# scroll-tech/zkevm-circuits

Hardware: AMD Instinct MI355X
Metric: SuperCircuit-shape proof-gen wall-clock (s) at k = 20 (lower is better)
Workload: dtype u32x8 limbs (254-bit modular integer, Montgomery)

## Files before the change

zkevm-circuits_amd/csrc/api.hip:

```cpp
#include <algorithm>
#include <set>

#include <thread>
#include "ctx.hpp"
#include "host_fq.hpp"
#include "host_util.hpp"

namespace zk {

Fr fr_from_u64(uint64_t v) {
    Fr a = Fr::zero();
    a.l[0] = (uint32_t)v;
    a.l[1] = (uint32_t)(v >> 32);
    return to_mont(a);
}
Fr fr_pow(Fr base, uint64_t e) { return pow_u64(base, e); }
Fr fr_inv_host(const Fr& a) { return inv(a); }
static Fr root_of_unity_28() {
    Fr c = Fr{{0x60c37c9cu, 0xd34f1ed9u, 0xd39329c8u, 0x3215cf6du, 0x3dd31f74u, 0x98865ea9u, 0x166d18b7u, 0x03ddb9f5u}};
    return to_mont(c);
}
Fr fr_root_of_unity(uint32_t log_n) {
    Fr w = root_of_unity_28();
    for (uint32_t i = log_n; i < 28; ++i) w = sqr(w);
// ... 32 lines not shown
        if (alias) st = prev_st;
        else {
            if (hipStreamCreateWithFlags(&st, hipStreamNonBlocking) != hipSuccess) { delete c; return ZK_ERR_HIP; }
            c->owned_streams.push_back(st);
            prev_st = st;
        }
        bool ok = st != nullptr;
        switch (alias ? *q - 'A' + 'a' : *q) {
            case 'm': if (c->stream) ok = false; else c->stream = st; break;
            case 'c': if (c->stream_copy) ok = false; else { c->stream_copy = st; ok = hipEventCreateWithFlags(&c->ev_copy, hipEventDisableTiming) == hipSuccess; } break;
            case 'a': if (c->stream_aux) ok = false; else { c->stream_aux = st; ok = hipEventCreateWithFlags(&c->ev_aux, hipEventDisableTiming) == hipSuccess; } break;
            case '2': if (c->stream2) ok = false; else c->stream2 = st; break;
            case 'b': if (c->stream2b) ok = false; else c->stream2b = st; break;
            case 'x': if (c->stream2c) ok = false; else c->stream2c = st; break;
            case 'd': break;
            default: ok = false;
        }
        if (!ok) { delete c; return ZK_ERR_INVALID_ARG; }
    }
    if (!c->stream) { delete c; return ZK_ERR_INVALID_ARG; }
    if (c->stream2) for (int i = 0; i < 3; ++i) { (void)hipEventCreateWithFlags(&c->ev_p1[i], hipEventDisableTiming); (void)hipEventCreateWithFlags(&c->ev_p2[i], hipEventDisableTiming); }
    c->own_stream = true;
    if (hipEventCreate(&c->ev0) != hipSuccess || hipEventCreate(&c->ev1) != hipSuccess) { delete c; return ZK_ERR_HIP; }
    *out = c;
    return ZK_OK;
}

void zk_ctx_destroy(zk_ctx* ctx) {
    if (!ctx) return;
    (void)hipSetDevice(ctx->device);
    (void)hipStreamSynchronize(ctx->stream);
    ctx->domains.clear();
    for (auto& kv : ctx->pow_tables) (void)hipFree(kv.second);
    ctx->pool_trim();
    ctx->prof_resolve();
    for (auto e : ctx->prof_pool) (void)hipEventDestroy(e);
    for (auto& s : ctx->scratch) if (s.ptr) (void)hipFree(s.ptr);
    if (ctx->ev0) (void)hipEventDestroy(ctx->ev0);
    if (ctx->ev1) (void)hipEventDestroy(ctx->ev1);
    zk::comm_release(ctx);
    std::set<hipStream_t> streams(ctx->owned_streams.begin(), ctx->owned_streams.end());
    for (hipStream_t st : {ctx->stream2, ctx->stream2b, ctx->stream2c, ctx->stream_aux, ctx->stream_copy}) if (st) streams.insert(st);
    if (ctx->own_stream && ctx->stream) streams.insert(ctx->stream); else streams.erase(ctx->stream);
    for (hipStream_t st : streams) { (void)hipStreamSynchronize(st); (void)hipStreamDestroy(st); }
    if (ctx->ev_aux) (void)hipEventDestroy(ctx->ev_aux);
    if (ctx->ev_copy) (void)hipEventDestroy(ctx->ev_copy);
    if (ctx->ev_pipe) (void)hipEventDestroy(ctx->ev_pipe);
    for (auto& kv : ctx->msm_graphs) (void)hipGraphExecDestroy((hipGraphExec_t)kv.second);
    for (auto e : ctx->ev_p1) if (e) (void)hipEventDestroy(e);
    for (auto e : ctx->ev_p2) if (e) (void)hipEventDestroy(e);
    delete ctx;
}

const char* zk_last_error(const zk_ctx* ctx) { return ctx ? ctx->err.c_str() : "null context"; }

int zk_ctx_set_stream(zk_ctx* ctx, void* hip_stream) {
    if (!ctx) return ZK_ERR_INVALID_ARG;
    ZK_HIP(ctx, hipStreamSynchronize(ctx->stream));
    if (ctx->own_stream && ctx->stream) {
        bool shared = false;
        for (hipStream_t st : {ctx->stream2, ctx->stream2b, ctx->stream2c, ctx->stream_aux, ctx->stream_copy}) shared |= st == ctx->stream;
        if (!shared) {
            ctx->owned_streams.erase(std::remove(ctx->owned_streams.begin(), ctx->owned_streams.end(), ctx->stream), ctx->owned_streams.end());
            (void)hipStreamDestroy(ctx->stream);
        }
        ctx->own_stream = false;
// ... 195 lines not shown
    Fr omega_inv = fr_inv_host(omega);
    Fr ninv = fr_inv_host(fr_from_u64(1ull << log_n));
    return ntt_run_many(ctx, (Fr* const*)d_datas, nullptr, count, log_n, omega_inv, &ninv, nullptr, nullptr, false);
}
int zk_ntt_omega(zk_ctx* ctx, void* d_data, uint32_t log_n, const void* h_omega) {
    if (!ctx) return ZK_ERR_INVALID_ARG;
    ZK_REQUIRE(ctx, d_data && h_omega, "null pointer");
    ZK_REQUIRE(ctx, log_n <= 28, "log_n exceeds the two-adicity of Fr (28)");
    return ntt_run(ctx, (Fr*)d_data, log_n, *(const Fr*)h_omega, nullptr, nullptr, nullptr);
}
int zk_coeff_to_extended(zk_ctx* ctx, const void* d_coeffs, uint32_t k, uint32_t ext_k, void* d_out) {
    if (!ctx) return ZK_ERR_INVALID_ARG;
    ZK_REQUIRE(ctx, d_coeffs && d_out && d_coeffs != d_out, "null or aliased pointer");
    ZK_REQUIRE(ctx, k <= ext_k && ext_k <= 28, "need k <= ext_k <= 28");
    const size_t n = (size_t)1 << k, ne = (size_t)1 << ext_k;
    ZK_HIP(ctx, hipMemcpyAsync(d_out, d_coeffs, n * sizeof(Fr), hipMemcpyDeviceToDevice, ctx->stream));
    if (ne > n) ZK_HIP(ctx, hipMemsetAsync((char*)d_out + n * sizeof(Fr), 0, (ne - n) * sizeof(Fr), ctx->stream));
    Fr zeta = fr_zeta();
    int rc = ntt_run(ctx, (Fr*)d_out, ext_k, fr_root_of_unity(ext_k), nullptr, &zeta, nullptr);
    return rc;
}
int zk_coeff_to_coset(zk_ctx* ctx, const void* d_coeffs, uint32_t k, const void* h_g, void* d_out) {
    if (!ctx) return ZK_ERR_INVALID_ARG;
    ZK_REQUIRE(ctx, d_coeffs && d_out && h_g, "null pointer");
    ZK_REQUIRE(ctx, k <= 28, "k exceeds the two-adicity of Fr (28)");
    return ntt_run(ctx, (Fr*)d_out, k, fr_root_of_unity(k), nullptr, (const Fr*)h_g, nullptr, d_coeffs == d_out ? nullptr : (const Fr*)d_coeffs, true);
}
int zk_coeff_to_coset_batch(zk_ctx* ctx, const void* const* d_coeffs, uint32_t k, const void* h_g, void* const* d_outs, size_t count) {
    if (!ctx) return ZK_ERR_INVALID_ARG;
    ZK_REQUIRE(ctx, (d_coeffs && d_outs) || !count, "null pointer");
    ZK_REQUIRE(ctx, h_g, "null pointer");
    ZK_REQUIRE(ctx, k <= 28, "k exceeds the two-adicity of Fr (28)");
    for (size_t i = 0; i < count; ++i) ZK_REQUIRE(ctx, d_coeffs[i] && d_outs[i], "null column pointer");
    return ntt_run_many(ctx, (Fr* const*)d_outs, (const Fr* const*)d_coeffs, count, k, fr_root_of_unity(k), nullptr, (const Fr*)h_g, nullptr, true);
}
int zk_extended_to_coeff(zk_ctx* ctx, void* d_ext, uint32_t ext_k) {
    if (!ctx) return ZK_ERR_INVALID_ARG;
    ZK_REQUIRE(ctx, d_ext, "null pointer");
    ZK_REQUIRE(ctx, ext_k <= 28, "ext_k exceeds 28");
    Fr omega_inv = fr_inv_host(fr_root_of_unity(ext_k));
    Fr ninv = fr_inv_host(fr_from_u64(1ull << ext_k));
    Fr zeta_inv = sqr(fr_zeta());
    return ntt_run(ctx, (Fr*)d_ext, ext_k, omega_inv, &ninv, nullptr, &zeta_inv);
}

int zk_msm_g1(zk_ctx* ctx, const void* d_scalars, const void* d_bases, size_t n, void* h_out_affine) {
    if (!ctx) return ZK_ERR_INVALID_ARG;
    ZK_REQUIRE(ctx, h_out_affine && ((d_scalars && d_bases) || n == 0), "null pointer");
    return msm_run(ctx, (const Fr*)d_scalars, (const G1Affine*)d_bases, n, (G1Affine*)h_out_affine);
}
int zk_commit(zk_ctx* ctx, const zk_srs* srs, int basis, const void* d_scalars, size_t n, void* h_out_affine) {
    if (!ctx) return ZK_ERR_INVALID_ARG;
    ZK_REQUIRE(ctx, srs && h_out_affine && (d_scalars || !n), "null pointer");
    ZK_REQUIRE(ctx, basis == 0 || basis == 1, "basis must be 0 (monomial) or 1 (Lagrange)");
    ZK_REQUIRE(ctx, n <= ((size_t)1 << srs->k), "polynomial longer than the SRS");
    const G1Affine* b = basis ? srs->g_lagrange : srs->g;
    ZK_REQUIRE(ctx, b, "SRS has no Lagrange basis");
    const Fr* sp = (const Fr*)d_scalars;
    return msm_batch_srs(ctx, srs, basis, &sp, 1, n, (G1Affine*)h_out_affine);
}
int zk_g1_sum_host(const void* h_points_affine, size_t n, void* h_out_affine) {
    if (!h_out_affine || (!h_points_affine && n)) return ZK_ERR_INVALID_ARG;
    const G1Affine* p = (const G1Affine*)h_points_affine;
    host::PXyzz acc;
    memset(&acc, 0, sizeof acc);
    const host::F4 one = host::fone<host::FqC>();
    for (size_t i = 0; i < n; ++i) {
// ... 178 lines not shown
```

zkevm-circuits_amd/csrc/ctx.hpp:

```cpp
#pragma once
#include <hip/hip_runtime.h>
#include <cstdarg>
#include <cstdio>
#include <cstring>
#include <map>
#include <memory>
#include <string>
#include <vector>

#include "../../include/zkmi355.h"
#include "ec.hip.hpp"
#include "ff.hip.hpp"

namespace zk {

struct NttDomain;

struct Scratch {
    void* ptr = nullptr;
    size_t cap = 0;
};

}

// ... 2 lines not shown
    hipStream_t stream = nullptr;
    bool own_stream = false;
    std::string err;
    hipEvent_t ev0 = nullptr, ev1 = nullptr;
    hipDeviceProp_t prop{};
    zk::Scratch scratch[19];
    hipStream_t stream2 = nullptr, stream2b = nullptr, stream2c = nullptr;
    std::vector<hipStream_t> owned_streams;
    hipEvent_t ev_p1[3] = {nullptr, nullptr, nullptr}, ev_p2[3] = {nullptr, nullptr, nullptr};
    std::map<uint64_t, std::vector<uint64_t>> msm_graph_keys;
    std::map<uint64_t, void*> msm_graphs;
    uint32_t msm_blinded_tail = 0;
    bool msm_graph_broken = false;
    hipEvent_t ev_pipe = nullptr;
    hipStream_t stream_copy = nullptr;
    hipEvent_t ev_copy = nullptr;
    hipStream_t stream_aux = nullptr;
    hipEvent_t ev_aux = nullptr;
    bool ensure_aux() {
        if (stream_aux) return ev_aux || hipEventCreateWithFlags(&ev_aux, hipEventDisableTiming) == hipSuccess;
        int least = 0, greatest = 0;
        const char* e = getenv("ZK_AUX_PRIORITY");
        const bool prio = e && atoi(e) == 1 && hipDeviceGetStreamPriorityRange(&least, &greatest) == hipSuccess && greatest != least;
        hipError_t rc = prio ? hipStreamCreateWithPriority(&stream_aux, hipStreamNonBlocking, greatest) : hipStreamCreateWithFlags(&stream_aux, hipStreamNonBlocking);
        if (rc != hipSuccess) { (void)hipGetLastError(); rc = hipStreamCreateWithFlags(&stream_aux, hipStreamNonBlocking); }
        if (rc != hipSuccess) { stream_aux = nullptr; return false; }
        if (!ev_aux && hipEventCreateWithFlags(&ev_aux, hipEventDisableTiming) != hipSuccess) return false;
        return true;
    }
    void* comm = nullptr;
    uint32_t comm_rank = 0, comm_world = 1;
    std::map<uint64_t, std::shared_ptr<zk::NttDomain>> domains;
    std::map<uint64_t, void*> pow_tables;
    std::vector<void*> pinned;
    std::map<size_t, std::vector<void*>> pool;
    size_t pool_bytes = 0, pool_cap = (size_t)96 << 30;
    size_t coset_cache_bytes = 0;
    void* pool_get(size_t bytes) {
        bytes = (bytes + 255) & ~(size_t)255;
        if (!bytes) bytes = 256;
        auto it = pool.find(bytes);
        if (it != pool.end() && !it->second.empty()) { void* p = it->second.back(); it->second.pop_back(); pool_bytes -= bytes; return p; }
        void* p = nullptr;
        if (hipMalloc(&p, bytes) == hipSuccess) return p;
        (void)hipGetLastError();
        pool_trim();
        if (hipMalloc(&p, bytes) == hipSuccess) return p;
        (void)hipGetLastError();
        return nullptr;
    }
    void pool_put(void* p, size_t bytes) {
        if (!p) return;
        bytes = (bytes + 255) & ~(size_t)255;
        if (!bytes) bytes = 256;
        if (pool_bytes + bytes > pool_cap) { (void)hipStreamSynchronize(stream); (void)hipFree(p); return; }
        pool[bytes].push_back(p);
        pool_bytes += bytes;
    }
    void pool_trim() {
        (void)hipStreamSynchronize(stream);
        for (auto& kv : pool) for (void* p : kv.second) (void)hipFree(p);
        pool.clear();
        pool_bytes = 0;
    }
    uint32_t msm_attr_set = 0;
    bool quotient_attr_set = false;
// ... 75 lines not shown
    zk::G1Affine* pfx_negtot_tab[2] = {nullptr, nullptr};
};

#define ZK_HIP(ctx, call)                                                                          \
    do {                                                                                           \
        hipError_t e__ = (call);                                                                   \
        if (e__ != hipSuccess) return (ctx)->fail(ZK_ERR_HIP, "%s failed: %s (%s:%d)", #call, hipGetErrorString(e__), __FILE__, __LINE__); \
    } while (0)

#define ZK_CHECK_LAUNCH(ctx)                                                                       \
    do {                                                                                           \
        hipError_t e__ = hipGetLastError();                                                        \
        if (e__ != hipSuccess) return (ctx)->fail(ZK_ERR_HIP, "kernel launch failed: %s (%s:%d)", hipGetErrorString(e__), __FILE__, __LINE__); \
    } while (0)

#define ZK_REQUIRE(ctx, cond, msg)                                                                 \
    do {                                                                                           \
        if (!(cond)) return (ctx)->fail(ZK_ERR_INVALID_ARG, "invalid argument: %s (%s:%d)", msg, __FILE__, __LINE__); \
    } while (0)

namespace zk {
enum ScratchSlot { SC_NTT = 0, SC_MSM_KEYS = 1, SC_MSM_BUCKETS = 2, SC_MSM_MISC = 3, SC_POLY = 4, SC_POLY2 = 5, SC_TMP = 6, SC_TMP2 = 7, SC_MSM_BUCKETS2 = 8, SC_MSM_RESULTS = 9, SC_QTMP = 10, SC_COMM = 11, SC_MSM_BUCKETS3 = 12, SC_MSM_BUCKETS4 = 13, SC_MSM_DESC = 14, SC_MSM_TAILS = 15, SC_NTT_AUX = 16, SC_QACC = 17, SC_QSLICE = 18 };

Fr fr_from_u64(uint64_t v);
Fr fr_pow(Fr base, uint64_t e);
Fr fr_inv_host(const Fr& a);
Fr fr_root_of_unity(uint32_t log_n);
Fr fr_zeta();

int ntt_run(zk_ctx* ctx, Fr* d_data, uint32_t log_n, const Fr& omega, const Fr* scale , const Fr* coset_pre , const Fr* coset_post ,
            const Fr* d_src = nullptr ,
            bool fuse_pre = false );
int ntt_run_many(zk_ctx* ctx, Fr* const* d_datas, const Fr* const* d_srcs, size_t count, uint32_t log_n, const Fr& omega, const Fr* scale, const Fr* coset_pre, const Fr* coset_post, bool fuse_pre);
int fr_scale_run(zk_ctx* ctx, Fr* d_a, const Fr& s, uint64_t n);
enum G1Enc : int { G1_ENC_COMPRESSED = 0, G1_ENC_RAW = 1, G1_ENC_BE_XY = 2 };
int g1_decode_run(zk_ctx* ctx, const void* d_in, int enc, G1Affine* d_out, uint64_t n, uint32_t* d_bad, uint8_t* d_bad_at);
int msm_run(zk_ctx* ctx, const Fr* d_scalars, const G1Affine* d_bases, size_t n, G1Affine* h_out);
int msm_run_rp(zk_ctx* ctx, const Fr* d_scalars, const G1Affine* d_bases, const G1Affine* d_bases_rp, size_t n, G1Affine* h_out);
int msm_batch_rp(zk_ctx* ctx, const Fr* const* d_scalar_ptrs, size_t count, const G1Affine* d_bases, const G1Affine* d_bases_rp, size_t n, G1Affine* h_out);
int msm_segments_run(zk_ctx* ctx, const Fr* d_scalars, const G1Affine* d_bases, const uint32_t* h_off, size_t num_segments, G1Affine* h_out);
int srs_bases_rp(zk_ctx* ctx, const zk_srs* srs, int basis, const G1Affine** out);
int srs_window_table(zk_ctx* ctx, const zk_srs* srs, int basis, size_t n, const G1Affine** out, size_t* stride);
typedef int (*MsmStageFn)(void* user, size_t it);
int msm_batch_tab(zk_ctx* ctx, const Fr* const* d_scalar_ptrs, size_t count, const G1Affine* d_bases, const G1Affine* d_bases_rp, const G1Affine* d_table, size_t tab_stride,
                  size_t n, G1Affine* h_out, MsmStageFn stage = nullptr, void* stage_user = nullptr);
int msm_batch_srs(zk_ctx* ctx, const zk_srs* srs, int basis, const Fr* const* d_scalar_ptrs, size_t count, size_t n, G1Affine* h_out, MsmStageFn stage = nullptr, void* stage_user = nullptr,
                  const uint8_t* narrow = nullptr );
int msm_runs_try(zk_ctx* ctx, const zk_srs* srs, int basis, const Fr* const* d_scalar_ptrs, size_t count, size_t n, const uint8_t* narrow, G1Affine* h_out, uint8_t* done);
int msm_diff_try(zk_ctx* ctx, const zk_srs* srs, int basis, const Fr* const* d_scalar_ptrs, size_t count, size_t n, const uint8_t* narrow, G1Affine* h_out, uint8_t* done);
int commit_batch_staged(zk_ctx* ctx, const zk_srs* srs, int basis, const void* const* d_scalar_ptrs, size_t count, size_t n, void* h_out_affine, MsmStageFn stage, void* stage_user, const uint8_t* narrow = nullptr);
void sample_narrow(const void* const* h_cols, size_t count, size_t n, uint8_t* narrow);
int sample_narrow_dev(zk_ctx* ctx, const void* const* d_cols, size_t count, size_t n, uint8_t* narrow);
int sample_narrow_dev_typed(zk_ctx* ctx, const void* const* d_cols, const uint8_t* widths, size_t count, size_t n, size_t rows, uint8_t* narrow);
int lookup_multiplicities_enqueue(zk_ctx* ctx, const Fr* const* d_inputs, size_t num_inputs, const Fr* d_table, size_t usable_rows, Fr* d_m, size_t n, uint32_t* d_status, bool reuse_hash = false);
struct MockFail { uint32_t kind, index, sub, row; };
int mock_hash_build(zk_ctx* ctx, const Fr* d_table, size_t rows, int scratch_slot, const uint32_t** slots_out, uint32_t* mask_out);
int mock_nonzero_enqueue(zk_ctx* ctx, const Fr* d_vals, const uint32_t* d_row_ids, uint32_t count, uint32_t kind, uint32_t index, uint32_t sub, MockFail* d_out, uint32_t cap, uint32_t* d_counter);
int mock_probe_enqueue(zk_ctx* ctx, const Fr* d_inputs, const Fr* d_table, const uint32_t* d_slots, uint32_t mask, const uint32_t* d_row_ids, uint32_t count,
                       uint32_t kind, uint32_t index, uint32_t sub, MockFail* d_out, uint32_t cap, uint32_t* d_counter);
int mock_perm_enqueue(zk_ctx* ctx, const Fr* const* d_sigma, const Fr* const* d_cols, const Fr* d_ids, const uint32_t* d_slots, uint32_t mask, uint32_t num_cols, uint32_t k,
                      uint32_t kind, MockFail* d_out, uint32_t cap, uint32_t* d_counter);
int fr_add_const_many(zk_ctx* ctx, const void* const* d_src, void* const* d_dst, size_t count, const void* h_k, size_t n);
int fr_from_uint_run(zk_ctx* ctx, hipStream_t stream, const void* d_packed, uint32_t width, uint64_t n, Fr* d_out);
int fr_from_uint_batch_run(zk_ctx* ctx, hipStream_t stream, const void* const* d_packed, const uint8_t* widths, size_t count, uint64_t n, Fr* const* d_out);
int sigma_from_mapping_run(zk_ctx* ctx, hipStream_t stream, const void* const* d_map, size_t count, uint64_t n, uint32_t P, const Fr* d_omega, const Fr* d_delta, uint32_t* d_bad, Fr* const* d_out);
int g_to_lagrange(zk_ctx* ctx, const G1Affine* d_g, uint32_t k, G1Affine* d_out);
// ... 9 lines not shown
```

zkevm-circuits_amd/csrc/ff29.hip.hpp:

```cpp
#pragma once
#include "ff.hip.hpp"

namespace zk {

constexpr uint32_t MASK29 = (1u << 29) - 1;

struct Fq29P {
    static constexpr uint32_t INV = 0x4866389u;
    __host__ __device__ static constexpr uint32_t M(int i) {
        constexpr uint32_t m[9] = {0x187cfd47u, 0x10460b6u, 0x1c72a34fu, 0x2d522d0u, 0x1585d978u, 0x2db40c0u, 0xa6e141u, 0xe5c2634u, 0x30644eu};
        return m[i];
    }
    using P32 = FqP;
};
struct Fr29P {
    static constexpr uint32_t INV = 0xfffffffu;
    __host__ __device__ static constexpr uint32_t M(int i) {
        constexpr uint32_t m[9] = {0x10000001u, 0x1f0fac9fu, 0xe5c2450u, 0x7d090f3u, 0x1585d283u, 0x2db40c0u, 0xa6e141u, 0xe5c2634u, 0x30644eu};
        return m[i];
    }
    using P32 = FrP;
};

template <class P>
// ... 354 lines not shown
    uint32_t m[9];
    F29<P> t;
    uint64_t acc = 0;
#pragma unroll
    for (int k = 0; k < 17; ++k) {
        const int lo = k < 9 ? 0 : k - 8, hi = k < 9 ? k : 8, nm = k < 9 ? k : 17 - k;
        uint32_t ys[9], ds[9], fs[9], ks[9];
#pragma unroll
        for (int i = lo; i <= hi; ++i) { ys[i - lo] = b.l[k - i]; ds[i - lo] = d.l[k - i]; fs[i - lo] = f.l[k - i]; ks[i - lo] = P::M(k - i); }
        acc = dotv(a.l + lo, ys, hi - lo + 1, acc);
        acc = dotv(c.l + lo, ds, hi - lo + 1, acc);
        acc = dotv(e.l + lo, fs, hi - lo + 1, acc);
        acc = dotk(m + lo, ks, nm, acc);
        if (k < 9) {
            m[k] = ((uint32_t)acc * P::INV) & MASK29;
            acc += (uint64_t)m[k] * P::M(0);
        } else {
            t.l[k - 9] = (uint32_t)acc & MASK29;
        }
        acc >>= 29;
    }
    t.l[8] = (uint32_t)acc;
    return t;
}
template <int K, class P>
__host__ __device__ __forceinline__ F29<P> neg29k(const F29<P>& b) {
    F29<P> r;
#pragma unroll
    for (int i = 0; i < 9; ++i) r.l[i] = kp_balanced<P>(K, i) - b.l[i];
    return r;
}

template <class P>
__host__ __device__ __forceinline__ Fp<typename P::P32> reduce_lazy29(const F29<P>& x) {
    constexpr uint64_t mhi = ((uint64_t)P::P32::M(7) << 32) | P::P32::M(6);
    constexpr uint32_t C = (uint32_t)((((unsigned __int128)1) << 92) / ((unsigned __int128)mhi + 1));
    const uint32_t q = (uint32_t)(((uint64_t)x.l[8] * C) >> 52);
    F29<P> r;
    int64_t c = 0;
#pragma unroll
    for (int i = 0; i < 9; ++i) {
        const int64_t s_ = (int64_t)x.l[i] - (int64_t)((uint64_t)q * P::M(i)) + c;
        r.l[i] = i < 8 ? (uint32_t)(s_ & MASK29) : (uint32_t)s_;
        c = s_ >> 29;
    }
    return pack29_lt2p(r);
}

template <class P>
__host__ __device__ __forceinline__ F29<P> sqr29_c(const F29<P>& a) {
    uint32_t m[9], a2[9];
#pragma unroll
    for (int i = 0; i < 9; ++i) a2[i] = a.l[i] << 1;
    F29<P> t;
    uint64_t acc = 0;
#pragma unroll
    for (int k = 0; k < 17; ++k) {
        const int lo = k < 9 ? 0 : k - 8, hi = k < 9 ? k : 8, nm = k < 9 ? k : 17 - k;
        uint32_t xs[9], ys[9], ks[9];
        int n = 0;
#pragma unroll
        for (int i = lo; 2 * i < k; ++i) { xs[n] = a2[i]; ys[n] = a.l[k - i]; ++n; }
        if (!(k & 1)) { xs[n] = a.l[k / 2]; ys[n] = a.l[k / 2]; ++n; }
#pragma unroll
        for (int i = lo; i <= hi; ++i) ks[i - lo] = P::M(k - i);
        acc = dotv(xs, ys, n, acc);
        acc = dotk(m + lo, ks, nm, acc);
        if (k < 9) {
            m[k] = ((uint32_t)acc * P::INV) & MASK29;
            acc += (uint64_t)m[k] * P::M(0);
        } else {
            t.l[k - 9] = (uint32_t)acc & MASK29;
        }
        acc >>= 29;
    }
    t.l[8] = (uint32_t)acc;
    return t;
}


// ... 88 lines not shown
```

zkevm-circuits_amd/csrc/ntt.hip:

```cpp
#include <climits>
#include <type_traits>

#include "ctx.hpp"
#include "ff29.hip.hpp"

namespace zk {

constexpr int NTT_MAX_DIGIT = 10;
constexpr int NTT_TILE = 4096;
constexpr int NTT_THREADS = 1024;
constexpr int NTT_LDS_BYTES_PER_ELT = 36;

struct Tw29;

constexpr int NTT_BATCH = 16;
struct NttIo { const Fr* src[NTT_BATCH]; Fr* dst[NTT_BATCH]; };

struct NttPass {
    int log_np;
    int log_m;
    const Tw29* tw;
    const Fr* out_tw = nullptr;
};

// ... 21 lines not shown
__device__ __forceinline__ uint32_t bitrev(uint32_t x, int bits) { return bits ? (__brev(x) >> (32 - bits)) : 0u; }

__host__ __device__ __forceinline__ Fr to_rprime(Fr x) {
#pragma unroll
    for (int i = 0; i < 5; ++i) x = dbl(x);
    return x;
}

struct Lds29 {
    uint32_t* p;
    int stride;
    __device__ __forceinline__ Fr29 load(int idx) const {
        Fr29 r;
#pragma unroll
        for (int k = 0; k < 9; ++k) r.l[k] = p[k * stride + idx];
        return r;
    }
    __device__ __forceinline__ void store(int idx, const Fr29& v) const {
#pragma unroll
        for (int k = 0; k < 9; ++k) p[k * stride + idx] = v.l[k];
    }
};

__global__ void k_powers(Fr base, Fr mul, Fr* out, uint32_t count, int rprime) {
    uint32_t j = blockIdx.x * blockDim.x + threadIdx.x;
    if (j >= count) return;
    Fr r = mul, b = base;
    uint32_t e = j;
    while (e) {
        if (e & 1) r = r * b;
        b = sqr(b);
        e >>= 1;
    }
    stg(out + j, rprime ? to_rprime(r) : r);
}

__device__ __forceinline__ Fr two_level(const Fr* __restrict__ lo, const Fr* __restrict__ hi, int h, uint32_t e) {
    return ldg(lo + (e & ((1u << h) - 1))) * ldg(hi + (e >> h));
}
__device__ __forceinline__ Fr29 two_level29(const Fr* __restrict__ lo, const Fr* __restrict__ hi, int h, uint32_t e) {
    return mul29(unpack29<Fr29P>(ldg(lo + (e & ((1u << h) - 1)))), unpack29<Fr29P>(ldg(hi + (e >> h))));
}

__global__ void k_build_out_twiddles(Fr* __restrict__ out_tw, const Fr* __restrict__ lo, const Fr* __restrict__ hi, int h, int log_np, int log_m, int tw_shift, uint64_t n,
                                     Fr fin, int apply_fin) {
    const uint64_t g = (uint64_t)blockIdx.x * blockDim.x + threadIdx.x;
    if (g >= n) return;
    const uint64_t m = 1ull << log_m;
    const uint32_t jpp = (uint32_t)(g & (m - 1)), d = (uint32_t)(g >> log_m) & ((1u << log_np) - 1);
    Fr29 v = two_level29(lo, hi, h, (jpp * d) << tw_shift);
    if (apply_fin) v = mul29(v, unpack29<Fr29P>(fin));
    stg(out_tw + g, pack29_lt2p(v));
}

__device__ __forceinline__ void bfly29(Fr29& u, Fr29& x, const Fr29& w) {
    const Fr29 v = mul29(x, w);
    Fr29 a0 = add29(u, v), a1 = sub29k<4>(u, v);
    normalize29(a0);
    normalize29(a1);
    u = a0;
    x = a1;
}
struct Tw29 { uint4 q[3]; };
__device__ __forceinline__ Fr29 tw29(const Tw29* __restrict__ tw, uint32_t idx) {
    const uint4 a = tw[idx].q[0], b = tw[idx].q[1], c = tw[idx].q[2];
    return Fr29{{a.x, a.y, a.z, a.w, b.x, b.y, b.z, b.w, c.x}};
}
// ... 123 lines not shown
    for (int s = 0; s < log_np;) {
        const int r = ((log_np - s) & 1) ? 1 : 2;
        auto step = [&](auto R, auto FIRST, auto LAST) {
            ntt_pass_step<decltype(R)::value, decltype(FIRST)::value, decltype(LAST)::value, OPT_RUNTIME, OPT_RUNTIME>(L, src, dst, tw, pre, out_tw, lo, hi, h, tw_shift, log_np, s, log_t, 1ull << log_m, t.base, t.blk);
        };
        if (s == 0) { if (r == 1) step(Int<1>{}, Bool<true>{}, Bool<false>{}); else step(Int<2>{}, Bool<true>{}, Bool<false>{}); }
        else if (s + r == log_np) step(Int<2>{}, Bool<false>{}, Bool<true>{});
        else step(Int<2>{}, Bool<false>{}, Bool<false>{});
        s += r;
        if (s < log_np) __syncthreads();
    }
}
template <int LOG_NP, int S, bool HAS_PRE>
__device__ __forceinline__ void ntt_pass_steps(const Lds29& L, const Fr* __restrict__ src, Fr* __restrict__ dst, const Tw29* __restrict__ tw,
                                               const Fr* __restrict__ pre, const Fr* __restrict__ out_tw, const int log_t, const uint64_t m, const uint64_t base) {
    constexpr int R = ((LOG_NP - S) & 1) ? 1 : 2;
    constexpr bool LAST = S + R == LOG_NP;
    ntt_pass_step<R, S == 0, LAST, HAS_PRE ? OPT_YES : OPT_NO, OPT_YES>(L, src, dst, tw, pre, out_tw, nullptr, nullptr, 0, 0, LOG_NP, S, log_t, m, base, 0u);
    if constexpr (!LAST) {
        __syncthreads();
        ntt_pass_steps<LOG_NP, S + R, HAS_PRE>(L, src, dst, tw, pre, out_tw, log_t, m, base);
    }
}
template <int LOG_NP, bool HAS_PRE>
__global__ void __launch_bounds__(NTT_THREADS)
k_ntt_pass_f(NttIo io, const Tw29* __restrict__ tw, const Fr* __restrict__ lo, const Fr* __restrict__ hi, int h, int , int log_t, int log_m, int tw_shift,
             const Fr* __restrict__ pre, const Fr* __restrict__ out_tw, uint32_t ncols, int xcd_cols, int log_grp) {
    extern __shared__ __attribute__((aligned(16))) uint32_t smem[];
    const PassTile t = pass_tile(LOG_NP, log_t, log_m, ncols, xcd_cols, log_grp);
    ntt_pass_steps<LOG_NP, 0, HAS_PRE>(Lds29{smem, 1 << (LOG_NP + log_t)}, io.src[t.col], io.dst[t.col], tw, pre, out_tw, log_t, 1ull << log_m, t.base);
}

__host__ __device__ __forceinline__ int ntt_row_pad(int log_np) { return log_np >= 8 ? 8 : 0; }
template <int R, bool FIRST, bool LAST, Opt PRE, Opt FOLDED>
__device__ __forceinline__ void ntt_last_step(const Lds29& L, const Fr* __restrict__ src, Fr* __restrict__ dst, const Tw29* __restrict__ tw, const Fr* __restrict__ pre,
                                              const Fr29& fin29, const bool fin_folded, const int log_np, const int s, const int log_t, const int row,
                                              const uint32_t blk, const uint32_t mid, const int log_mid, const int log_n1) {
    static_assert(R == 2 || FIRST, "only the first step of a pass can be radix 2");
    constexpr int NE = 1 << R;
    const int hgt = 1 << s, T = 1 << log_t, items = (1 << (log_np + log_t)) >> R;
    const bool has_pre = opt_on<PRE>(pre != nullptr), folded = opt_on<FOLDED>(fin_folded);
    for (int it = threadIdx.x; it < items; it += blockDim.x) {
        int c, b;
        if (LAST) { c = it & (T - 1); b = it >> log_t; }
        else { b = it & ((1 << (log_np - R)) - 1); c = it >> (log_np - R); }
        const int j = b & (hgt - 1);
        const int lo_d = ((b >> s) << (s + R)) | j;
        const uint64_t i1 = ((uint64_t)blk << log_t) + c;
        Fr29 e[4];
        if (FIRST) {
            Fr raw[NE], praw[NE];
            uint64_t gi[NE];
#pragma unroll
            for (int k = 0; k < NE; ++k) {
                gi[k] = (((i1 << log_mid) + mid) << log_np) + bitrev(lo_d + k * hgt, log_np);
                raw[k] = ldg(src + gi[k]);
                if (PRE == OPT_YES) praw[k] = ldg(pre + gi[k]);
            }
#pragma unroll
            for (int k = 0; k < NE; ++k) {
                e[k] = unpack29<Fr29P>(raw[k]);
                if (has_pre) e[k] = mul29(e[k], unpack29<Fr29P>(PRE == OPT_YES ? praw[k] : ldg(pre + gi[k])));
            }
            dit_first_step<R>(e, tw, log_np);
        } else {
#pragma unroll
            for (int k = 0; k < NE; ++k) e[k] = L.load(c * row + lo_d + k * hgt);
            dit_step<R>(e, tw, log_np, s, j);
        }
#pragma unroll
        for (int k = 0; k < NE; ++k) {
            const int dl = lo_d + k * hgt;
            if (LAST) stg(dst + (i1 + (((uint64_t)mid + ((uint64_t)dl << log_mid)) << log_n1)), folded ? reduce_lazy29(e[k]) : pack29_lt2p(mul29(e[k], fin29)));
            else L.store(c * row + dl, e[k]);
        }
    }
}

__device__ __forceinline__ uint32_t last_tile(int xcd_remap) {
    return xcd_remap ? (blockIdx.x & 7u) * (gridDim.x >> 3) + (blockIdx.x >> 3) : blockIdx.x;
}

__global__ void __launch_bounds__(NTT_THREADS)
k_ntt_last(NttIo io, const Tw29* __restrict__ tw, int log_np, int log_t, int log_n1, int log_mid, Fr fin, const Fr* __restrict__ pre, int fin_folded, int xcd_remap) {
    extern __shared__ __attribute__((aligned(16))) uint32_t smem[];
    const Fr* __restrict__ src = io.src[blockIdx.y];
    Fr* __restrict__ dst = io.dst[blockIdx.y];
    const int row = (1 << log_np) + ntt_row_pad(log_np);
    const Lds29 L{smem, row << log_t};
    const uint32_t bx = last_tile(xcd_remap), mid = bx & ((1u << log_mid) - 1), blk = bx >> log_mid;
    const Fr29 fin29 = unpack29<Fr29P>(fin);
    for (int s = 0; s < log_np;) {
        const int r = ((log_np - s) & 1) ? 1 : 2;
        const bool last = s + r == log_np;
        auto step = [&](auto R, auto FIRST, auto LAST) {
            ntt_last_step<decltype(R)::value, decltype(FIRST)::value, decltype(LAST)::value, OPT_RUNTIME, OPT_RUNTIME>(L, src, dst, tw, pre, fin29, fin_folded != 0, log_np, s, log_t, row, blk, mid, log_mid, log_n1);
        };
        if (s == 0 && last) { if (r == 1) step(Int<1>{}, Bool<true>{}, Bool<true>{}); else step(Int<2>{}, Bool<true>{}, Bool<true>{}); }
        else if (s == 0) { if (r == 1) step(Int<1>{}, Bool<true>{}, Bool<false>{}); else step(Int<2>{}, Bool<true>{}, Bool<false>{}); }
        else if (last) step(Int<2>{}, Bool<false>{}, Bool<true>{});
        else step(Int<2>{}, Bool<false>{}, Bool<false>{});
        s += r;
        if (s < log_np) __syncthreads();
    }
}
template <int LOG_NP, int S>
__device__ __forceinline__ void ntt_last_steps(const Lds29& L, const Fr* __restrict__ src, Fr* __restrict__ dst, const Tw29* __restrict__ tw,
                                               const int log_t, const int row, const uint32_t blk, const uint32_t mid, const int log_mid, const int log_n1) {
    constexpr int R = ((LOG_NP - S) & 1) ? 1 : 2;
    constexpr bool LAST = S + R == LOG_NP;
    ntt_last_step<R, S == 0, LAST, OPT_NO, OPT_YES>(L, src, dst, tw, nullptr, Fr29{}, true, LOG_NP, S, log_t, row, blk, mid, log_mid, log_n1);
    if constexpr (!LAST) {
        __syncthreads();
        ntt_last_steps<LOG_NP, S + R>(L, src, dst, tw, log_t, row, blk, mid, log_mid, log_n1);
    }
}
template <int LOG_NP>
__global__ void __launch_bounds__(NTT_THREADS)
k_ntt_last_f(NttIo io, const Tw29* __restrict__ tw, int , int log_t, int log_n1, int log_mid, Fr fin, const Fr* __restrict__ pre, int fin_folded, int xcd_remap) {
    extern __shared__ __attribute__((aligned(16))) uint32_t smem[];
    const int row = (1 << LOG_NP) + ntt_row_pad(LOG_NP);
    const uint32_t bx = last_tile(xcd_remap), mid = bx & ((1u << log_mid) - 1), blk = bx >> log_mid;
    ntt_last_steps<LOG_NP, 0>(Lds29{smem, row << log_t}, io.src[blockIdx.y], io.dst[blockIdx.y], tw, log_t, row, blk, mid, log_mid, log_n1);
}

__global__ void k_scale(Fr* a, Fr s, uint64_t n) {
    uint64_t i = (uint64_t)blockIdx.x * blockDim.x + threadIdx.x;
    if (i < n) stg(a + i, ldg(a + i) * s);
}
int fr_scale_run(zk_ctx* ctx, Fr* d_a, const Fr& s, uint64_t n) {
    if (!n) return ZK_OK;
    hipLaunchKernelGGL(k_scale, dim3((unsigned)((n + 255) / 256)), dim3(256), 0, ctx->stream, d_a, s, n);
    ZK_CHECK_LAUNCH(ctx);
    return ZK_OK;
}

__global__ void k_distribute_powers(const Fr* src, Fr* dst, const Fr* __restrict__ lo, const Fr* __restrict__ hi, int h, uint64_t n) {
    uint64_t i = (uint64_t)blockIdx.x * blockDim.x + threadIdx.x;
    if (i >= n) return;
    stg(dst + i, ldg(src + i) * two_level(lo, hi, h, (uint32_t)i));
}

static int build_powers(zk_ctx* ctx, const Fr& base, const Fr& mul, Fr* d_out, uint32_t count, int rprime) {
    hipLaunchKernelGGL(k_powers, dim3((count + 255) / 256), dim3(256), 0, ctx->stream, base, mul, d_out, count, rprime);
    ZK_CHECK_LAUNCH(ctx);
    return ZK_OK;
}

static uint64_t domain_key(uint32_t log_n, const Fr& omega, const Fr* scale) {
    uint64_t hsh = 1469598103934665603ull;
    auto mix = [&](uint32_t v) { hsh = (hsh ^ v) * 1099511628211ull; };
    mix(log_n);
    for (int i = 0; i < 8; ++i) mix(omega.l[i]);
    if (scale) for (int i = 0; i < 8; ++i) mix(scale->l[i] ^ 0x9e3779b9u);
    return hsh;
}
// ... 160 lines not shown
    NttPlan pl{};
    int log_tile = 11;
    if (kn.last_logtile >= 10 && kn.last_logtile <= 12) log_tile = kn.last_logtile;
    pl.log_t = std::min(std::max(log_tile - ps.log_np, 0), log_n1);
    pl.tile = 1 << (ps.log_np + pl.log_t);
    pl.blocks = (unsigned)((1ull << dom.log_n) >> (ps.log_np + pl.log_t));
    pl.fixed = kn.fixed && P > 1 && dom.fin_folded && has_fixed_instance(ps.log_np);
    pl.grid = dim3(pl.blocks, (unsigned)nb);
    pl.threads = plan_threads(pl.tile, pl.fixed);
    pl.lds = (size_t)(pl.tile + (ntt_row_pad(ps.log_np) << pl.log_t)) * NTT_LDS_BYTES_PER_ELT;
    pl.xcd = (log_mid == 0 && pl.blocks % 8 == 0 && pl.blocks >= 16 && kn.xcd_last) ? 1 : 0;
    return pl;
}

static bool pass_kernel_ready(zk_ctx* ctx, const void* kernel, size_t max_lds) {
    auto it = ctx->ntt_fixed_attr.find(kernel);
    if (it != ctx->ntt_fixed_attr.end()) return it->second;
    const bool ok = hipFuncSetAttribute(kernel, hipFuncAttributeMaxDynamicSharedMemorySize, (int)max_lds) == hipSuccess;
    if (!ok) (void)hipGetLastError();
    return ctx->ntt_fixed_attr[kernel] = ok;
}
constexpr size_t NTT_PASS_MAX_LDS = (size_t)NTT_TILE * NTT_LDS_BYTES_PER_ELT, NTT_LAST_MAX_LDS = (size_t)(NTT_TILE + 128) * NTT_LDS_BYTES_PER_ELT;

using PassKernel = decltype(&k_ntt_pass);
using LastKernel = decltype(&k_ntt_last);
static PassKernel pass_instance(int log_np, bool pre) {
    switch (log_np) {
        case 7: return pre ? k_ntt_pass_f<7, true> : k_ntt_pass_f<7, false>;
        case 8: return pre ? k_ntt_pass_f<8, true> : k_ntt_pass_f<8, false>;
        case 9: return pre ? k_ntt_pass_f<9, true> : k_ntt_pass_f<9, false>;
        default: return pre ? k_ntt_pass_f<10, true> : k_ntt_pass_f<10, false>;
    }
}
static LastKernel last_instance(int log_np) {
    switch (log_np) {
        case 7: return k_ntt_last_f<7>;
        case 8: return k_ntt_last_f<8>;
        case 9: return k_ntt_last_f<9>;
        default: return k_ntt_last_f<10>;
    }
}
static int launch_pass(zk_ctx* ctx, const NttDomain& dom, int p, size_t nb, const NttKnobs& kn, const NttIo& io, const Fr* pre) {
    const NttPass& ps = dom.pass[p];
    if (ps.log_np < 3) return ctx->fail(ZK_ERR_INVALID_ARG, "NTT: a strided pass over a digit of 2^%d", ps.log_np);
    NttPlan pl = plan_pass(dom, p, nb, kn, ps.out_tw != nullptr);
    PassKernel kernel = pl.fixed ? pass_instance(ps.log_np, pre != nullptr) : k_ntt_pass;
    if (pl.fixed && !pass_kernel_ready(ctx, (const void*)kernel, NTT_PASS_MAX_LDS)) {
        NttKnobs generic = kn;
        generic.fixed = false;
        pl = plan_pass(dom, p, nb, generic, ps.out_tw != nullptr);
        kernel = k_ntt_pass;
    }
    if (!pl.fixed && !pass_kernel_ready(ctx, (const void*)kernel, NTT_PASS_MAX_LDS)) return ctx->fail(ZK_ERR_HIP, "NTT: the device refuses %zu bytes of LDS per workgroup", NTT_PASS_MAX_LDS);
    ZkProfScope pscope(ctx, "ntt_pass");
    pscope.bytes = (uint64_t)nb * (1ull << dom.log_n) * 64 / (uint64_t)dom.npass;
    hipLaunchKernelGGL(kernel, pl.grid, dim3(pl.threads), pl.lds, ctx->stream, io, ps.tw, (const Fr*)dom.d_lo, (const Fr*)dom.d_hi, dom.h, ps.log_np, pl.log_t, ps.log_m,
                       (int)dom.log_n - ps.log_np - ps.log_m, pre, ps.out_tw, (uint32_t)nb, pl.xcd, pl.log_grp);
    ZK_CHECK_LAUNCH(ctx);
    return ZK_OK;
}
static int launch_last(zk_ctx* ctx, const NttDomain& dom, size_t nb, const NttKnobs& kn, const NttIo& io, const Fr* pre) {
    const int P = dom.npass;
    const NttPass& ps = dom.pass[P - 1];
    NttPlan pl = plan_last(dom, nb, kn);
    LastKernel kernel = pl.fixed ? last_instance(ps.log_np) : k_ntt_last;
    if (pl.fixed && !pass_kernel_ready(ctx, (const void*)kernel, NTT_LAST_MAX_LDS)) {
        NttKnobs generic = kn;
        generic.fixed = false;
        pl = plan_last(dom, nb, generic);
        kernel = k_ntt_last;
    }
    if (!pl.fixed && !pass_kernel_ready(ctx, (const void*)kernel, NTT_LAST_MAX_LDS)) return ctx->fail(ZK_ERR_HIP, "NTT: the device refuses %zu bytes of LDS per workgroup", NTT_LAST_MAX_LDS);
    ZkProfScope pscope(ctx, "ntt_last");
    pscope.bytes = (uint64_t)nb * (1ull << dom.log_n) * 64 / (uint64_t)P;
    hipLaunchKernelGGL(kernel, pl.grid, dim3(pl.threads), pl.lds, ctx->stream, io, ps.tw, ps.log_np, pl.log_t, P == 1 ? 0 : dom.pass[0].log_np, P == 3 ? dom.pass[1].log_np : 0,
                       dom.final_mul, pre, dom.fin_folded ? 1 : 0, pl.xcd);
    ZK_CHECK_LAUNCH(ctx);
    return ZK_OK;
}

static size_t columns_per_launch(uint32_t log_n, size_t count, bool coset_pass, const NttKnobs& kn) {
    if (count <= 1 || coset_pass) return 1;
    const uint64_t tiles = std::max<uint64_t>(1, (1ull << log_n) >> 12);
    size_t per_launch = (size_t)std::min<uint64_t>(NTT_BATCH, std::max<uint64_t>(1, 4096 / tiles));
    if (kn.batch >= 1 && kn.batch <= NTT_BATCH) per_launch = (size_t)kn.batch;
    return per_launch;
}

int ntt_run(zk_ctx* ctx, Fr* d_data, uint32_t log_n, const Fr& omega, const Fr* scale, const Fr* coset_pre, const Fr* coset_post, const Fr* d_src, bool fuse_pre) {
    return ntt_run_many(ctx, &d_data, d_src ? &d_src : nullptr, 1, log_n, omega, scale, coset_pre, coset_post, fuse_pre);
}
int ntt_run_many(zk_ctx* ctx, Fr* const* d_datas, const Fr* const* d_srcs, size_t count, uint32_t log_n, const Fr& omega, const Fr* scale, const Fr* coset_pre, const Fr* coset_post, bool fuse_pre) {
    if (count == 0) return ZK_OK;
    const NttKnobs kn = read_ntt_knobs();
    if (log_n == 0) {
        for (size_t i = 0; i < count; ++i) {
            if (d_srcs && d_srcs[i] && d_srcs[i] != d_datas[i]) ZK_HIP(ctx, hipMemcpyAsync(d_datas[i], d_srcs[i], sizeof(Fr), hipMemcpyDeviceToDevice, ctx->stream));
            if (scale) {
                hipLaunchKernelGGL(k_scale, dim3(1), dim3(64), 0, ctx->stream, d_datas[i], *scale, (uint64_t)1);
                ZK_CHECK_LAUNCH(ctx);
            }
        }
        return ZK_OK;
    }
    const uint64_t n = 1ull << log_n;
    const Fr* pre_table = nullptr;
    int rc = (coset_pre && fuse_pre) ? get_pow_table(ctx, log_n, *coset_pre, POW_FULL, &pre_table) : ZK_OK;
    if (rc) return rc;
    const bool pre_apart = coset_pre && !pre_table;
    std::shared_ptr<NttDomain> dom;
    rc = get_domain(ctx, kn, log_n, omega, scale, &dom);
    if (rc) return rc;
    const int P = dom->npass;
    size_t per_launch = columns_per_launch(log_n, count, pre_apart || coset_post, kn);
    Fr* scratch = nullptr;
    if (P > 1) {
        const int slot = ctx->stream_aux && ctx->stream == ctx->stream_aux ? SC_NTT_AUX : SC_NTT;
        for (;;) {
            scratch = (Fr*)ctx->get_scratch(slot, sizeof(Fr) * n * per_launch);
            if (scratch || per_launch == 1) break;
            (void)hipGetLastError();
            per_launch = (per_launch + 1) / 2;
        }
        if (!scratch) return ZK_ERR_OOM;
    }
    for (size_t first = 0; first < count; first += per_launch) {
        const size_t nb = std::min(per_launch, count - first);
        NttIo io{};
        for (size_t j = 0; j < nb; ++j) {
            Fr* dd = d_datas[first + j];
            io.src[j] = d_srcs && d_srcs[first + j] ? d_srcs[first + j] : dd;
            if (pre_apart) { rc = run_distribute(ctx, log_n, *coset_pre, io.src[j], dd); if (rc) return rc; io.src[j] = dd; }
        }
        for (int p = 0; p + 1 < P; ++p) {
            for (size_t j = 0; j < nb; ++j) io.dst[j] = (p == P - 2) ? scratch + j * n : d_datas[first + j];
            rc = launch_pass(ctx, *dom, p, nb, kn, io, p == 0 ? pre_table : nullptr);
            if (rc) return rc;
            for (size_t j = 0; j < nb; ++j) io.src[j] = io.dst[j];
        }
        for (size_t j = 0; j < nb; ++j) io.dst[j] = d_datas[first + j];
        rc = launch_last(ctx, *dom, nb, kn, io, P == 1 ? pre_table : nullptr);
        if (rc) return rc;
        if (coset_post) for (size_t j = 0; j < nb; ++j) { rc = run_distribute(ctx, log_n, *coset_post, io.dst[j], io.dst[j]); if (rc) return rc; }
    }
    return ZK_OK;
}

template <int W>
__global__ void __launch_bounds__(256) k_ntt_cross(const Fr* __restrict__ recv, Fr* __restrict__ out, size_t cols, const Fr* __restrict__ tw , Fr scale, int scaled) {
    const size_t c = (size_t)blockIdx.x * blockDim.x + threadIdx.x;
    if (c >= cols) return;
    constexpr int LOGW = W == 2 ? 1 : W == 4 ? 2 : W == 8 ? 3 : 4;
    Fr a[W];
#pragma unroll
    for (int i = 0; i < W; ++i) {
        int rev = 0;
#pragma unroll
        for (int b = 0; b < LOGW; ++b) rev |= ((i >> b) & 1) << (LOGW - 1 - b);
        a[rev] = ldg(recv + (size_t)i * cols + c);
    }
#pragma unroll
    for (int st = 1; st <= LOGW; ++st) {
#pragma unroll
        for (int h = 0; h < W / 2; ++h) {
            const int half = 1 << (st - 1), t = h & (half - 1), lo = ((h >> (st - 1)) << st) + t, hi = lo + half;
            const Fr u = a[lo];
            const Fr v = t == 0 ? a[hi] : a[hi] * tw[t << (LOGW - st)];
            a[lo] = u + v;
            a[hi] = u - v;
        }
    }
#pragma unroll
    for (int j = 0; j < W; ++j) stg(out + (size_t)j * cols + c, scaled ? a[j] * scale : a[j]);
}

}

using namespace zk;
// ... 74 lines not shown
```

zkevm-circuits_amd/csrc/prover.hip:

```cpp
#include <algorithm>
#include <array>
#include <unordered_map>
#include <unordered_set>
#include <memory>
#include <string>

#include <chrono>
#include <cstdlib>
#include <random>
#include <tuple>
#include <functional>
#include "ctx.hpp"
#include "host_hash.hpp"
#include "cs.hpp"
#include "quotient_plan.hpp"

using namespace zk;
using zk::host::F4;
using namespace zk::cs;
using namespace zk::qplan;

extern "C" int zk_quotient_eval(zk_ctx*, const uint32_t*, uint32_t, const void* const*, uint32_t, const void*, uint32_t, uint32_t, uint32_t, int, void*);
extern "C" int zk_fr_powers(zk_ctx*, const void*, const void*, void*, size_t);
extern "C" int zk_ntt(zk_ctx*, void*, uint32_t, int);
extern "C" int zk_fr_batch_invert(zk_ctx*, void*, size_t);
extern "C" int zk_fr_random(zk_ctx*, const uint8_t*, uint64_t, uint64_t, void*, size_t);
extern "C" int zk_lookup_multiplicities(zk_ctx*, const void*, const void*, size_t, void*, size_t, uint64_t*);
extern "C" int zk_coeff_to_coset(zk_ctx*, const void*, uint32_t, const void*, void*);
extern "C" int zk_coeff_to_coset_batch(zk_ctx*, const void* const*, uint32_t, const void*, void* const*, size_t);
extern "C" int zk_fr_scatter_scaled(zk_ctx*, const void*, size_t, const void*, void*, size_t, size_t);
extern "C" int zk_msm_g1(zk_ctx*, const void*, const void*, size_t, void*);
extern "C" int zk_g1_sum_host(const void*, size_t, void*);
extern "C" int zk_poly_eval_batch(zk_ctx*, const void* const*, size_t, size_t, const void*, void*);
extern "C" int zk_poly_eval_pairs(zk_ctx*, const void* const*, const uint32_t*, size_t, const void*, size_t, size_t, void*);

namespace {

static thread_local zk_ctx* tl_pool_ctx = nullptr;
struct PoolScope {
    zk_ctx* prev;
    explicit PoolScope(zk_ctx* c) : prev(tl_pool_ctx) { tl_pool_ctx = c; }
    ~PoolScope() { tl_pool_ctx = prev; }
};

struct DevBuf {
// ... 27 lines not shown
        owner = nullptr;
        return hipMalloc(&p, n ? n : 1) == hipSuccess;
    }
    Fr* fr() const { return (Fr*)p; }
};

struct PinnedBuf {
    void* p = nullptr;
    ~PinnedBuf() { if (p) (void)hipHostFree(p); }
    bool alloc(size_t bytes) { return hipHostMalloc(&p, bytes ? bytes : 1, hipHostMallocDefault) == hipSuccess; }
};


struct StageTrace {
    zk_ctx* ctx; bool on; std::chrono::steady_clock::time_point t0;
    explicit StageTrace(zk_ctx* c) : ctx(c), on(getenv("ZK_PROVER_TRACE") != nullptr), t0(std::chrono::steady_clock::now()) {}
    void mark(const char* what) {
        if (!on) return;
        (void)hipStreamSynchronize(ctx->stream);
        const auto t1 = std::chrono::steady_clock::now();
        fprintf(stderr, "[zk prover] %-28s %8.2f ms\n", what, std::chrono::duration<double, std::milli>(t1 - t0).count());
        t0 = t1;
    }
};

}

struct zk_pk : zk::cs::ConstraintSystem {
    std::vector<DevBuf> fixed_lag, fixed_coeff, sigma_lag, sigma_coeff;
    DevBuf omega_lag, l0_lag, llast_lag, lactive_lag, l0_coeff, llast_coeff, lactive_coeff;
    mutable std::vector<std::unordered_map<uint32_t, DevBuf>> part_cache;
    mutable int part_cache_state = -1;
    mutable size_t part_cache_bytes = 0;
    std::vector<G1Affine> fixed_com, sigma_com;
    F4 vk_repr;
    const zk_srs* srs = nullptr;
    mutable std::shared_ptr<const QuotientPlan> qplan;
};

struct zk_proof {
    const zk_pk* pk;
    host::XorShiftRng rng;
    host::Transcript tr;
    std::vector<DevBuf> inst_lag, inst_coeff, adv_lag, adv_coeff;
    std::vector<std::vector<DevBuf>> adv_coset;
    std::vector<uint32_t> pre_mask;
    bool pre_planned = false;
    uint32_t phase = 0;
    int multiopen = ZK_MULTIOPEN_GWC;
    int vanishing_random = ZK_VANISHING_ONE;
    bool advice_on_device = false;
    bool advice_in_place = false;
    bool lag_partial = false;
    std::vector<F4> absorbed;
    zk_transcript_vtable ext_vt{};
    uint32_t rank = 0, world = 1;
    zk_allgather_fn gather = nullptr;
    void* gather_user = nullptr;
    bool use_comm = false;
    zk_allgather_fn gather_dev = nullptr;
    void* gather_dev_user = nullptr;
    std::vector<F4> challenges;
    zk_proof(const zk_pk* k, const uint8_t* seed) : pk(k), rng(seed), inst_lag(k->I), inst_coeff(k->I), adv_lag(k->A), adv_coeff(k->A), challenges(k->chal_phase.size(), host::fr_zero()) {}
};

namespace {

#define PK_TRY(expr) do { int rc__ = (expr); if (rc__) return rc__; } while (0)
#define PK_ALLOC(ctx, buf, nbytes) do { if (!(buf).alloc(nbytes)) return (ctx)->fail(ZK_ERR_OOM, "prover: alloc failed"); } while (0)

struct StreamRestore {
    zk_ctx* c; hipStream_t s;
    explicit StreamRestore(zk_ctx* ctx) : c(ctx), s(ctx->stream) {}
    ~StreamRestore() { c->stream = s; }
};

size_t device_free_bytes(bool* ok = nullptr) {
    size_t free_b = 0, total_b = 0;
    const bool got = hipMemGetInfo(&free_b, &total_b) == hipSuccess;
    if (!got) { (void)hipGetLastError(); free_b = 0; }
    if (ok) *ok = got;
    return free_b;
}

struct PairOwners {
    uint32_t E = 0, rank = 0;
    bool sharded = false;
    std::vector<uint32_t> owner;
    size_t at(uint32_t e, uint32_t r) const { return ((size_t)e << E) | r; }
    bool mine(uint32_t e, uint32_t r) const { return class_on_coset(E, e, r) && (!sharded || owner[at(e, r)] == rank); }
};

template <class Count>
std::vector<std::pair<uint32_t, uint32_t>> cosets_by_columns_served(uint32_t R, Count served) {
    std::vector<std::pair<uint32_t, uint32_t>> by_count;
    for (uint32_t r = 0; r < R; ++r) {
        const uint32_t cnt = served(r);
        if (cnt) by_count.push_back({cnt, r});
    }
    std::sort(by_count.begin(), by_count.end(), [](const auto& a, const auto& b) { return a.first != b.first ? a.first > b.first : a.second < b.second; });
    return by_count;
}

int lincomb(zk_ctx* ctx, uint32_t k, const std::vector<const void*>& polys, const F4& ch, void* d_out) {
    std::vector<uint32_t> words;
    std::vector<const void*> cols;
    for (size_t j = polys.size(); j-- > 0;) { words.insert(words.end(), {Q_PUSH_COL, (uint32_t)cols.size(), 0u, Q_FOLD, 0u, 0u}); cols.push_back(polys[j]); }
    return zk_quotient_eval(ctx, words.data(), (uint32_t)(words.size() / 3), cols.data(), (uint32_t)cols.size(), &ch, 1, k, k, 0, d_out);
}

int commit_lagrange(zk_ctx* ctx, const zk_srs* srs, const Fr* d_vals, size_t n, G1Affine* out) { return zk_commit(ctx, srs, 1, d_vals, n, out); }
int commit_coeff(zk_ctx* ctx, const zk_srs* srs, const Fr* d_vals, size_t n, G1Affine* out) { return zk_commit(ctx, srs, 0, d_vals, n, out); }

int to_coeff(zk_ctx* ctx, const zk_pk* pk, const DevBuf& lag, DevBuf* coeff) {
    const size_t n = (size_t)1 << pk->k;
// ... 64 lines not shown
        default: break;
    }
    if (ref >= C_DELTA0 && ref - C_DELTA0 < e.beta_delta.size()) { *out = e.beta_delta[ref - C_DELTA0]; return true; }
    if (ref >= C_CHAL0 && ref - C_CHAL0 < e.challenges.size()) { *out = e.challenges[ref - C_CHAL0]; return true; }
    if (ref >= C_YPOW0 && ref < C_CHAL0) { *out = ref - C_YPOW0 < e.ypow.size() ? e.ypow[ref - C_YPOW0] : host::fr_pow(e.y, ref - C_YPOW0); return true; }
    return false;
}
int concretise(zk_ctx* ctx, const Env& e, const Prog& g, Concrete* c) {
    for (const Instr& in : g) {
        uint32_t a = in.a;
        if (in.op == Q_PUSH_COL) {
            auto it = c->col_index.find(in.a);
            if (it == c->col_index.end()) {
                const void* p = resolve_col(e, in.a);
                if (!p) return ctx->fail(ZK_ERR_INVALID_ARG, "prover: unresolved column reference 0x%08x", in.a);
                a = (uint32_t)c->cols.size();
                c->cols.push_back(p);
                c->col_index[in.a] = a;
            } else a = it->second;
        } else if (in.op == Q_PUSH_CONST || in.op == Q_FOLD || in.op == Q_MUL_CONST || in.op == Q_ADD_CONST) {
            auto it = c->const_index.find(in.a);
            if (it == c->const_index.end()) {
                F4 v;
                if (!resolve_const(e, in.a, &v)) return ctx->fail(ZK_ERR_INVALID_ARG, "prover: unresolved constant reference 0x%08x", in.a);
                a = (uint32_t)c->consts.size();
                c->consts.push_back(v);
                c->const_index[in.a] = a;
            } else a = it->second;
        }
        c->words.push_back(in.op); c->words.push_back(a); c->words.push_back(in.b);
    }
    return ZK_OK;
}
int run_program(zk_ctx* ctx, const Env& e, const Prog& g, void* d_out) {
    Concrete c;
    PK_TRY(concretise(ctx, e, g, &c));
    {
        static const int alias = getenv("ZK_QUOTIENT_ALIAS") ? atoi(getenv("ZK_QUOTIENT_ALIAS")) : 0;
        if (alias > 0 && ctx->prof_tag && !strcmp(ctx->prof_tag, "quotient_coset")) for (size_t i = 0; i < c.cols.size(); ++i) c.cols[i] = c.cols[i % (size_t)alias];
    }
    return zk_quotient_eval(ctx, c.words.data(), (uint32_t)(c.words.size() / 3), c.cols.data(), (uint32_t)c.cols.size(),
                            c.consts.empty() ? nullptr : c.consts.data(), (uint32_t)c.consts.size(), e.pk->k, e.pk->k, 0, d_out);
}
const Fr* coeff_of(const zk_pk* pk, uint32_t ref, const std::vector<DevBuf>& adv, const std::vector<DevBuf>& inst, const std::vector<DevBuf>& pz,
                   const std::vector<DevBuf>& lkm, const std::vector<DevBuf>& lkphi) {
    const uint32_t type = ref >> 24, idx = ref & 0xFFFFFF;
    auto at = [&](const std::vector<DevBuf>& v) -> const Fr* { return idx < v.size() ? v[idx].fr() : nullptr; };
    switch (type) {
        case CT_FIXED: return at(pk->fixed_coeff);
        case CT_ADVICE: return at(adv);
        case CT_INSTANCE: return at(inst);
        case CT_SPECIAL: return idx == SP_L0 ? pk->l0_coeff.fr() : idx == SP_LLAST ? pk->llast_coeff.fr() : idx == SP_LACTIVE ? pk->lactive_coeff.fr() : nullptr;
        case CT_PERM_Z: return at(pz);
        case CT_SIGMA: return at(pk->sigma_coeff);
        case CT_LK_M: return at(lkm);
        case CT_LK_PHI: return at(lkphi);
        default: return nullptr;
    }
}

size_t share_size(const zk_proof* pr, size_t count) { return (count + pr->world - 1) / pr->world; }
int share_gather(zk_ctx* ctx, const zk_proof* pr, const void* local, size_t count, size_t elem, void* out) {
    const size_t per = share_size(pr, count);
    std::vector<uint8_t> all(per * pr->world * elem);
    if (per && pr->gather(pr->gather_user, local, per * elem, all.data())) return ctx->fail(ZK_ERR_INVALID_ARG, "sharded session: all-gather callback failed");
    for (size_t i = 0; i < count; ++i) memcpy((uint8_t*)out + i * elem, all.data() + ((i % pr->world) * per + i / pr->world) * elem, elem);
    return ZK_OK;
}

int sharded_commit(zk_ctx* ctx, const zk_proof* pr, const zk_srs* srs, int basis, const void* const* ptrs, size_t count, size_t n, G1Affine* out, uint8_t kind = 0 ) {
    const std::vector<uint8_t> hint(count, kind);
    if (pr->world <= 1 || !pr->gather) return commit_batch_staged(ctx, srs, basis, ptrs, count, n, out, nullptr, nullptr, hint.data());
    if (count < pr->world && n >= ((size_t)pr->world << 10)) {
        const size_t base = n / pr->world, rem = n % pr->world;
        const size_t lo = pr->rank * base + std::min<size_t>(pr->rank, rem), len = base + (pr->rank < rem ? 1 : 0);
// ... 505 lines not shown
    StageTrace trace(ctx);
    struct Stage {
        zk_ctx* ctx; size_t body, tail;
        std::vector<const void*> src; std::vector<void*> dst; std::vector<F4> blind_v; const F4* blind = nullptr;
        std::vector<uint8_t> width;
        void* packed = nullptr;
        bool grouped = false; size_t expanded = 0;
        uint32_t world = 1;
        hipMemcpyKind kind = hipMemcpyHostToDevice;
        std::vector<size_t> own;
        const zk_pk* pk = nullptr; std::vector<DevBuf*> lag, coeff;
        zk_proof* pr = nullptr; std::vector<uint32_t> col; std::vector<size_t> pending; std::vector<Fr> g_of_r;
        int flush() {
            if (pending.empty()) return ZK_OK;
            StreamRestore back(ctx);
            ctx->stream = ctx->stream_aux;
            const size_t n_ = (size_t)1 << pk->k;
            std::vector<Fr*> dsts;
            std::vector<const Fr*> srcs;
            for (size_t c_ : pending) {
                PK_ALLOC(ctx, *coeff[c_], n_ * 32);
                dsts.push_back(coeff[c_]->fr());
                srcs.push_back(lag[c_]->fr());
            }
            const Fr omega_inv = fr_inv_host(fr_root_of_unity(pk->k)), ninv = fr_inv_host(fr_from_u64(1ull << pk->k));
            PK_TRY(ntt_run_many(ctx, dsts.data(), srcs.data(), dsts.size(), pk->k, omega_inv, &ninv, nullptr, nullptr, false));
            for (size_t r = 0; r < g_of_r.size(); ++r) {
                std::vector<const void*> csrc;
                std::vector<void*> cdst;
                for (size_t c_ : pending) {
                    const uint32_t gc = col[c_];
                    if (!(pr->pre_mask[gc] >> r & 1u)) continue;
                    DevBuf& slot = pr->adv_coset[r][gc];
                    if (!slot.alloc(n_ * 32)) {
                        for (uint32_t& m_ : pr->pre_mask) m_ = 0;
                        break;
                    }
                    csrc.push_back(coeff[c_]->p);
                    cdst.push_back(slot.p);
                }
                if (!csrc.empty()) PK_TRY(zk_coeff_to_coset_batch(ctx, csrc.data(), pk->k, &g_of_r[r], cdst.data(), csrc.size()));
            }
            pending.clear();
            return ZK_OK;
        }
    } sg{ctx, (size_t)pk->u * 32, (size_t)(pk->bf + 1) * 32, {}, {}, {}};
    sg.pk = pk;
    sg.pr = pr;
    sg.kind = dev_src ? hipMemcpyDeviceToDevice : hipMemcpyHostToDevice;
    sg.grouped = dev_src && widths;
    for (uint32_t c = 0; c < pk->A; ++c) {
        if (!seen[c]) continue;
        if (in_place && by_col[c] && (!owner_only || sg.dst.size() % pr->world == pr->rank)) pr->adv_lag[c].borrow(const_cast<void*>(by_col[c]));
        else if (!pr->adv_lag[c].alloc(n * 32)) return ctx->fail(ZK_ERR_OOM, "prover: alloc of %zu bytes failed", n * 32);
        sg.src.push_back(by_col[c]);
        sg.width.push_back(width_of[c]);
        sg.dst.push_back(pr->adv_lag[c].p);
        sg.lag.push_back(&pr->adv_lag[c]);
        sg.coeff.push_back(&pr->adv_coeff[c]);
        sg.col.push_back(c);
        for (uint32_t r = 0; r <= pk->bf; ++r) sg.blind_v.push_back(pr->rng.next_fr());
    }
    DevBuf packed_buf;
    size_t widest_packed = 0;
    for (uint8_t w : sg.width) if (w < 32) widest_packed = std::max<size_t>(widest_packed, w);
    if (widest_packed && !sg.grouped) {
        PK_ALLOC(ctx, packed_buf, (size_t)pk->u * widest_packed);
        sg.packed = packed_buf.p;
    }
    PinnedBuf blind_pinned;
    if (!blind_pinned.alloc(sg.blind_v.size() * sizeof(F4))) return ctx->fail(ZK_ERR_OOM, "prover: pinned staging allocation failed");
    memcpy(blind_pinned.p, sg.blind_v.data(), sg.blind_v.size() * sizeof(F4));
    sg.blind = (const F4*)blind_pinned.p;
    trace.mark("  advice: blinding rows drawn and staged");
// ... 175 lines not shown
        const int rc = choose_quotient_plan(*pk, knobs, &pk->qplan, &err);
        if (rc) return ctx->fail(rc, "%s", err.c_str());
    }
    *out = pk->qplan;
    return ZK_OK;
}
static int advice_coset_plan(zk_ctx* ctx, const zk_pk* pk, std::vector<uint32_t>& mask, size_t* key_slots = nullptr) {
    std::shared_ptr<const QuotientPlan> qp;
    PK_TRY(quotient_plan(ctx, pk, &qp));
    advice_coset_masks(*pk, *qp, mask, key_slots);
    return ZK_OK;
}
static int advice_lagrange_readers(zk_ctx* ctx, const zk_pk* pk, std::vector<uint8_t>* need) {
    std::shared_ptr<const QuotientPlan> qp;
    PK_TRY(quotient_plan(ctx, pk, &qp));
    advice_lagrange_readers(*pk, *qp, need);
    return ZK_OK;
}


static int plan_advice_cosets(zk_ctx* ctx, zk_proof* pr) {
    pr->pre_planned = true;
    const zk_pk* pk = pr->pk;
    const bool sharded = pr->world > 1 && pr->gather;
    const char* env = getenv("ZK_ADVICE_COSET_GB");
    const double cap = (env ? atof(env) : (pr->advice_on_device ? 0.0 : 64.0)) * (double)(1ull << 30);
    if (sharded || cap <= 0 || pk->A == 0) return ZK_OK;
    std::vector<uint32_t> mask;
    size_t key_slots = 0;
    PK_TRY(advice_coset_plan(ctx, pk, mask, &key_slots));
    const uint32_t E = pk->ext_k - pk->k, R = 1u << E;
    if (E > 5) return ZK_OK;
    const double col_bytes = (double)((size_t)1 << pk->k) * 32.0;
    bool mem_known = false;
    const size_t free_b = device_free_bytes(&mem_known);
    if (!mem_known) return ZK_OK;
    const double cols_ahead = (pr->advice_in_place ? 1.0 : 2.0) * pk->A + 3.0 * (2.0 * pk->L + pk->C) + (2.0 * pk->L + pk->C + pk->I + 8.0) + 2.0 * R + 32.0;
    double avail = (double)free_b + (double)ctx->pool_bytes - cols_ahead * col_bytes - 16.0 * (double)(1ull << 30);
    if (pk->part_cache_state < 0 || (pk->part_cache_state == 1 && pk->part_cache_bytes == 0)) {
        const double key_need = (double)key_slots * col_bytes;
        const char* kenv = getenv("ZK_PK_COSET_CACHE_GB");
        const double kcap = std::min((kenv ? atof(kenv) : 96.0) * (double)(1ull << 30), (double)ctx->prop.totalGlobalMem / 3.0);
        if (key_need <= kcap) avail -= std::max(0.0, key_need - (double)pk->part_cache_bytes);
    }
    const double budget = std::min(cap, avail);
    const auto by_count = cosets_by_columns_served(R, [&](uint32_t r) { uint32_t cnt = 0; for (uint32_t m_ : mask) cnt += m_ >> r & 1u; return cnt; });
    uint32_t chosen = 0;
    double used = 0;
    for (const auto& cr : by_count) {
        uint32_t rest = 0;
        for (uint32_t m_ : mask) rest += (m_ & ~(chosen | 1u << cr.second)) != 0;
        if (used + cr.first * col_bytes > cap || used + (cr.first + rest) * col_bytes > avail) break;
        used += cr.first * col_bytes;
        chosen |= 1u << cr.second;
    }
    if (getenv("ZK_PROVER_TRACE")) {
        fprintf(stderr, "[zk prover] advice coset plan: free %.1f + pooled %.1f GiB, reserve %.1f GiB, budget %.1f GiB, cosets by columns served:", free_b / 1073741824.0, ctx->pool_bytes / 1073741824.0,
                (cols_ahead * col_bytes) / 1073741824.0 + 16.0, budget / 1073741824.0);
        for (const auto& cr : by_count) fprintf(stderr, " r%u:%u", cr.second, cr.first);
        fprintf(stderr, " -> chosen 0x%x\n", chosen);
    }
    if (!chosen) return ZK_OK;
    pr->pre_mask.assign(pk->A, 0u);
    for (uint32_t c = 0; c < pk->A; ++c) pr->pre_mask[c] = mask[c] & chosen;
    pr->adv_coset.resize(R);
    for (auto& v : pr->adv_coset) v.resize(pk->A);
    if (getenv("ZK_PROVER_TRACE")) fprintf(stderr, "[zk prover] advice cosets computed ahead: cosets 0x%x, %.1f GiB\n", chosen, used / (double)(1ull << 30));
    return ZK_OK;
}

int zk_pk_quotient_plan(zk_ctx* ctx, const zk_pk* pk, uint32_t* out_summary, size_t cap_summary) {
    if (!ctx) return ZK_ERR_INVALID_ARG;
    ZK_REQUIRE(ctx, pk && out_summary, "null pointer");
    std::shared_ptr<const QuotientPlan> qp;
    PK_TRY(quotient_plan(ctx, pk, &qp));
    if (write_plan_summary(*qp, out_summary, cap_summary, 0xFFFFFFFFu, nullptr, 0, nullptr)) return ctx->fail(ZK_ERR_INVALID_ARG, "zk_pk_quotient_plan: the summary needs %u words", 8 + 8 * (qp->E + 1));
    return ZK_OK;
}


struct Finish {
    zk_ctx* ctx;
    zk_proof* pr;
    const zk_pk* pk;
    const zk_srs* srs;
    const uint32_t k, ext_k;
    const size_t n;
    Env lag;
    StageTrace trace;
    const bool sharded;
    const bool shard_args;
    std::vector<uint32_t> act;
    bool late_cosets = false;
    std::vector<std::vector<DevBuf>> lk_f;
    std::vector<DevBuf> lk_t, lk_m, lk_phi;
    std::vector<uint8_t> same_table;
    std::vector<uint32_t> table_owner;
    std::vector<DevBuf> pz_lag;
    DevBuf random_coeff;
    std::vector<DevBuf> pz_coeff, m_coeff, phi_coeff, rem_coeff;
    DevBuf h;
    F4 x, w, w_inv;
    std::vector<Open> evals, queries;
    size_t e_fix = 0, e_random = 0, e_sigma = 0, e_lk = 0;
    std::vector<size_t> e_pz;
    DevBuf hcomb;
    F4 h_eval;

    Finish(zk_ctx* c, zk_proof* p)
        : ctx(c), pr(p), pk(p->pk), srs(p->pk->srs), k(p->pk->k), ext_k(p->pk->ext_k), n((size_t)1 << p->pk->k),
          lag{p->pk, nullptr, &p->adv_lag, &p->inst_lag, nullptr, nullptr, nullptr, host::fr_one(), host::fr_one(), host::fr_one(), host::fr_one(), {}, p->challenges},
          trace(c), sharded(p->world > 1 && p->gather),
          shard_args(sharded && pk->L >= p->world && !(getenv("ZK_SHARD_LOOKUPS") && atoi(getenv("ZK_SHARD_LOOKUPS")) == 0)),
          lk_f(pk->L), lk_t(pk->L), lk_m(pk->L), lk_phi(pk->L), same_table(pk->L, 0), table_owner(pk->L, 0), pz_lag(pk->C),
          pz_coeff(pk->C), m_coeff(pk->L), phi_coeff(pk->L), e_pz(pk->C) {
        for (uint32_t l = 0; l < pk->L; ++l) if (!shard_args || l % pr->world == pr->rank) act.push_back(l);
        const Fr t = fr_root_of_unity(k);
        memcpy(w.l, &t, 32);
        w_inv = host::fr_inv(w);
    }
    Finish(const Finish&) = delete;
    Finish& operator=(const Finish&) = delete;

    F4 rotate(int32_t rot) const { F4 p = x; const F4 b = rot >= 0 ? w : w_inv; for (int32_t i = 0; i < (rot >= 0 ? rot : -rot); ++i) p = host::fr_mul(p, b); return p; }
    int32_t norm_rot(int32_t rot) const { const int64_t nn = (int64_t)n; return (int32_t)((((int64_t)rot % nn) + nn) % nn); }
    F4 point_of(int32_t nrot) const { const int64_t nn = (int64_t)n; return rotate(nrot > nn / 2 ? (int32_t)(nrot - nn) : nrot); }
};

struct AuxJoin { zk_ctx* c; const bool* on; ~AuxJoin() { if (*on && c->stream_aux) (void)hipStreamSynchronize(c->stream_aux); } };

static int stage_late_advice_cosets(Finish& f) {
    zk_ctx* ctx = f.ctx; zk_proof* pr = f.pr; const zk_pk* pk = f.pk; const size_t n = f.n;
    const char* env = getenv("ZK_ADVICE_COSET_LATE_GB");
    const double cap = (env ? atof(env) : 0.0) * (double)(1ull << 30);
    const uint32_t E = f.ext_k - f.k, R = 1u << E;
    if (f.sharded || !(cap > 0) || !pk->A || E > 5 || !ctx->ensure_aux()) return ZK_OK;
    std::vector<uint32_t> mask;
    size_t key_slots = 0;
    PK_TRY(advice_coset_plan(ctx, pk, mask, &key_slots));
    if (pr->adv_coset.empty()) { pr->adv_coset.resize(R); for (auto& v : pr->adv_coset) v.resize(pk->A); }
    const double col_bytes = (double)n * 32.0;
    const size_t free_b = device_free_bytes();
    double avail = (double)free_b + (double)ctx->pool_bytes - (4.0 * (2.0 * pk->L + pk->C) + (2.0 * pk->L + pk->C + pk->I + 8.0) + 2.0 * R + 32.0) * col_bytes - 24.0 * (double)(1ull << 30);
    if (pk->part_cache_state < 0 || (pk->part_cache_state == 1 && pk->part_cache_bytes == 0)) avail -= (double)key_slots * col_bytes;
    auto todo = [&](uint32_t r, uint32_t c) { return (mask[c] >> r & 1u) && !pr->adv_coset[r][c].p && pr->adv_coeff[c].p; };
    const auto by_count = cosets_by_columns_served(R, [&](uint32_t r) { uint32_t cnt = 0; for (uint32_t c = 0; c < pk->A; ++c) cnt += todo(r, c); return cnt; });
    double used = 0;
    StreamRestore back(ctx);
    const hipStream_t main_stream = ctx->stream;
    const Fr w_ext = fr_root_of_unity(f.ext_k);
    for (const auto& cr : by_count) {
        if (used + cr.first * col_bytes > std::min(cap, avail)) continue;
        Fr g = fr_zeta();
        for (uint32_t i = 0; i < cr.second; ++i) g = g * w_ext;
        std::vector<const void*> csrc;
        std::vector<void*> cdst;
        bool ok = true;
        for (uint32_t c = 0; c < pk->A && ok; ++c) {
            if (!todo(cr.second, c)) continue;
            DevBuf& slot = pr->adv_coset[cr.second][c];
            if (!slot.alloc(n * 32)) { ok = false; break; }
            csrc.push_back(pr->adv_coeff[c].p);
            cdst.push_back(slot.p);
        }
        if (!f.late_cosets) {
            ZK_HIP(ctx, hipEventRecord(ctx->ev_aux, main_stream));
            ZK_HIP(ctx, hipStreamWaitEvent(ctx->stream_aux, ctx->ev_aux, 0));
        }
        ctx->stream = ctx->stream_aux;
        f.late_cosets = true;
        if (!csrc.empty()) PK_TRY(zk_coeff_to_coset_batch(ctx, csrc.data(), f.k, &g, cdst.data(), csrc.size()));
        ctx->stream = main_stream;
        used += csrc.size() * col_bytes;
        if (!ok) break;
    }
    if (f.late_cosets) {
        ZK_HIP(ctx, hipEventRecord(ctx->ev_aux, ctx->stream_aux));
        if (getenv("ZK_PROVER_TRACE")) fprintf(stderr, "[zk prover] advice cosets computed beside the lookup / permutation stages: %.1f GiB\n", used / (double)(1ull << 30));
    }
    return ZK_OK;
}

static int exchange_owned(Finish& f, std::vector<DevBuf>& cols) {
    zk_ctx* ctx = f.ctx; const zk_proof* pr = f.pr; const size_t n = f.n;
    const size_t total = cols.size(), W = pr->world, groups_total = (total + W - 1) / W;
    static const size_t xg_knob = getenv("ZK_SHARD_EXCHANGE_GROUPS") ? (size_t)atol(getenv("ZK_SHARD_EXCHANGE_GROUPS")) : 16;
    const size_t XG = std::max<size_t>(1, std::min(xg_knob, groups_total));
    DevBuf gbuf, sbuf;
    PK_ALLOC(ctx, gbuf, W * XG * n * 32);
    PK_ALLOC(ctx, sbuf, XG * n * 32);
    HostStaging host;
    for (size_t grp0 = 0; grp0 < groups_total; grp0 += XG) {
        const size_t gcnt = std::min(XG, groups_total - grp0);
        for (size_t g = 0; g < gcnt; ++g) {
            const size_t mine_c = (grp0 + g) * W + pr->rank;
            if (mine_c < total) ZK_HIP(ctx, hipMemcpyAsync((char*)sbuf.p + g * n * 32, cols[mine_c].p, n * 32, hipMemcpyDeviceToDevice, ctx->stream));
            else ZK_HIP(ctx, hipMemsetAsync((char*)sbuf.p + g * n * 32, 0, n * 32, ctx->stream));
        }
        bool on_device = false;
        PK_TRY(allgather_rows(ctx, pr, false, sbuf.p, true, gcnt * n * 32, gbuf.p, host, &on_device));
        if (!on_device) PK_TRY(zk_h2d(ctx, gbuf.p, host.recv.data(), host.recv.size()));
        for (size_t g = 0; g < gcnt; ++g)
            for (uint32_t q_ = 0; q_ < W; ++q_) {
                const size_t c_ = (grp0 + g) * W + q_;
// ... 271 lines not shown
            PK_TRY(run_program(ctx, lag_r, rp.prog, f.rem_coeff[j].p));
            const F4 yp = host::fr_pow(f.lag.y, K - 1 - rp.last);
            PK_TRY(zk_fr_scale(ctx, f.rem_coeff[j].p, &yp, n));
            dsts.push_back(f.rem_coeff[j].fr());
        }
        const Fr omega_inv = fr_inv_host(fr_root_of_unity(pk->k)), ninv = fr_inv_host(fr_from_u64(1ull << pk->k));
        PK_TRY(ntt_run_many(ctx, dsts.data(), nullptr, dsts.size(), pk->k, omega_inv, &ninv, nullptr, nullptr, false));
        f.trace.mark("  quotient: remainders of the split constraints");
    }
    for (uint32_t e = 0; e <= E; ++e)
        if (q.cls(e).used || e == E) {
            PK_ALLOC(ctx, q.h[e], ((size_t)n << e) * 32);
            if (!q.cls(e).used) ZK_HIP(ctx, hipMemsetAsync(q.h[e].p, 0, ((size_t)n << e) * 32, ctx->stream));
        }
    return ZK_OK;
}

static void quotient_decide_key_cache(Finish& f, const Quotient& q) {
    zk_ctx* ctx = f.ctx; const zk_pk* pk = f.pk; const size_t n = f.n;
    const std::vector<uint32_t>& refs = q.plan->refs;
    size_t key_slots = 0;
    for (uint32_t ref : refs) {
        if (!key_column(ref)) continue;
        for (uint32_t r = 0; r < q.nparts; ++r) {
            bool read = false;
            for (uint32_t e = 0; e <= q.E && !read; ++e) read = q.cls(e).used && class_on_coset(q.E, e, r) && q.reads(e, ref);
            key_slots += read;
        }
    }
    const char* env = getenv("ZK_PK_COSET_CACHE_GB");
    double budget = (env ? atof(env) : 96.0) * (double)(1ull << 30);
    budget = std::min(budget, (double)ctx->prop.totalGlobalMem / 3.0) - (double)ctx->coset_cache_bytes;
    const size_t free_b = device_free_bytes();
    const double need = (double)key_slots * n * 32.0;
    const double session = (double)refs.size() * n * 32.0 + (double)((size_t)n << q.E) * 32.0 * 2.0;
    pk->part_cache_state = (need <= budget && need + session <= (double)free_b + (double)ctx->pool_bytes) ? 1 : 0;
    if (pk->part_cache_state) pk->part_cache.resize(q.nparts);
}

static int quotient_deal_pairs(Finish& f, const Quotient& q, CosetPass& cp) {
    zk_ctx* ctx = f.ctx; const zk_proof* pr = f.pr;
    const uint32_t E = q.E;
    cp.deal.resize(f.sharded ? pr->world : 1);
    cp.owners = PairOwners{E, pr->rank, f.sharded, std::vector<uint32_t>((size_t)(E + 1) << E, 0u)};
    if (f.sharded) {
        PK_ALLOC(ctx, cp.rtmp, f.n * 32);
        std::vector<QPair> all;
        for (uint32_t e = 0; e <= E; ++e)
            if (q.cls(e).used)
                for (uint32_t r = 0; r < q.nparts; r += 1u << (E - e)) all.push_back({e, r, (double)q.cls(e).refs.size() + (double)q.cls(e).prog.size() / 64.0});
        std::stable_sort(all.begin(), all.end(), [](const QPair& a, const QPair& b) { return a.cost > b.cost; });
        std::vector<double> load(pr->world, 0.0);
        for (const QPair& pp_ : all) {
            uint32_t best = 0;
            for (uint32_t q_ = 1; q_ < pr->world; ++q_) if (load[q_] < load[best]) best = q_;
            load[best] += pp_.cost;
            cp.deal[best].push_back(pp_);
            cp.owners.owner[cp.owners.at(pp_.e, pp_.r)] = best;
        }
        for (auto& d_ : cp.deal) std::sort(d_.begin(), d_.end(), [](const QPair& a, const QPair& b) { return a.r != b.r ? a.r < b.r : a.e < b.e; });
    }
    const Fr w_ext = fr_root_of_unity(f.ext_k);
    Fr g = fr_zeta();
    for (uint32_t r_ = 0; r_ < q.nparts; ++r_) {
        bool any = false;
        for (uint32_t e = 0; e <= E && !any; ++e) any = q.cls(e).used && cp.owners.mine(e, r_);
        if (any) cp.cosets.push_back({r_, g});
        g = g * w_ext;
    }
    return ZK_OK;
}

static int quotient_transform(Finish& f, const Quotient& q, CosetPass& cp, CosetWork& w) {
    zk_ctx* ctx = f.ctx; zk_proof* pr = f.pr; const zk_pk* pk = f.pk; const size_t n = f.n;
    const std::vector<uint32_t>& refs = q.plan->refs;
    std::vector<DevBuf>& bufs = cp.part_buf;
    const bool cache_on = cp.cache_on;
    const uint32_t k = f.k;
    const Fr w_n = fr_root_of_unity(k);
    auto pre_coset = [&](uint32_t ref, uint32_t r) -> const void* {
        if ((ref >> 24) != CT_ADVICE || r >= pr->adv_coset.size()) return nullptr;
        const uint32_t c_ = ref & 0xFFFFFFu;
        return c_ < pr->adv_coset[r].size() ? pr->adv_coset[r][c_].p : nullptr;
    };
    const uint32_t r_ = w.r;
    w.active.clear();
    for (uint32_t e = 0; e <= q.E; ++e)
        if (q.cls(e).used && cp.owners.mine(e, r_)) w.active.push_back(e);
    w.part_of.clear();
    std::vector<const void*> bat_src;
    std::vector<void*> bat_dst;
    std::vector<std::pair<uint32_t, DevBuf>> fresh_slots;
    for (size_t i = 0; i < refs.size(); ++i) {
        bool needed = false;
        for (uint32_t e : w.active) needed |= q.reads(e, refs[i]);
        if (!needed) continue;
        if (const void* pre = pre_coset(refs[i], r_)) { w.part_of[refs[i]] = pre; continue; }
        if (!(cache_on && key_column(refs[i])) && !bufs[i].p) PK_ALLOC(ctx, bufs[i], n * 32);
        void* dst = bufs[i].p;
        DevBuf fresh;
        const bool cached = cache_on && key_column(refs[i]);
        if (cached) {
            auto it = pk->part_cache[r_].find(refs[i]);
            if (it != pk->part_cache[r_].end()) { w.part_of[refs[i]] = it->second.p; continue; }
            const char* env_fail = getenv("ZK_PK_COSET_CACHE_FAIL_AFTER");
            const bool inject = env_fail && pk->part_cache_bytes / (n * 32) + fresh_slots.size() >= (size_t)atoll(env_fail);
            bool got = pk->part_cache_state == 1 && !inject && fresh.alloc_unpooled(n * 32);
            if (!got && pk->part_cache_state == 1) {
                (void)hipGetLastError();
                ctx->pool_trim();
                got = !inject && fresh.alloc_unpooled(n * 32);
                if (!got) { (void)hipGetLastError(); pk->part_cache_state = 2; }
            }
            if (got) dst = fresh.p;
            else {
                if (!bufs[i].p) PK_ALLOC(ctx, bufs[i], n * 32);
                dst = bufs[i].p;
            }
        }
        w.part_of[refs[i]] = dst;
        if (refs[i] == colref(CT_SPECIAL, SP_X)) PK_TRY(zk_fr_powers(ctx, &w_n, &w.g, dst, n));
        else {
            const Fr* cf = (refs[i] >> 24) == CT_SPLIT_R ? ((refs[i] & 0xFFFFFFu) < f.rem_coeff.size() ? f.rem_coeff[refs[i] & 0xFFFFFFu].fr() : nullptr)
                                                         : coeff_of(pk, refs[i], pr->adv_coeff, pr->inst_coeff, f.pz_coeff, f.m_coeff, f.phi_coeff);
            if (!cf) return ctx->fail(ZK_ERR_INVALID_ARG, "prover: unresolved column reference 0x%08x", refs[i]);
            bat_src.push_back(cf);
            bat_dst.push_back(dst);
        }
        if (cached && fresh.p) fresh_slots.emplace_back(refs[i], std::move(fresh));
    }
    PK_TRY(zk_coeff_to_coset_batch(ctx, bat_src.data(), k, &w.g, bat_dst.data(), bat_src.size()));
    for (auto& fs : fresh_slots) {
        pk->part_cache_bytes += n * 32;
        ctx->coset_cache_bytes += n * 32;
        pk->part_cache[r_][fs.first] = std::move(fs.second);
    }
    return ZK_OK;
}

static int quotient_programs(Finish& f, Quotient& q, CosetPass& cp, CosetWork& w) {
    zk_ctx* ctx = f.ctx; const size_t n = f.n;
    const uint32_t k = f.k, E = q.E, K = q.K;
    const bool sharded = f.sharded;
    const Fr one_fr = Fr::one();
    DevBuf& hpart = cp.hpart;
    Env& part = cp.part;
    std::vector<DevBuf>& mine = cp.mine;
    const uint32_t r_ = w.r;
    part.part = &w.part_of;
    Fr gn = w.g;
    for (uint32_t i = 0; i < k; ++i) gn = sqr(gn);
    const Fr vinv = fr_inv_host(gn - Fr::one());
    for (uint32_t e : w.active) {
        ctx->prof_tag = "quotient_coset";
        const int rc_q = run_program(ctx, part, q.cls(e).prog, hpart.p);
        ctx->prof_tag = nullptr;
        PK_TRY(rc_q);
        const F4 yp = host::fr_pow(f.lag.y, K - 1 - q.cls(e).last);
        Fr scale;
        memcpy((void*)&scale, yp.l, 32);
        scale = scale * vinv;
        if (sharded) {
            PK_TRY(zk_fr_scale(ctx, hpart.p, &scale, n));
            DevBuf keep;
            PK_ALLOC(ctx, keep, n * 32);
            ZK_HIP(ctx, hipMemcpyAsync(keep.p, hpart.p, n * 32, hipMemcpyDeviceToDevice, ctx->stream));
            mine.push_back(std::move(keep));
        }
        PK_TRY(zk_fr_scatter_scaled(ctx, hpart.p, n, sharded ? &one_fr : &scale, q.h[e].p, (size_t)1 << e, r_ >> (E - e)));
    }
    return ZK_OK;
}

static int quotient_exchange_pairs(Finish& f, Quotient& q, CosetPass& cp) {
    zk_ctx* ctx = f.ctx; const zk_proof* pr = f.pr; const size_t n = f.n;
    const Fr one_fr = Fr::one();
    if (cp.mine.size() != cp.deal[pr->rank].size()) return ctx->fail(ZK_ERR_INVALID_ARG, "sharded session: %zu pairs evaluated, %zu dealt", cp.mine.size(), cp.deal[pr->rank].size());
    size_t rounds = 0;
    for (const auto& d_ : cp.deal) rounds = std::max(rounds, d_.size());
    for (size_t t = 0; t < rounds; ++t) {
        const void* mine_t = t < cp.mine.size() ? cp.mine[t].p : cp.hpart.p;
        if ((pr->use_comm || pr->gather_dev) && !cp.gbuf.p) PK_ALLOC(ctx, cp.gbuf, (size_t)pr->world * n * 32);
        bool on_device = false;
        PK_TRY(allgather_rows(ctx, pr, pr->use_comm, mine_t, t < cp.mine.size(), n * 32, cp.gbuf.p, cp.host, &on_device));
        for (uint32_t q_ = 0; q_ < pr->world; ++q_) {
            if (q_ == pr->rank || t >= cp.deal[q_].size()) continue;
            const QPair& pp_ = cp.deal[q_][t];
            const void* src = on_device ? (const void*)((const char*)cp.gbuf.p + (size_t)q_ * n * 32) : nullptr;
            if (!src) { PK_TRY(zk_h2d(ctx, cp.rtmp.p, cp.host.recv.data() + (size_t)q_ * n * 32, n * 32)); src = cp.rtmp.p; }
            PK_TRY(zk_fr_scatter_scaled(ctx, src, n, &one_fr, q.h[pp_.e].p, (size_t)1 << pp_.e, pp_.r >> (q.E - pp_.e)));
        }
    }
    return ZK_OK;
}

static int quotient_to_coeff(Finish& f, Quotient& q) {
    zk_ctx* ctx = f.ctx;
    const uint32_t E = q.E;
    DevBuf& h = q.h[E];
    for (uint32_t e = 0; e < E; ++e) {
        if (!q.cls(e).used) continue;
        PK_TRY(zk_extended_to_coeff(ctx, q.h[e].p, f.k + e));
    }
    PK_TRY(zk_extended_to_coeff(ctx, h.p, f.ext_k));
    for (uint32_t e = 0; e < E; ++e) {
        if (!q.cls(e).used) continue;
        PK_TRY(zk_field_vec_op(ctx, ZK_FIELD_FR, ZK_OP_ADD, h.p, q.h[e].p, h.p, f.n << e));
        q.h[e].release();
    }
    f.h = std::move(h);
    return ZK_OK;
}

static int stage_quotient(Finish& f) {
    zk_ctx* ctx = f.ctx;
    Quotient q;
    PK_TRY(quotient_prepare(f, q));
    {
        CosetPass cp;
        if (f.pk->part_cache_state < 0) quotient_decide_key_cache(f, q);
        cp.cache_on = f.pk->part_cache_state >= 1;
        cp.part_buf.resize(q.plan->refs.size());
        PK_ALLOC(ctx, cp.hpart, f.n * 32);
        if (f.late_cosets) ZK_HIP(ctx, hipStreamWaitEvent(ctx->stream, ctx->ev_aux, 0));
        cp.part = f.lag;
        PK_TRY(quotient_deal_pairs(f, q, cp));
        CosetWork work;
        for (const auto& rg : cp.cosets) {
            work.r = rg.first; work.g = rg.second;
            PK_TRY(quotient_transform(f, q, cp, work));
            f.trace.mark("  quotient: cosets of the columns");
            PK_TRY(quotient_programs(f, q, cp, work));
            f.trace.mark("  quotient: program");
        }
        if (f.sharded) PK_TRY(quotient_exchange_pairs(f, q, cp));
    }
    PK_TRY(quotient_to_coeff(f, q));
    f.trace.mark("quotient eval + ifft");
    return ZK_OK;
}

static int stage_h_commits(Finish& f) {
    zk_ctx* ctx = f.ctx; const size_t n = f.n;
    const uint32_t pieces = f.pk->d - 1;
    std::vector<const void*> hptrs(pieces);
    for (uint32_t i = 0; i < pieces; ++i) hptrs[i] = f.h.fr() + (size_t)i * n;
    std::vector<G1Affine> coms(pieces);
    PK_TRY(sharded_commit(ctx, f.pr, f.srs, 0, hptrs.data(), pieces, n, coms.data()));
    for (const G1Affine& com : coms) f.pr->tr.write_point(com);
    f.trace.mark("h commits");
    return ZK_OK;
}
// ... 225 lines not shown

static int multiopen_gwc(Finish& f) {
    zk_ctx* ctx = f.ctx; const size_t n = f.n; host::Transcript& tr = f.pr->tr;
    const std::vector<Open>& queries = f.queries;
    DevBuf batch, wit;
    PK_ALLOC(ctx, batch, n * 32);
    PK_ALLOC(ctx, wit, n * 32);
    const F4 v = tr.squeeze();
    std::vector<int32_t> rots;
    for (const Open& o : queries) if (std::find(rots.begin(), rots.end(), o.rot) == rots.end()) rots.push_back(o.rot);
    for (int32_t rot : rots) {
        std::vector<const void*> members;
        for (const Open& o : queries) if (o.rot == rot) members.push_back(o.poly);
        PK_TRY(lincomb(ctx, f.k, members, v, batch.p));
        const F4 z = f.point_of(rot);
        PK_TRY(zk_kate_division(ctx, batch.p, n, &z, wit.p));
        G1Affine com;
        PK_TRY(commit_coeff(ctx, f.srs, wit.fr(), n - 1, &com));
        tr.write_point(com);
    }
    PK_TRY(zk_ctx_sync(ctx));
    f.trace.mark("multiopen");
    return ZK_OK;
}

static int write_proof_out(zk_ctx* ctx, const host::Transcript& tr, void* h_proof, size_t proof_cap, size_t* proof_len) {
    if (tr.err) return ctx->fail(ZK_ERR_INVALID_ARG, "transcript failed with status %d (external callback, or the identity point in a Poseidon / EVM transcript)", tr.err);
    *proof_len = tr.proof.size();
    if (tr.proof.size() > proof_cap) return ctx->fail(ZK_ERR_INVALID_ARG, "proof buffer too small: need %zu bytes", tr.proof.size());
    memcpy(h_proof, tr.proof.data(), tr.proof.size());
    return ZK_OK;
}

int zk_proof_finish(zk_ctx* ctx, zk_proof* pr_raw, void* h_proof, size_t proof_cap, size_t* proof_len) {
    if (!ctx) return ZK_ERR_INVALID_ARG;
    PoolScope pool_scope(ctx);
    std::unique_ptr<zk_proof> pr(pr_raw);
    ZK_REQUIRE(ctx, pr && h_proof && proof_len, "null pointer");
    if (pr->phase != pr->pk->num_phases) return ctx->fail(ZK_ERR_INVALID_ARG, "only %u of %u advice phases were committed", pr->phase, pr->pk->num_phases);
    host::Transcript& tr = pr->tr;
    Finish f(ctx, pr.get());
    AuxJoin aux_join{ctx, &f.late_cosets};
    f.lag.theta = tr.squeeze();
    PK_TRY(stage_late_advice_cosets(f));
    PK_TRY(stage_lookup_multiplicities(f));
    f.lag.beta = tr.squeeze();
    f.lag.gamma = tr.squeeze();
    PK_TRY(stage_permutation_products(f));
    PK_TRY(stage_lookup_grand_sums(f));
    PK_TRY(stage_vanishing_random(f));
    f.lag.y = tr.squeeze();
    PK_TRY(stage_coefficient_forms(f));
    PK_TRY(stage_quotient(f));
    PK_TRY(stage_h_commits(f));
    f.x = tr.squeeze();
    PK_TRY(stage_evaluations(f));
    PK_TRY(stage_h_recombination(f));
    stage_opening_queries(f);
    PK_TRY(pr->multiopen == ZK_MULTIOPEN_SHPLONK ? multiopen_shplonk(f) : multiopen_gwc(f));
    return write_proof_out(ctx, tr, h_proof, proof_cap, proof_len);
}

struct zk_transcript { host::Transcript tr; };
zk_transcript* zk_transcript_new(int kind) {
    if (kind != ZK_TRANSCRIPT_BLAKE2B && kind != ZK_TRANSCRIPT_POSEIDON && kind != ZK_TRANSCRIPT_EVM) return nullptr;
    zk_transcript* t = new (std::nothrow) zk_transcript();
    if (t) t->tr.reset(kind);
    return t;
}
void zk_transcript_free(zk_transcript* t) { delete t; }
static int transcript_status(zk_transcript* t) { const int e = t->tr.err; t->tr.err = 0; return e; }
int zk_transcript_common_point(zk_transcript* t, const void* affine64) {
    if (!t || !affine64) return ZK_ERR_INVALID_ARG;
    G1Affine p; memcpy((void*)&p, affine64, 64);
    t->tr.common_point(p);
    return transcript_status(t);
// ... 259 lines not shown
```

zkevm-circuits_amd/csrc/quotient.hip:

```cpp
#include "ctx.hpp"
#include "ff29.hip.hpp"
#include <unordered_map>

namespace zk {

using Q29 = F29<Fr29P>;

template <class P>
__host__ __device__ constexpr uint32_t kp_norm(int K, int idx) {
    uint64_t carry = 0;
    uint32_t out = 0;
    for (int i = 0; i <= idx; ++i) {
        const uint64_t v = (uint64_t)K * P::M(i) + carry;
        out = i < 8 ? (uint32_t)(v & MASK29) : (uint32_t)v;
        carry = v >> 29;
    }
    return out;
}
__device__ __forceinline__ Q29 q_settle(Q29 r) {
    normalize29(r);
    Q29 d;
    int32_t c = 0;
#pragma unroll
    for (int i = 0; i < 9; ++i) {
// ... 256 lines not shown
        d[i] = i < 8 ? ((uint32_t)s_ & MASK29) : (uint32_t)s_;
        c = s_ >> 29;
    }
    const bool neg_ = (int32_t)d[8] < 0;
#pragma unroll
    for (int i = 0; i < 9; ++i) r.l[i] = neg_ ? r.l[i] : d[i];
    q_settle_ip(r);
}

enum QClass : uint32_t {
    C_SPILL = 1u << 0,
    C_UNPACK_T = 1u << 1,
    C_UNPACK_B = 1u << 2,
    C_UNPACK_B32 = 1u << 3,
    C_POP_B = 1u << 4,
    C_HASMEM = 1u << 5,
    C_FLAGS = 1u << 6,
    C_MULV = 1u << 7,
    C_MULC = 1u << 8,
    C_ADDV = 1u << 9,
    C_SUBV = 1u << 10,
    C_FOLDC = 1u << 11,
    C_RARE = 1u << 12,
    C_PUSHC = 1u << 13,
    C_ADDC = 1u << 14,
    C_RSUB = 1u << 15,
    C_MULS = 1u << 16,
    C_NEG = 1u << 17, C_SQ = 1u << 18, C_DBL = 1u << 19, C_TEE = 1u << 20,
    C_FOLD = 1u << 21,
    C_MACC = 1u << 22,
    C_UNPACK_T32 = 1u << 23,
    C_MAC2 = 1u << 24,
    C_MACS = 1u << 25,
};
static uint32_t q_class_mask(uint32_t w0) {
    uint32_t m = 0;
    switch (w0 & 0xffu) {
        case Q_PUSH_COL: m = C_SPILL | C_UNPACK_T | C_HASMEM; break;
        case Q_PUSH_CONST: m = C_SPILL | C_RARE | C_PUSHC; break;
        case Q_ADD: m = C_POP_B | C_ADDV; break;
        case Q_SUB: m = C_POP_B | C_RARE | C_RSUB; break;
        case Q_MUL: m = C_POP_B | C_RARE | C_MULS; break;
        case Q_NEG: m = C_RARE | C_NEG; break;
        case Q_SQUARE: m = C_RARE | C_SQ; break;
        case Q_DOUBLE: m = C_RARE | C_DBL; break;
        case Q_FOLD: m = C_RARE | C_FOLD; break;
        case Q_MUL_CONST: m = C_MULC; break;
        case Q_ADD_CONST: m = C_RARE | C_ADDC; break;
        case Q_TEE_TMP: m = C_RARE | C_TEE; break;
        case K_ADD_COL: m = C_UNPACK_B | C_HASMEM | C_ADDV; break;
        case K_SUB_COL: m = C_UNPACK_B | C_HASMEM | C_SUBV; break;
        case K_RSUB_COL: m = C_UNPACK_B | C_HASMEM | C_RARE | C_RSUB; break;
        case K_MUL_COL: m = C_UNPACK_B32 | C_HASMEM | C_MULV; break;
        case K_FOLD_COL: m = C_UNPACK_B | C_HASMEM | C_FOLDC; break;
        case K_MAC_COL: m = C_UNPACK_B32 | C_HASMEM | C_MACC; break;
        case K_PUSH_COL32: return C_UNPACK_T32 | C_HASMEM;
        case K_MAC2_COL: m = C_UNPACK_B32 | C_HASMEM | C_MAC2; break;
        case K_MAC_STK: m = C_POP_B | C_RARE | C_MACS; break;
        default: break;
    }
    if (w0 & (K_SETTLE0 | K_SETTLE1 | K_NORM0 | K_NORM1 | K_SETTLE0_8 | K_SETTLE1_8)) m |= C_FLAGS;
    return m;
}

template <bool FULL, bool ACC_MEM>
__global__ void __launch_bounds__(Q_THREADS) Q_OCC_ATTR
k_quotient_eval2(const uint32_t* __restrict__ prog, uint32_t prog_len, const Fr* const* __restrict__ cols, const QC29* __restrict__ consts,
                 const QC29* __restrict__ consts_rp , const Fr* __restrict__ t_evals , uint32_t ext_k, uint32_t k,
                 Fr* __restrict__ out, Fr* tmp , uint32_t* acc_mem , uint32_t tile_alias ,
                 const uint32_t* __restrict__ slice_tab , uint32_t num_slices ) {
    extern __shared__ __attribute__((aligned(16))) uint32_t smem[];
    auto st_addr = [&](int slot) -> uint32_t {
        uint32_t a = (uint32_t)slot * (9u * Q_THREADS * 4u) + threadIdx.x * 4u;
        asm volatile("" : "+v"(a));
        return a;
    };
    auto st_put = [&](int slot, const Q29& v) {
        const uint32_t a = st_addr(slot);
#pragma unroll
        for (int q = 0; q < 9; ++q) *(uint32_t*)((char*)smem + a + q * (Q_THREADS * 4)) = v.l[q];
    };
    auto st_get = [&](int slot, Q29& v) {
        const uint32_t a = st_addr(slot);
#pragma unroll
        for (int q = 0; q < 9; ++q) v.l[q] = *(const uint32_t*)((const char*)smem + a + q * (Q_THREADS * 4));
    };
    const uint64_t ne = 1ull << ext_k;
    uint32_t blk = blockIdx.x;
    if (tile_alias) { const uint32_t xcd = blk & 7u, j = blk >> 3; blk = ((j >> tile_alias) << 3) | xcd; }
    if (num_slices) {
        const uint32_t xcd = blk & 7u, j = blk >> 3, sl = j % num_slices;
        blk = ((j / num_slices) << 3) | xcd;
        prog += slice_tab[2 * sl];
        prog_len = slice_tab[2 * sl + 1];
        out += (size_t)sl << ext_k;
    }
    const uint32_t i = blk * blockDim.x + threadIdx.x;
    const bool live = FULL || i < (uint32_t)ne;
    const uint32_t rot_scale = 1u << (ext_k - k), row_mask = (uint32_t)ne - 1u;
    Q29 t0, acc, B;
#pragma unroll
    for (int q = 0; q < 9; ++q) { t0.l[q] = 0; acc.l[q] = 0; B.l[q] = 0; }
    int sp = 0;
    typedef uint32_t U32x4 __attribute__((ext_vector_type(4)));
    using GU4 = const U32x4 __attribute__((address_space(1)));
    using GU1 = uint32_t __attribute__((address_space(1)));
    struct Raw { U32x4 lo, hi; };
    auto load = [&](uint32_t a, uint32_t b, Raw& r) {
        const uint32_t row = (i + b * rot_scale) & row_mask;
        if (FULL || live) {
            GU4* q = (GU4*)(uintptr_t)(cols[a] + row);
            r.lo = q[0]; r.hi = q[1];
        }
    };
    auto raw_fr = [](Raw& r) -> Fr {
        asm volatile("" : "+v"(r.lo), "+v"(r.hi));
        Fr x;
        x.l[0] = r.lo.x; x.l[1] = r.lo.y; x.l[2] = r.lo.z; x.l[3] = r.lo.w;
        x.l[4] = r.hi.x; x.l[5] = r.hi.y; x.l[6] = r.hi.z; x.l[7] = r.hi.w;
        return x;
    };
    auto cst = [&](const QC29* __restrict__ tab, uint32_t j) -> Q29 {
        Q29 r;
#pragma unroll
        for (int q = 0; q < 9; ++q) r.l[q] = tab[j].l[q];
        return r;
    };
    auto fold = [&](uint32_t w0_, const Q29& c, const Q29& v) {
        if (!ACC_MEM) {
            mul29_ub_ipa(acc, c);
#pragma unroll
            for (int q = 0; q < 9; ++q) acc.l[q] += v.l[q];
            return;
        }
        Q29 a;
#pragma unroll
        for (int q = 0; q < 9; ++q) a.l[q] = 0;
        uint32_t ii = i;
        asm volatile("" : "+v"(ii));
        GU1* qa = (GU1*)(uintptr_t)(acc_mem + ii);
        if (!(w0_ & K_FIRST_FOLD) && live) {
#pragma unroll
            for (int l = 0; l < 9; ++l) a.l[l] = qa[(uint64_t)l << ext_k];
        }
        mul29_ub_ipa(a, c);
        if (live) {
#pragma unroll
            for (int l = 0; l < 9; ++l) qa[(uint64_t)l << ext_k] = a.l[l] + v.l[l];
        }
    };
    uint32_t w0 = prog[0], w1 = prog[1], w2 = prog[2], w3 = prog[3];
    uint32_t n0 = prog[4], n1 = prog[5], n2 = prog[6], n3 = prog[7];
    Raw m;
    m.lo = U32x4{0, 0, 0, 0}; m.hi = U32x4{0, 0, 0, 0};
    if (w3 & C_HASMEM) load(w1, w2, m);
    for (uint32_t pc = 0; pc < prog_len; ++pc) {
        const uint32_t f0 = prog[4 * pc + 8], f1 = prog[4 * pc + 9], f2 = prog[4 * pc + 10], f3 = prog[4 * pc + 11];
        if ((w0 & 0xffu) == Q_END) break;
        if (w3 & C_SPILL) { if (sp >= 1) st_put(sp - 1, t0); ++sp; }
        if (w3 & C_UNPACK_T) q_unpack_to(t0, raw_fr(m));
        if (w3 & C_UNPACK_T32) {
            if (w0 & K_SETTLE0) q_settle_ip(t0);
            if (w0 & K_NORM0) normalize29(t0);
            if (w0 & K_SETTLE0_8) q_settle8_ip(t0);
            st_put(sp - 1, t0);
            ++sp;
            q_unpack_x32_to(t0, raw_fr(m));
        }
        if (w3 & C_UNPACK_B) q_unpack_to(B, raw_fr(m));
        if (w3 & C_UNPACK_B32) q_unpack_x32_to(B, raw_fr(m));
        if (w3 & C_POP_B) { st_get(sp - 2, B); --sp; }
        if (n3 & C_HASMEM) load(n1, n2, m);
        if (w3 & C_FLAGS) {
            if (w0 & K_SETTLE0) q_settle_ip(t0);
            if (w0 & K_SETTLE1) q_settle_ip(B);
            if (w0 & K_NORM0) normalize29(t0);
            if (w0 & K_NORM1) normalize29(B);
            if (w0 & K_SETTLE0_8) q_settle8_ip(t0);
            if (w0 & K_SETTLE1_8) q_settle8_ip(B);
        }
        if (w3 & C_MULV) mul29_ipa(t0, B);
        if (w3 & C_MULC) mul29_ub_ipa(t0, cst(consts_rp, w1));
        if (w3 & C_MACC) {
            Q29 S;
            st_get(sp - 2, S);
            --sp;
            mul2add29_ub_ipa(t0, B, S, cst(consts_rp, w0 >> K_CONST_SHIFT));
        }
        if (w3 & C_MAC2) {
            Q29 M1, X, S;
            st_get(sp - 2, M1);
            st_get(sp - 3, X);
            st_get(sp - 4, S);
            sp -= 3;
            mul3add29_ub_ipa(t0, B, X, M1, S, cst(consts_rp, w0 >> K_CONST_SHIFT));
        }
        if (w3 & C_ADDV) {
#pragma unroll
            for (int q = 0; q < 9; ++q) t0.l[q] += B.l[q];
        }
        if (w3 & C_SUBV) {
#pragma unroll
            for (int q = 0; q < 9; ++q) t0.l[q] = t0.l[q] + kp_balanced<Fr29P>(2, q) - B.l[q];
        }
        if (w3 & C_FOLDC) fold(w0, cst(consts_rp, w0 >> K_CONST_SHIFT), B);
        if (w3 & C_RARE) {
            if (w3 & C_PUSHC) {
                const Q29 c = cst(consts, w1);
#pragma unroll
                for (int q = 0; q < 9; ++q) t0.l[q] = c.l[q];
            }
            if (w3 & C_ADDC) {
                const Q29 c = cst(consts, w1);
#pragma unroll
                for (int q = 0; q < 9; ++q) t0.l[q] += c.l[q];
            }
            if (w3 & C_RSUB) {
#pragma unroll
                for (int q = 0; q < 9; ++q) t0.l[q] = B.l[q] + kp_balanced<Fr29P>(2, q) - t0.l[q];
                normalize29(t0);
            }
            if (w3 & C_MULS) { q_shl5_ip(t0); mul29_ipb(t0, B); }
            if (w3 & C_MACS) {
                Q29 S;
                st_get(sp - 2, S);
                --sp;
                q_shl5_ip(t0);
                mul2add29_ub_ipb(t0, B, S, cst(consts_rp, w0 >> K_CONST_SHIFT));
            }
            if (w3 & C_NEG) {
#pragma unroll
                for (int q = 0; q < 9; ++q) t0.l[q] = kp_balanced<Fr29P>(2, q) - t0.l[q];
                normalize29(t0);
            }
            if (w3 & C_SQ) { Q29 s2 = t0; q_shl5_ip(s2); mul29_ipa(t0, s2); }
            if (w3 & C_DBL) {
#pragma unroll
                for (int q = 0; q < 9; ++q) t0.l[q] <<= 1;
            }
            if (w3 & C_TEE) { if (live) stg(tmp + (((uint64_t)w1 << ext_k) + i), pack29_lt2p(t0)); }
            if (w3 & C_FOLD) { fold(w0, cst(consts_rp, w1), t0); --sp; if (sp >= 1) st_get(sp - 1, t0); }
        }
        w0 = n0; w1 = n1; w2 = n2; w3 = n3;
        n0 = f0; n1 = f1; n2 = f2; n3 = f3;
    }
    if (live) {
        Q29 a = acc;
        if (ACC_MEM) {
            GU1* qa = (GU1*)(uintptr_t)(acc_mem + i);
#pragma unroll
            for (int l = 0; l < 9; ++l) a.l[l] = qa[(uint64_t)l << ext_k];
        }
        if (t_evals) stg(out + i, pack29_lt2p(mul29(a, unpack29<Fr29P>(ldg(t_evals + (i & (rot_scale - 1u)))))));
        else { normalize29(a); stg(out + i, reduce_lazy29(a)); }
    }
}

struct LNode {
    enum Kind : uint8_t { MEM, CONST, UN, BIN, CONSTOP, TEE, MAT } kind;
    bool has_tee;
    bool is_tmp;
    uint32_t op, a, b;
    int32_t x, y;
};
struct LowInstr { uint32_t w0, a, b; };

static void lower_fuse(const uint32_t* prog, uint32_t len, uint32_t num_cols, std::vector<LowInstr>* out, bool mac = false, bool mac2 = false, uint32_t* declined = nullptr) {
    std::vector<LNode> nodes;
    nodes.reserve(len);
    std::vector<int32_t> st;
    auto leafish = [&](int32_t n) { return nodes[n].kind == LNode::MEM || nodes[n].kind == LNode::CONST; };
    std::vector<int16_t> du, net;
    du.reserve(len); net.reserve(len);
// ... 384 lines not shown
    if (!h_program || !out_instr || !out_depth) return ZK_ERR_INVALID_ARG;
    if (out_declined) *out_declined = 0;
    {
        int sp = 0;
        for (uint32_t pc = 0; pc < num_instr && h_program[3 * pc] != Q_END; ++pc) {
            const uint32_t op = h_program[3 * pc];
            if (op == Q_PUSH_COL || op == Q_PUSH_CONST || op == Q_PUSH_TMP) ++sp;
            else if (op == Q_ADD || op == Q_SUB || op == Q_MUL) { if (sp < 2) return ZK_ERR_INVALID_ARG; --sp; }
            else if (op == Q_FOLD) { if (sp < 1) return ZK_ERR_INVALID_ARG; --sp; }
            else if (op == Q_NEG || op == Q_SQUARE || op == Q_DOUBLE || op == Q_MUL_CONST || op == Q_ADD_CONST || op == Q_TEE_TMP) { if (sp < 1) return ZK_ERR_INVALID_ARG; }
            else return ZK_ERR_INVALID_ARG;
        }
    }
    std::vector<LowInstr> low;
    if (fuse) lower_fuse(h_program, num_instr, num_cols, &low, (fuse & 2) != 0, (fuse & 6) == 6, out_declined);
    else
        for (uint32_t pc = 0; pc < num_instr && h_program[3 * pc] != Q_END; ++pc) {
            const uint32_t op = h_program[3 * pc], a_ = h_program[3 * pc + 1], b_ = h_program[3 * pc + 2];
            if (op == Q_PUSH_TMP) low.push_back({Q_PUSH_COL, num_cols + a_, 0});
            else low.push_back({op, a_, b_});
        }
    int depth = 0;
    if (lower_bounds(&low, num_cols, &depth)) return ZK_ERR_INVALID_ARG;
    *out_instr = (uint32_t)low.size();
    *out_depth = depth;
    if (out_words) {
        if (cap_words < low.size() * 3) return ZK_ERR_INVALID_ARG;
        for (size_t i = 0; i < low.size(); ++i) { out_words[3 * i] = low[i].w0; out_words[3 * i + 1] = low[i].a; out_words[3 * i + 2] = low[i].b; }
    }
    return ZK_OK;
}

struct SlicePlan { std::vector<uint32_t> cut; };
static bool plan_slices(const uint32_t* prog, uint32_t len, uint32_t ext_k, SlicePlan* out) {
    const int knob = getenv("ZK_QUOTIENT_SLICES") ? atoi(getenv("ZK_QUOTIENT_SLICES")) : -1;
    if (knob == 0 || (knob < 0 && (len < 2048 || ext_k < 16)) || ext_k < 11) return false;
    std::vector<uint32_t> bpos;
    std::vector<uint64_t> bcost;
    std::vector<int32_t> blocked(len + 2, 0);
    std::vector<uint32_t> last_tee;
    std::vector<uint64_t> ops;
    std::vector<uint32_t> colset;
    uint64_t cost = 0, reads = 0;
    int sp = 0;
    uint32_t n = 0;
    for (; n < len && prog[3 * n] != Q_END; ++n) {
        const uint32_t op = prog[3 * n], a = prog[3 * n + 1];
        switch (op) {
            case Q_PUSH_COL: ++sp; cost += 3; ++reads; ops.push_back(((uint64_t)a << 32) | prog[3 * n + 2]); colset.push_back(a); break;
            case Q_PUSH_CONST: ++sp; cost += 1; break;
            case Q_PUSH_TMP:
                ++sp; cost += 3;
                if (a < last_tee.size()) { ++blocked[last_tee[a] + 1]; --blocked[n + 1]; }
                break;
            case Q_TEE_TMP: if (a >= last_tee.size()) last_tee.resize(a + 1, 0); last_tee[a] = n; cost += 4; break;
            case Q_ADD: case Q_SUB: --sp; cost += 1; break;
            case Q_MUL: --sp; cost += 24; break;
            case Q_SQUARE: case Q_MUL_CONST: cost += 24; break;
            case Q_FOLD: --sp; cost += 24; if (sp == 0) { bpos.push_back(n + 1); bcost.push_back(cost); } break;
            default: cost += 1; break;
        }
    }
    if (bpos.size() < 2 || bpos.back() != n) return false;
    std::sort(ops.begin(), ops.end()); ops.erase(std::unique(ops.begin(), ops.end()), ops.end());
    std::sort(colset.begin(), colset.end()); colset.erase(std::unique(colset.begin(), colset.end()), colset.end());
    if (knob < 0 && reads < 4 * ops.size()) return false;
    const uint64_t rows_in_flight = std::min<uint64_t>(1ull << ext_k, 327680);
    const uint64_t ws = colset.size() * 32ull * rows_in_flight;
    uint32_t want = knob > 0 ? (uint32_t)knob : (uint32_t)std::min<uint64_t>(64, (ws + (96ull << 20) - 1) / (96ull << 20));
    if (want < 2) return false;
    std::vector<char> ok(bpos.size(), 1);
    {
        int32_t run = 0;
        size_t b = 0;
        for (uint32_t q = 0; q <= n && b < bpos.size(); ++q) {
            run += blocked[q];
            if (bpos[b] == q) { ok[b] = run == 0; ++b; }
        }
    }
    out->cut.assign(1, 0);
    uint32_t made = 1;
    for (size_t b = 0; b + 1 < bpos.size() && made < want; ++b) {
        if (!ok[b]) continue;
        if (bcost[b] * want >= cost * made) { out->cut.push_back(bpos[b]); ++made; }
    }
    out->cut.push_back(n);
    return out->cut.size() > 2;
}

extern "C" int zk_host_quotient_slices(const uint32_t* program, uint32_t num_instr, uint32_t ext_k, uint32_t* out_cuts, size_t cap, uint32_t* out_count) {
    if (!program || !out_count) return ZK_ERR_INVALID_ARG;
    SlicePlan plan;
    *out_count = 0;
    if (!plan_slices(program, num_instr, ext_k, &plan)) return ZK_OK;
    *out_count = (uint32_t)plan.cut.size();
    if (out_cuts) {
        if (cap < plan.cut.size()) return ZK_ERR_INVALID_ARG;
        for (size_t i = 0; i < plan.cut.size(); ++i) out_cuts[i] = plan.cut[i];
    }
    return ZK_OK;
}

extern "C" int zk_quotient_eval(zk_ctx* ctx, const uint32_t* h_program, uint32_t num_instr, const void* const* h_col_ptrs, uint32_t num_cols,
                                const void* h_consts, uint32_t num_consts, uint32_t k, uint32_t ext_k, int divide_by_vanishing, void* d_out) {
    if (!ctx) return ZK_ERR_INVALID_ARG;
    ZK_REQUIRE(ctx, h_program && d_out && (h_col_ptrs || !num_cols) && (h_consts || !num_consts), "null pointer");
    ZK_REQUIRE(ctx, k <= ext_k && ext_k <= 28, "need k <= ext_k <= 28");
    int depth = 0;
    uint32_t num_tmp = 0;
    int rc = validate_program(ctx, h_program, num_instr, num_cols, num_consts, &depth, &num_tmp);
    if (rc) return rc;
    const int kernel_knob = getenv("ZK_QUOTIENT_KERNEL") ? atoi(getenv("ZK_QUOTIENT_KERNEL")) : 2;
    const bool v2 = kernel_knob != 1;
    const int mac_level = getenv("ZK_QUOTIENT_MAC") ? atoi(getenv("ZK_QUOTIENT_MAC")) : 2;
    const bool mac = v2 && mac_level != 0, mac2 = mac && mac_level != 1;
    const uint64_t ne = 1ull << ext_k;
    SlicePlan plan;
    const bool sliced = v2 && ((ne / Q_THREADS) & 7) == 0 && plan_slices(h_program, num_instr, ext_k, &plan);
    const uint32_t S = sliced ? (uint32_t)plan.cut.size() - 1 : 1;
    std::vector<std::vector<LowInstr>> lows(S);
    std::vector<Fr> slice_k;
    if (sliced) {
        uint32_t next_slot = 0;
        int dmax = 0;
        slice_k.assign(S, Fr::one());
        for (uint32_t sl = 0; sl < S; ++sl) {
            std::vector<uint32_t> sub(h_program + 3 * plan.cut[sl], h_program + 3 * plan.cut[sl + 1]);
            std::unordered_map<uint32_t, uint32_t> slot_of;
            int spd = 0;
            for (size_t q = 0; q < sub.size() / 3; ++q) {
                const uint32_t op = sub[3 * q];
                if (op == Q_TEE_TMP || op == Q_PUSH_TMP) {
                    auto it = slot_of.find(sub[3 * q + 1]);
                    if (it == slot_of.end()) {
                        if (op == Q_PUSH_TMP) return ctx->fail(ZK_ERR_INVALID_ARG, "quotient program: slice %u reads an intermediate parked outside it", sl);
                        it = slot_of.emplace(sub[3 * q + 1], next_slot++).first;
                    }
                    sub[3 * q + 1] = it->second;
                }
                if (op == Q_PUSH_COL || op == Q_PUSH_CONST || op == Q_PUSH_TMP) ++spd;
                else if (op == Q_ADD || op == Q_SUB || op == Q_MUL) --spd;
                else if (op == Q_FOLD) { --spd; slice_k[sl] = slice_k[sl] * ((const Fr*)h_consts)[sub[3 * q + 1]]; }
            }
            sub.push_back(Q_END); sub.push_back(0); sub.push_back(0);
            lower_fuse(sub.data(), (uint32_t)(sub.size() / 3), num_cols, &lows[sl], mac, mac2);
            int dsl = 0;
            if (lower_bounds(&lows[sl], num_cols, &dsl)) return ctx->fail(ZK_ERR_INVALID_ARG, "quotient program: lowering failed");
            dmax = std::max(dmax, dsl);
        }
        depth = dmax;
        num_tmp = next_slot;
    } else {
        std::vector<LowInstr>& low = lows[0];
        const char* env = getenv("ZK_QUOTIENT_FUSE");
        if (env && atoi(env) == 0) {
            for (uint32_t pc = 0; pc < num_instr && h_program[3 * pc] != Q_END; ++pc) {
                const uint32_t op = h_program[3 * pc], a_ = h_program[3 * pc + 1], b_ = h_program[3 * pc + 2];
                if (op == Q_PUSH_TMP) low.push_back({Q_PUSH_COL, num_cols + a_, 0});
                else low.push_back({op, a_, b_});
            }
        } else lower_fuse(h_program, num_instr, num_cols, &low, mac, mac2);
        if (lower_bounds(&low, num_cols, &depth)) return ctx->fail(ZK_ERR_INVALID_ARG, "quotient program: lowering failed");
    }
    if (depth > Q_MAX_STACK) return ctx->fail(ZK_ERR_UNSUPPORTED, "quotient program: stack deeper than %d", Q_MAX_STACK);
    if (depth < 1) depth = 1;
    Fr* d_tmp = nullptr;
    if (num_tmp) {
        d_tmp = (Fr*)ctx->get_scratch(SC_QTMP, ((size_t)num_tmp << ext_k) * sizeof(Fr));
        if (!d_tmp) return ZK_ERR_OOM;
    }
    uint32_t low_len = 0;
    uint32_t folds = 0;
    for (std::vector<LowInstr>& low : lows) {
        bool first = true;
        for (LowInstr& in : low) {
            const uint32_t o = in.w0 & 0xffu;
            if (o == Q_FOLD || o == K_FOLD_COL) { if (first) in.w0 |= K_FIRST_FOLD; first = false; ++folds; }
        }
        low_len += (uint32_t)low.size();
    }
    static const int acc_knob = getenv("ZK_QUOTIENT_ACC_MEM") ? atoi(getenv("ZK_QUOTIENT_ACC_MEM")) : -1;
    const bool acc_in_mem = !sliced && folds > 0 && (acc_knob < 0 ? (uint64_t)folds * 16 <= low_len : acc_knob == 1);
    uint32_t* d_acc = nullptr;
    if (acc_in_mem) {
        d_acc = (uint32_t*)ctx->get_scratch(SC_QACC, ((size_t)9 << ext_k) * sizeof(uint32_t));
        if (!d_acc) return ZK_ERR_OOM;
    }
    Fr* d_part = nullptr;
    if (sliced) {
        d_part = (Fr*)ctx->get_scratch(SC_QSLICE, ((size_t)S << ext_k) * sizeof(Fr));
        if (!d_part) return ZK_ERR_OOM;
    }
    if (getenv("ZK_QUOTIENT_TRACE") && low_len >= 64) {
        static const char* names[26] = {"END", "PUSH_COL", "PUSH_CONST", "ADD", "SUB", "MUL", "NEG", "SQUARE", "DOUBLE", "FOLD", "MUL_CONST", "ADD_CONST", "TEE_TMP", "PUSH_TMP", "?", "?",
                                        "ADD_COL", "SUB_COL", "RSUB_COL", "MUL_COL", "FOLD_COL", "NOP", "MAC_COL", "PUSH_COL32", "MAC2_COL", "MAC_STK"};
        uint32_t hist[26] = {0}, settles = 0, norms = 0;
        for (const std::vector<LowInstr>& low : lows) for (const LowInstr& in : low) { const uint32_t o = in.w0 & 0xffu; if (o < 26) ++hist[o]; settles += ((in.w0 & (K_SETTLE0 | K_SETTLE0_8)) ? 1 : 0) + ((in.w0 & (K_SETTLE1 | K_SETTLE1_8)) ? 1 : 0); norms += ((in.w0 & K_NORM0) ? 1 : 0) + ((in.w0 & K_NORM1) ? 1 : 0); }
        fprintf(stderr, "[zk quotient] 2^%u rows, %u lowered instructions%s, depth %d, %u settles, %u carry propagations:", ext_k, low_len, sliced ? (" in " + std::to_string(S) + " slices").c_str() : "", depth, settles, norms);
        for (int o = 0; o < 26; ++o) if (hist[o]) fprintf(stderr, " %s %u", names[o], hist[o]);
        if (sliced) { fprintf(stderr, "; slice lengths"); for (const std::vector<LowInstr>& low : lows) fprintf(stderr, " %zu", low.size()); fprintf(stderr, "; %u parking slots", num_tmp); }
        fprintf(stderr, "\n");
    }
    std::vector<Fr> tev;
    if (divide_by_vanishing) vanishing_inverses(k, ext_k, &tev);
    auto times32 = [](Fr x) { for (int j = 0; j < 5; ++j) x = dbl(x); return x; };
    std::vector<Fr> consts_r((const Fr*)h_consts, (const Fr*)h_consts + num_consts);
    if (sliced) consts_r.insert(consts_r.end(), slice_k.begin(), slice_k.end());
    const uint32_t nc_all = (uint32_t)consts_r.size();
    std::vector<Fr> consts_rp(consts_r);
    for (Fr& c : consts_rp) c = times32(c);
    for (Fr& t : tev) t = times32(t);
    std::vector<const void*> col_tab(h_col_ptrs, h_col_ptrs + num_cols);
    for (uint32_t t = 0; t < num_tmp; ++t) col_tab.push_back(d_tmp + ((size_t)t << ext_k));
    std::vector<LowInstr> comb;
    if (sliced) {
        if (nc_all >= (1u << (32 - K_CONST_SHIFT))) return ctx->fail(ZK_ERR_UNSUPPORTED, "quotient program: too many constants for a sliced launch");
        for (uint32_t sl = 0; sl < S; ++sl) {
            col_tab.push_back(d_part + ((size_t)sl << ext_k));
            comb.push_back({K_FOLD_COL | ((num_consts + sl) << K_CONST_SHIFT) | (sl ? 0u : K_FIRST_FOLD), num_cols + num_tmp + sl, 0});
        }
    }
    const size_t prog_bytes = (size_t)(low_len + 4 * S + comb.size() + 4) * (v2 ? 16 : 12) + (sliced ? S * 8 : 0), col_bytes = (col_tab.size() ? col_tab.size() : 1) * 8;
    const size_t const_bytes = (size_t)(nc_all ? nc_all : 1) * sizeof(QC29) * 2, tev_bytes = tev.size() * sizeof(Fr);
    auto al = [](size_t x) { return (x + 255) & ~(size_t)255; };
    char* d = (char*)ctx->get_scratch(SC_POLY, al(prog_bytes) + al(col_bytes) + al(const_bytes) + al(tev_bytes) + 256);
    if (!d) return ZK_ERR_OOM;
    uint32_t* d_prog = (uint32_t*)d;
    const Fr** d_cols = (const Fr**)(d + al(prog_bytes));
    QC29* d_consts = (QC29*)(d + al(prog_bytes) + al(col_bytes));
    Fr* d_tev = (Fr*)(d + al(prog_bytes) + al(col_bytes) + al(const_bytes));
    const size_t total_bytes = al(prog_bytes) + al(col_bytes) + al(const_bytes) + al(tev_bytes);
    std::vector<char> staging(total_bytes, 0);
    std::vector<uint32_t> slice_tab(2 * S);
    size_t slice_tab_at = 0, comb_at = 0;
    {
        uint32_t* hp = (uint32_t*)staging.data();
        size_t w = 0;
        for (uint32_t sl = 0; sl < S; ++sl) {
            slice_tab[2 * sl] = (uint32_t)w; slice_tab[2 * sl + 1] = (uint32_t)lows[sl].size() + 1;
            for (const LowInstr& in : lows[sl]) { hp[w++] = in.w0; hp[w++] = in.a; hp[w++] = in.b; if (v2) hp[w++] = q_class_mask(in.w0); }
            for (int e = 0; e < 4; ++e) { hp[w++] = Q_END; hp[w++] = 0; hp[w++] = 0; if (v2) hp[w++] = 0; }
        }
        comb_at = w;
        if (sliced) {
            for (const LowInstr& in : comb) { hp[w++] = in.w0; hp[w++] = in.a; hp[w++] = in.b; hp[w++] = q_class_mask(in.w0); }
            for (int e = 0; e < 4; ++e) { hp[w++] = Q_END; hp[w++] = 0; hp[w++] = 0; hp[w++] = 0; }
        }
        slice_tab_at = w;
        if (sliced) for (uint32_t q = 0; q < 2 * S; ++q) hp[w++] = slice_tab[q];
        if (!col_tab.empty()) memcpy(staging.data() + al(prog_bytes), col_tab.data(), col_tab.size() * 8);
        char* hc = staging.data() + al(prog_bytes) + al(col_bytes);
        QC29* hq = (QC29*)hc;
        for (uint32_t j = 0; j < nc_all; ++j) {
            const Q29 a = unpack29<Fr29P>(consts_r[j]), b = unpack29<Fr29P>(consts_rp[j]);
            for (int q = 0; q < 9; ++q) { hq[j].l[q] = a.l[q]; hq[nc_all + j].l[q] = b.l[q]; }
        }
        if (!tev.empty()) memcpy(staging.data() + al(prog_bytes) + al(col_bytes) + al(const_bytes), tev.data(), tev_bytes);
    }
    ZK_HIP(ctx, hipMemcpyAsync(d, staging.data(), total_bytes, hipMemcpyHostToDevice, ctx->stream));
    ZK_HIP(ctx, hipStreamSynchronize(ctx->stream));
    size_t lds = (size_t)(v2 ? (depth > 1 ? depth - 1 : 1) : (depth > 2 ? depth - 2 : 1)) * 9 * Q_THREADS * 4;
    {
        static const long pad = getenv("ZK_QUOTIENT_LDS_PAD") ? atol(getenv("ZK_QUOTIENT_LDS_PAD")) : 0;
        if (pad > 0 && (size_t)pad > lds && (size_t)pad <= (size_t)Q_MAX_STACK * 9 * Q_THREADS * 4) lds = (size_t)pad;
    }
    if (!ctx->quotient_attr_set) {
        const int lds_max = Q_MAX_STACK * 9 * Q_THREADS * 4;
        ZK_HIP(ctx, hipFuncSetAttribute((const void*)k_quotient_eval<true, false>, hipFuncAttributeMaxDynamicSharedMemorySize, lds_max));
        ZK_HIP(ctx, hipFuncSetAttribute((const void*)k_quotient_eval<false, false>, hipFuncAttributeMaxDynamicSharedMemorySize, lds_max));
        ZK_HIP(ctx, hipFuncSetAttribute((const void*)k_quotient_eval<true, true>, hipFuncAttributeMaxDynamicSharedMemorySize, lds_max));
        ZK_HIP(ctx, hipFuncSetAttribute((const void*)k_quotient_eval<false, true>, hipFuncAttributeMaxDynamicSharedMemorySize, lds_max));
        ZK_HIP(ctx, hipFuncSetAttribute((const void*)k_quotient_eval2<true, false>, hipFuncAttributeMaxDynamicSharedMemorySize, lds_max));
        ZK_HIP(ctx, hipFuncSetAttribute((const void*)k_quotient_eval2<false, false>, hipFuncAttributeMaxDynamicSharedMemorySize, lds_max));
        ZK_HIP(ctx, hipFuncSetAttribute((const void*)k_quotient_eval2<true, true>, hipFuncAttributeMaxDynamicSharedMemorySize, lds_max));
        ZK_HIP(ctx, hipFuncSetAttribute((const void*)k_quotient_eval2<false, true>, hipFuncAttributeMaxDynamicSharedMemorySize, lds_max));
        ctx->quotient_attr_set = true;
    }
    ZkProfScope ps(ctx, ctx->prof_tag ? ctx->prof_tag : "quotient_eval");
    if (ctx->prof_on) {
        std::vector<uint64_t> ops;
        uint64_t tmp_moves = 0;
        for (uint32_t i = 0; i < num_instr; ++i) {
            const uint32_t op = h_program[3 * i];
            if (op == Q_PUSH_COL) ops.push_back(((uint64_t)h_program[3 * i + 1] << 32) | h_program[3 * i + 2]);
            else if (op == Q_TEE_TMP || op == Q_PUSH_TMP) ++tmp_moves;
        }
        std::sort(ops.begin(), ops.end());
        ops.erase(std::unique(ops.begin(), ops.end()), ops.end());
        ps.bytes = (ops.size() + tmp_moves + 1) * ne * 32;
    }
    {
        const dim3 grid((unsigned)((ne + Q_THREADS - 1) / Q_THREADS) * S), block(Q_THREADS);
        const bool full = ne >= (uint64_t)Q_THREADS;
        auto launch = [&](auto kern) {
            hipLaunchKernelGGL(kern, grid, block, lds, ctx->stream, (const uint32_t*)d_prog, low_len + 1, (const Fr* const*)d_cols, (const QC29*)d_consts, (const QC29*)(d_consts + nc_all),
                               tev.empty() ? (const Fr*)nullptr : (const Fr*)d_tev, ext_k, k, (Fr*)d_out, d_tmp, d_acc);
        };
        static const uint32_t tile_alias = getenv("ZK_QUOTIENT_TILE_ALIAS") ? (uint32_t)atoi(getenv("ZK_QUOTIENT_TILE_ALIAS")) : 0;
        auto launch2 = [&](auto kern) {
            hipLaunchKernelGGL(kern, grid, block, lds, ctx->stream, (const uint32_t*)d_prog, low_len + 1, (const Fr* const*)d_cols, (const QC29*)d_consts, (const QC29*)(d_consts + nc_all),
                               tev.empty() || sliced ? (const Fr*)nullptr : (const Fr*)d_tev, ext_k, k, sliced ? d_part : (Fr*)d_out, d_tmp, d_acc, sliced ? 0u : tile_alias,
                               (const uint32_t*)d_prog + slice_tab_at, sliced ? S : 0u);
        };
        if (v2 && full && acc_in_mem) launch2(k_quotient_eval2<true, true>);
        else if (v2 && full) launch2(k_quotient_eval2<true, false>);
        else if (v2 && acc_in_mem) launch2(k_quotient_eval2<false, true>);
        else if (v2) launch2(k_quotient_eval2<false, false>);
        else if (full && acc_in_mem) launch(k_quotient_eval<true, true>);
        else if (full) launch(k_quotient_eval<true, false>);
        else if (acc_in_mem) launch(k_quotient_eval<false, true>);
        else launch(k_quotient_eval<false, false>);
    }
    ZK_CHECK_LAUNCH(ctx);
    if (sliced) {
        const dim3 grid((unsigned)((ne + Q_THREADS - 1) / Q_THREADS)), block(Q_THREADS);
        hipLaunchKernelGGL((k_quotient_eval2<true, false>), grid, block, (size_t)9 * Q_THREADS * 4, ctx->stream, (const uint32_t*)d_prog + comb_at, S + 1, (const Fr* const*)d_cols, (const QC29*)d_consts,
                           (const QC29*)(d_consts + nc_all), tev.empty() ? (const Fr*)nullptr : (const Fr*)d_tev, ext_k, k, (Fr*)d_out, d_tmp, (uint32_t*)nullptr, 0u, (const uint32_t*)nullptr, 0u);
        ZK_CHECK_LAUNCH(ctx);
    }
    return ZK_OK;
}

namespace zk { __global__ void k_powers(Fr base, Fr mul, Fr* out, uint32_t count, int rprime); }

extern "C" int zk_fr_powers(zk_ctx* ctx, const void* h_base, const void* h_mul, void* d_out, size_t n) {
    if (!ctx) return ZK_ERR_INVALID_ARG;
    ZK_REQUIRE(ctx, h_base && h_mul && d_out, "null pointer");
    ZK_REQUIRE(ctx, n <= (1ull << 28), "too many powers");
    if (!n) return ZK_OK;
    hipLaunchKernelGGL(zk::k_powers, dim3((unsigned)((n + 255) / 256)), dim3(256), 0, ctx->stream, *(const Fr*)h_base, *(const Fr*)h_mul, (Fr*)d_out, (uint32_t)n, 0);
    ZK_CHECK_LAUNCH(ctx);
    return ZK_OK;
}
```

Baseline: 1.837.

## Store coset columns as pre-unpacked 29-bit limb records for quotient evaluation

Adds a record output format: the NTT last pass, the powers kernel and the quotient temporaries write values already converted to nine 29-bit limbs (8 in the Fr slot plus a ninth limb in a side array, 36 bytes per row). Quotient evaluation gets a templated variant that reads these records directly, so the per-operand unpacking from 32-bit Montgomery form is skipped. It is enabled by default for k in 2..26 and can be turned off through an environment variable. In exchange, every buffer is larger and needs more memory traffic, the coset cache and its byte accounting change, and more kernel instantiations are added.

```diff
diff --git a/zkevm-circuits_amd/csrc/api.hip b/zkevm-circuits_amd/csrc/api.hip
--- a/zkevm-circuits_amd/csrc/api.hip
+++ b/zkevm-circuits_amd/csrc/api.hip
@@ -88,6 +88,7 @@
     (void)hipStreamSynchronize(ctx->stream);
     ctx->domains.clear();
     for (auto& kv : ctx->pow_tables) (void)hipFree(kv.second);
+    for (auto& kv : ctx->loop_records) (void)hipFree(kv.second);
     ctx->pool_trim();
     ctx->prof_resolve();
     for (auto e : ctx->prof_pool) (void)hipEventDestroy(e);
@@ -349,7 +350,7 @@
     ZK_REQUIRE(ctx, h_g, "null pointer");
     ZK_REQUIRE(ctx, k <= 28, "k exceeds the two-adicity of Fr (28)");
     for (size_t i = 0; i < count; ++i) ZK_REQUIRE(ctx, d_coeffs[i] && d_outs[i], "null column pointer");
-    return ntt_run_many(ctx, (Fr* const*)d_outs, (const Fr* const*)d_coeffs, count, k, fr_root_of_unity(k), nullptr, (const Fr*)h_g, nullptr, true);
+    return coeff_to_coset_batch_fmt(ctx, d_coeffs, k, *(const Fr*)h_g, d_outs, count, false);
 }
 int zk_extended_to_coeff(zk_ctx* ctx, void* d_ext, uint32_t ext_k) {
     if (!ctx) return ZK_ERR_INVALID_ARG;
diff --git a/zkevm-circuits_amd/csrc/ctx.hpp b/zkevm-circuits_amd/csrc/ctx.hpp
--- a/zkevm-circuits_amd/csrc/ctx.hpp
+++ b/zkevm-circuits_amd/csrc/ctx.hpp
@@ -58,6 +58,7 @@
     uint32_t comm_rank = 0, comm_world = 1;
     std::map<uint64_t, std::shared_ptr<zk::NttDomain>> domains;
     std::map<uint64_t, void*> pow_tables;
+    std::map<const void*, void*> loop_records;
     std::vector<void*> pinned;
     std::map<size_t, std::vector<void*>> pool;
     size_t pool_bytes = 0, pool_cap = (size_t)96 << 30;
@@ -199,6 +200,12 @@
             const Fr* d_src = nullptr ,
             bool fuse_pre = false );
 int ntt_run_many(zk_ctx* ctx, Fr* const* d_datas, const Fr* const* d_srcs, size_t count, uint32_t log_n, const Fr& omega, const Fr* scale, const Fr* coset_pre, const Fr* coset_post, bool fuse_pre);
+int ntt_run_many_fmt(zk_ctx* ctx, Fr* const* d_datas, const Fr* const* d_srcs, size_t count, uint32_t log_n, const Fr& omega, const Fr* scale, const Fr* coset_pre, const Fr* coset_post, bool fuse_pre,
+                     bool records);
+int coeff_to_coset_batch_fmt(zk_ctx* ctx, const void* const* d_coeffs, uint32_t k, const Fr& g, void* const* d_outs, size_t count, bool records);
+int fr_powers_fmt(zk_ctx* ctx, const Fr& base, const Fr& mul, void* d_out, size_t n, bool records);
+int quotient_eval_fmt(zk_ctx* ctx, const uint32_t* h_program, uint32_t num_instr, const void* const* h_col_ptrs, uint32_t num_cols, const void* h_consts, uint32_t num_consts, uint32_t k, uint32_t ext_k,
+                      int divide_by_vanishing, void* d_out, bool records);
 int fr_scale_run(zk_ctx* ctx, Fr* d_a, const Fr& s, uint64_t n);
 enum G1Enc : int { G1_ENC_COMPRESSED = 0, G1_ENC_RAW = 1, G1_ENC_BE_XY = 2 };
 int g1_decode_run(zk_ctx* ctx, const void* d_in, int enc, G1Affine* d_out, uint64_t n, uint32_t* d_bad, uint8_t* d_bad_at);
diff --git a/zkevm-circuits_amd/csrc/ff29.hip.hpp b/zkevm-circuits_amd/csrc/ff29.hip.hpp
--- a/zkevm-circuits_amd/csrc/ff29.hip.hpp
+++ b/zkevm-circuits_amd/csrc/ff29.hip.hpp
@@ -410,7 +410,7 @@
 }
 
 template <class P>
-__host__ __device__ __forceinline__ Fp<typename P::P32> reduce_lazy29(const F29<P>& x) {
+__host__ __device__ __forceinline__ F29<P> reduce_lazy29_limbs(const F29<P>& x) {
     constexpr uint64_t mhi = ((uint64_t)P::P32::M(7) << 32) | P::P32::M(6);
     constexpr uint32_t C = (uint32_t)((((unsigned __int128)1) << 92) / ((unsigned __int128)mhi + 1));
     const uint32_t q = (uint32_t)(((uint64_t)x.l[8] * C) >> 52);
@@ -422,8 +422,48 @@
         r.l[i] = i < 8 ? (uint32_t)(s_ & MASK29) : (uint32_t)s_;
         c = s_ >> 29;
     }
-    return pack29_lt2p(r);
-}
+    return r;
+}
+template <class P>
+__host__ __device__ __forceinline__ Fp<typename P::P32> reduce_lazy29(const F29<P>& x) { return pack29_lt2p(reduce_lazy29_limbs(x)); }
+
+#ifndef ZK_REC29_AOS
+#define ZK_REC29_AOS 0
+#endif
+constexpr size_t REC29_BYTES = 36;
+template <class P>
+__host__ __device__ __forceinline__ F29<P> canon29_lt2p(const F29<P>& a) {
+    F29<P> d;
+    int32_t c = 0;
+#pragma unroll
+    for (int i = 0; i < 9; ++i) {
+        const int32_t s_ = (int32_t)a.l[i] - (int32_t)P::M(i) + c;
+        d.l[i] = i < 8 ? ((uint32_t)s_ & MASK29) : (uint32_t)s_;
+        c = s_ >> 29;
+    }
+    const bool neg_ = (int32_t)d.l[8] < 0;
+    F29<P> r;
+#pragma unroll
+    for (int i = 0; i < 9; ++i) r.l[i] = neg_ ? a.l[i] : d.l[i];
+    return r;
+}
+#if defined(__HIPCC__)
+template <class P>
+__device__ __forceinline__ void rec29_store(Fp<typename P::P32>* base, uint64_t n, uint64_t idx, const F29<P>& v) {
+#if ZK_REC29_AOS
+    typedef uint32_t U4A __attribute__((ext_vector_type(4), aligned(4)));
+    char* p = reinterpret_cast<char*>(base) + idx * REC29_BYTES;
+    *reinterpret_cast<U4A*>(p) = U4A{v.l[0], v.l[1], v.l[2], v.l[3]};
+    *reinterpret_cast<U4A*>(p + 16) = U4A{v.l[4], v.l[5], v.l[6], v.l[7]};
+    *reinterpret_cast<uint32_t*>(p + 32) = v.l[8];
+#else
+    uint4* q = reinterpret_cast<uint4*>(base + idx);
+    q[0] = make_uint4(v.l[0], v.l[1], v.l[2], v.l[3]);
+    q[1] = make_uint4(v.l[4], v.l[5], v.l[6], v.l[7]);
+    reinterpret_cast<uint32_t*>(base + n)[idx] = v.l[8];
+#endif
+}
+#endif
 
 template <class P>
 __host__ __device__ __forceinline__ F29<P> sqr29_c(const F29<P>& a) {
diff --git a/zkevm-circuits_amd/csrc/ntt.hip b/zkevm-circuits_amd/csrc/ntt.hip
--- a/zkevm-circuits_amd/csrc/ntt.hip
+++ b/zkevm-circuits_amd/csrc/ntt.hip
@@ -77,7 +77,8 @@
         b = sqr(b);
         e >>= 1;
     }
-    stg(out + j, rprime ? to_rprime(r) : r);
+    if (rprime == 2) rec29_store<Fr29P>(out, count, j, unpack29<Fr29P>(to_rprime(r)));
+    else stg(out + j, rprime ? to_rprime(r) : r);
 }
 
 __device__ __forceinline__ Fr two_level(const Fr* __restrict__ lo, const Fr* __restrict__ hi, int h, uint32_t e) {
@@ -267,14 +268,14 @@
 }
 
 __host__ __device__ __forceinline__ int ntt_row_pad(int log_np) { return log_np >= 8 ? 8 : 0; }
-template <int R, bool FIRST, bool LAST, Opt PRE, Opt FOLDED>
+template <int R, bool FIRST, bool LAST, Opt PRE, Opt FOLDED, Opt REC>
 __device__ __forceinline__ void ntt_last_step(const Lds29& L, const Fr* __restrict__ src, Fr* __restrict__ dst, const Tw29* __restrict__ tw, const Fr* __restrict__ pre,
                                               const Fr29& fin29, const bool fin_folded, const int log_np, const int s, const int log_t, const int row,
-                                              const uint32_t blk, const uint32_t mid, const int log_mid, const int log_n1) {
+                                              const uint32_t blk, const uint32_t mid, const int log_mid, const int log_n1, const bool records) {
     static_assert(R == 2 || FIRST, "only the first step of a pass can be radix 2");
     constexpr int NE = 1 << R;
     const int hgt = 1 << s, T = 1 << log_t, items = (1 << (log_np + log_t)) >> R;
-    const bool has_pre = opt_on<PRE>(pre != nullptr), folded = opt_on<FOLDED>(fin_folded);
+    const bool has_pre = opt_on<PRE>(pre != nullptr), folded = opt_on<FOLDED>(fin_folded), rec = opt_on<REC>(records);
     for (int it = threadIdx.x; it < items; it += blockDim.x) {
         int c, b;
         if (LAST) { c = it & (T - 1); b = it >> log_t; }
@@ -306,8 +307,11 @@
 #pragma unroll
         for (int k = 0; k < NE; ++k) {
             const int dl = lo_d + k * hgt;
-            if (LAST) stg(dst + (i1 + (((uint64_t)mid + ((uint64_t)dl << log_mid)) << log_n1)), folded ? reduce_lazy29(e[k]) : pack29_lt2p(mul29(e[k], fin29)));
-            else L.store(c * row + dl, e[k]);
+            if (LAST) {
+                const uint64_t oi = i1 + (((uint64_t)mid + ((uint64_t)dl << log_mid)) << log_n1);
+                if (rec) rec29_store<Fr29P>(dst, 1ull << (log_np + log_mid + log_n1), oi, canon29_lt2p(folded ? reduce_lazy29_limbs(e[k]) : mul29(e[k], fin29)));
+                else stg(dst + oi, folded ? reduce_lazy29(e[k]) : pack29_lt2p(mul29(e[k], fin29)));
+            } else L.store(c * row + dl, e[k]);
         }
     }
 }
@@ -317,7 +321,7 @@
 }
 
 __global__ void __launch_bounds__(NTT_THREADS)
-k_ntt_last(NttIo io, const Tw29* __restrict__ tw, int log_np, int log_t, int log_n1, int log_mid, Fr fin, const Fr* __restrict__ pre, int fin_folded, int xcd_remap) {
+k_ntt_last(NttIo io, const Tw29* __restrict__ tw, int log_np, int log_t, int log_n1, int log_mid, Fr fin, const Fr* __restrict__ pre, int fin_folded, int xcd_remap, int records) {
     extern __shared__ __attribute__((aligned(16))) uint32_t smem[];
     const Fr* __restrict__ src = io.src[blockIdx.y];
     Fr* __restrict__ dst = io.dst[blockIdx.y];
@@ -329,7 +333,7 @@
         const int r = ((log_np - s) & 1) ? 1 : 2;
         const bool last = s + r == log_np;
         auto step = [&](auto R, auto FIRST, auto LAST) {
-            ntt_last_step<decltype(R)::value, decltype(FIRST)::value, decltype(LAST)::value, OPT_RUNTIME, OPT_RUNTIME>(L, src, dst, tw, pre, fin29, fin_folded != 0, log_np, s, log_t, row, blk, mid, log_mid, log_n1);
+            ntt_last_step<decltype(R)::value, decltype(FIRST)::value, decltype(LAST)::value, OPT_RUNTIME, OPT_RUNTIME, OPT_RUNTIME>(L, src, dst, tw, pre, fin29, fin_folded != 0, log_np, s, log_t, row, blk, mid, log_mid, log_n1, records != 0);
         };
         if (s == 0 && last) { if (r == 1) step(Int<1>{}, Bool<true>{}, Bool<true>{}); else step(Int<2>{}, Bool<true>{}, Bool<true>{}); }
         else if (s == 0) { if (r == 1) step(Int<1>{}, Bool<true>{}, Bool<false>{}); else step(Int<2>{}, Bool<true>{}, Bool<false>{}); }
@@ -339,24 +343,24 @@
         if (s < log_np) __syncthreads();
     }
 }
-template <int LOG_NP, int S>
+template <int LOG_NP, int S, bool REC>
 __device__ __forceinline__ void ntt_last_steps(const Lds29& L, const Fr* __restrict__ src, Fr* __restrict__ dst, const Tw29* __restrict__ tw,
                                                const int log_t, const int row, const uint32_t blk, const uint32_t mid, const int log_mid, const int log_n1) {
     constexpr int R = ((LOG_NP - S) & 1) ? 1 : 2;
     constexpr bool LAST = S + R == LOG_NP;
-    ntt_last_step<R, S == 0, LAST, OPT_NO, OPT_YES>(L, src, dst, tw, nullptr, Fr29{}, true, LOG_NP, S, log_t, row, blk, mid, log_mid, log_n1);
+    ntt_last_step<R, S == 0, LAST, OPT_NO, OPT_YES, REC ? OPT_YES : OPT_NO>(L, src, dst, tw, nullptr, Fr29{}, true, LOG_NP, S, log_t, row, blk, mid, log_mid, log_n1, REC);
     if constexpr (!LAST) {
         __syncthreads();
-        ntt_last_steps<LOG_NP, S + R>(L, src, dst, tw, log_t, row, blk, mid, log_mid, log_n1);
-    }
-}
-template <int LOG_NP>
+        ntt_last_steps<LOG_NP, S + R, REC>(L, src, dst, tw, log_t, row, blk, mid, log_mid, log_n1);
+    }
+}
+template <int LOG_NP, bool REC>
 __global__ void __launch_bounds__(NTT_THREADS)
-k_ntt_last_f(NttIo io, const Tw29* __restrict__ tw, int , int log_t, int log_n1, int log_mid, Fr fin, const Fr* __restrict__ pre, int fin_folded, int xcd_remap) {
+k_ntt_last_f(NttIo io, const Tw29* __restrict__ tw, int , int log_t, int log_n1, int log_mid, Fr fin, const Fr* __restrict__ pre, int fin_folded, int xcd_remap, int ) {
     extern __shared__ __attribute__((aligned(16))) uint32_t smem[];
     const int row = (1 << LOG_NP) + ntt_row_pad(LOG_NP);
     const uint32_t bx = last_tile(xcd_remap), mid = bx & ((1u << log_mid) - 1), blk = bx >> log_mid;
-    ntt_last_steps<LOG_NP, 0>(Lds29{smem, row << log_t}, io.src[blockIdx.y], io.dst[blockIdx.y], tw, log_t, row, blk, mid, log_mid, log_n1);
+    ntt_last_steps<LOG_NP, 0, REC>(Lds29{smem, row << log_t}, io.src[blockIdx.y], io.dst[blockIdx.y], tw, log_t, row, blk, mid, log_mid, log_n1);
 }
 
 __global__ void k_scale(Fr* a, Fr s, uint64_t n) {
@@ -583,12 +587,12 @@
         default: return pre ? k_ntt_pass_f<10, true> : k_ntt_pass_f<10, false>;
     }
 }
-static LastKernel last_instance(int log_np) {
+static LastKernel last_instance(int log_np, bool rec) {
     switch (log_np) {
-        case 7: return k_ntt_last_f<7>;
-        case 8: return k_ntt_last_f<8>;
-        case 9: return k_ntt_last_f<9>;
-        default: return k_ntt_last_f<10>;
+        case 7: return rec ? k_ntt_last_f<7, true> : k_ntt_last_f<7, false>;
+        case 8: return rec ? k_ntt_last_f<8, true> : k_ntt_last_f<8, false>;
+        case 9: return rec ? k_ntt_last_f<9, true> : k_ntt_last_f<9, false>;
+        default: return rec ? k_ntt_last_f<10, true> : k_ntt_last_f<10, false>;
     }
 }
 static int launch_pass(zk_ctx* ctx, const NttDomain& dom, int p, size_t nb, const NttKnobs& kn, const NttIo& io, const Fr* pre) {
@@ -610,11 +614,11 @@
     ZK_CHECK_LAUNCH(ctx);
     return ZK_OK;
 }
-static int launch_last(zk_ctx* ctx, const NttDomain& dom, size_t nb, const NttKnobs& kn, const NttIo& io, const Fr* pre) {
+static int launch_last(zk_ctx* ctx, const NttDomain& dom, size_t nb, const NttKnobs& kn, const NttIo& io, const Fr* pre, bool records) {
     const int P = dom.npass;
     const NttPass& ps = dom.pass[P - 1];
     NttPlan pl = plan_last(dom, nb, kn);
-    LastKernel kernel = pl.fixed ? last_instance(ps.log_np) : k_ntt_last;
+    LastKernel kernel = pl.fixed ? last_instance(ps.log_np, records) : k_ntt_last;
     if (pl.fixed && !pass_kernel_ready(ctx, (const void*)kernel, NTT_LAST_MAX_LDS)) {
         NttKnobs generic = kn;
         generic.fixed = false;
@@ -625,7 +629,7 @@
     ZkProfScope pscope(ctx, "ntt_last");
     pscope.bytes = (uint64_t)nb * (1ull << dom.log_n) * 64 / (uint64_t)P;
     hipLaunchKernelGGL(kernel, pl.grid, dim3(pl.threads), pl.lds, ctx->stream, io, ps.tw, ps.log_np, pl.log_t, P == 1 ? 0 : dom.pass[0].log_np, P == 3 ? dom.pass[1].log_np : 0,
-                       dom.final_mul, pre, dom.fin_folded ? 1 : 0, pl.xcd);
+                       dom.final_mul, pre, dom.fin_folded ? 1 : 0, pl.xcd, records ? 1 : 0);
     ZK_CHECK_LAUNCH(ctx);
     return ZK_OK;
 }
@@ -642,7 +646,15 @@
     return ntt_run_many(ctx, &d_data, d_src ? &d_src : nullptr, 1, log_n, omega, scale, coset_pre, coset_post, fuse_pre);
 }
 int ntt_run_many(zk_ctx* ctx, Fr* const* d_datas, const Fr* const* d_srcs, size_t count, uint32_t log_n, const Fr& omega, const Fr* scale, const Fr* coset_pre, const Fr* coset_post, bool fuse_pre) {
+    return ntt_run_many_fmt(ctx, d_datas, d_srcs, count, log_n, omega, scale, coset_pre, coset_post, fuse_pre, false);
+}
+int ntt_run_many_fmt(zk_ctx* ctx, Fr* const* d_datas, const Fr* const* d_srcs, size_t count, uint32_t log_n, const Fr& omega, const Fr* scale, const Fr* coset_pre, const Fr* coset_post, bool fuse_pre,
+                     bool records) {
     if (count == 0) return ZK_OK;
+    if (records) {
+        if (coset_post || log_n == 0 || !d_srcs) return ctx->fail(ZK_ERR_INVALID_ARG, "NTT: record output needs a source of its own, one row at least and no pass behind the transform");
+        for (size_t i = 0; i < count; ++i) if (!d_srcs[i] || d_srcs[i] == d_datas[i]) return ctx->fail(ZK_ERR_INVALID_ARG, "NTT: record output in place");
+    }
     const NttKnobs kn = read_ntt_knobs();
     if (log_n == 0) {
         for (size_t i = 0; i < count; ++i) {
@@ -690,11 +702,16 @@
             for (size_t j = 0; j < nb; ++j) io.src[j] = io.dst[j];
         }
         for (size_t j = 0; j < nb; ++j) io.dst[j] = d_datas[first + j];
-        rc = launch_last(ctx, *dom, nb, kn, io, P == 1 ? pre_table : nullptr);
+        rc = launch_last(ctx, *dom, nb, kn, io, P == 1 ? pre_table : nullptr, records);
         if (rc) return rc;
         if (coset_post) for (size_t j = 0; j < nb; ++j) { rc = run_distribute(ctx, log_n, *coset_post, io.dst[j], io.dst[j]); if (rc) return rc; }
     }
     return ZK_OK;
+}
+
+int coeff_to_coset_batch_fmt(zk_ctx* ctx, const void* const* d_coeffs, uint32_t k, const Fr& g, void* const* d_outs, size_t count, bool records) {
+    const Fr s32 = fr_from_u64(32);
+    return ntt_run_many_fmt(ctx, (Fr* const*)d_outs, (const Fr* const*)d_coeffs, count, k, fr_root_of_unity(k), records ? &s32 : nullptr, &g, nullptr, true, records);
 }
 
 template <int W>
diff --git a/zkevm-circuits_amd/csrc/prover.hip b/zkevm-circuits_amd/csrc/prover.hip
--- a/zkevm-circuits_amd/csrc/prover.hip
+++ b/zkevm-circuits_amd/csrc/prover.hip
@@ -11,6 +11,7 @@
 #include <tuple>
 #include <functional>
 #include "ctx.hpp"
+#include "ff29.hip.hpp"
 #include "host_hash.hpp"
 #include "cs.hpp"
 #include "quotient_plan.hpp"
@@ -104,6 +105,7 @@
     mutable std::vector<std::unordered_map<uint32_t, DevBuf>> part_cache;
     mutable int part_cache_state = -1;
     mutable size_t part_cache_bytes = 0;
+    mutable bool part_cache_records = false;
     std::vector<G1Affine> fixed_com, sigma_com;
     F4 vk_repr;
     const zk_srs* srs = nullptr;
@@ -118,6 +120,7 @@
     std::vector<std::vector<DevBuf>> adv_coset;
     std::vector<uint32_t> pre_mask;
     bool pre_planned = false;
+    int coset_fmt = -1;
     uint32_t phase = 0;
     int multiopen = ZK_MULTIOPEN_GWC;
     int vanishing_random = ZK_VANISHING_ONE;
@@ -153,6 +156,17 @@
     if (!got) { (void)hipGetLastError(); free_b = 0; }
     if (ok) *ok = got;
     return free_b;
+}
+
+bool quotient_records(uint32_t k) {
+    const char* r = getenv("ZK_QUOTIENT_RECORDS");
+    const char* q = getenv("ZK_QUOTIENT_KERNEL");
+    return !(r && atoi(r) == 0) && !(q && atoi(q) == 1) && k >= 2 && k <= 26;
+}
+size_t coset_row_bytes(bool records) { return records ? REC29_BYTES : sizeof(Fr); }
+bool session_records(zk_proof* pr) {
+    if (pr->coset_fmt < 0) pr->coset_fmt = quotient_records(pr->pk->k) ? 1 : 0;
+    return pr->coset_fmt == 1;
 }
 
 struct PairOwners {
@@ -283,15 +297,15 @@
     }
     return ZK_OK;
 }
-int run_program(zk_ctx* ctx, const Env& e, const Prog& g, void* d_out) {
+int run_program(zk_ctx* ctx, const Env& e, const Prog& g, void* d_out, bool records = false) {
     Concrete c;
     PK_TRY(concretise(ctx, e, g, &c));
     {
         static const int alias = getenv("ZK_QUOTIENT_ALIAS") ? atoi(getenv("ZK_QUOTIENT_ALIAS")) : 0;
         if (alias > 0 && ctx->prof_tag && !strcmp(ctx->prof_tag, "quotient_coset")) for (size_t i = 0; i < c.cols.size(); ++i) c.cols[i] = c.cols[i % (size_t)alias];
     }
-    return zk_quotient_eval(ctx, c.words.data(), (uint32_t)(c.words.size() / 3), c.cols.data(), (uint32_t)c.cols.size(),
-                            c.consts.empty() ? nullptr : c.consts.data(), (uint32_t)c.consts.size(), e.pk->k, e.pk->k, 0, d_out);
+    return quotient_eval_fmt(ctx, c.words.data(), (uint32_t)(c.words.size() / 3), c.cols.data(), (uint32_t)c.cols.size(),
+                             c.consts.empty() ? nullptr : c.consts.data(), (uint32_t)c.consts.size(), e.pk->k, e.pk->k, 0, d_out, records);
 }
 const Fr* coeff_of(const zk_pk* pk, uint32_t ref, const std::vector<DevBuf>& adv, const std::vector<DevBuf>& inst, const std::vector<DevBuf>& pz,
                    const std::vector<DevBuf>& lkm, const std::vector<DevBuf>& lkphi) {
@@ -863,14 +877,14 @@
                     const uint32_t gc = col[c_];
                     if (!(pr->pre_mask[gc] >> r & 1u)) continue;
                     DevBuf& slot = pr->adv_coset[r][gc];
-                    if (!slot.alloc(n_ * 32)) {
+                    if (!slot.alloc(n_ * coset_row_bytes(session_records(pr)))) {
                         for (uint32_t& m_ : pr->pre_mask) m_ = 0;
                         break;
                     }
                     csrc.push_back(coeff[c_]->p);
                     cdst.push_back(slot.p);
                 }
-                if (!csrc.empty()) PK_TRY(zk_coeff_to_coset_batch(ctx, csrc.data(), pk->k, &g_of_r[r], cdst.data(), csrc.size()));
+                if (!csrc.empty()) PK_TRY(coeff_to_coset_batch_fmt(ctx, csrc.data(), pk->k, g_of_r[r], cdst.data(), csrc.size(), session_records(pr)));
             }
             pending.clear();
             return ZK_OK;
@@ -1112,13 +1126,15 @@
     const uint32_t E = pk->ext_k - pk->k, R = 1u << E;
     if (E > 5) return ZK_OK;
     const double col_bytes = (double)((size_t)1 << pk->k) * 32.0;
+    const double coset_bytes = (double)((size_t)1 << pk->k) * (double)coset_row_bytes(session_records(pr));
     bool mem_known = false;
     const size_t free_b = device_free_bytes(&mem_known);
     if (!mem_known) return ZK_OK;
-    const double cols_ahead = (pr->advice_in_place ? 1.0 : 2.0) * pk->A + 3.0 * (2.0 * pk->L + pk->C) + (2.0 * pk->L + pk->C + pk->I + 8.0) + 2.0 * R + 32.0;
-    double avail = (double)free_b + (double)ctx->pool_bytes - cols_ahead * col_bytes - 16.0 * (double)(1ull << 30);
+    const double cols_ahead = (pr->advice_in_place ? 1.0 : 2.0) * pk->A + 3.0 * (2.0 * pk->L + pk->C) + 2.0 * R + 32.0, cosets_ahead = 2.0 * pk->L + pk->C + pk->I + 8.0;
+    const double reserve = cols_ahead * col_bytes + cosets_ahead * coset_bytes;
+    double avail = (double)free_b + (double)ctx->pool_bytes - reserve - 16.0 * (double)(1ull << 30);
     if (pk->part_cache_state < 0 || (pk->part_cache_state == 1 && pk->part_cache_bytes == 0)) {
-        const double key_need = (double)key_slots * col_bytes;
+        const double key_need = (double)key_slots * coset_bytes;
         const char* kenv = getenv("ZK_PK_COSET_CACHE_GB");
         const double kcap = std::min((kenv ? atof(kenv) : 96.0) * (double)(1ull << 30), (double)ctx->prop.totalGlobalMem / 3.0);
         if (key_need <= kcap) avail -= std::max(0.0, key_need - (double)pk->part_cache_bytes);
@@ -1130,13 +1146,13 @@
     for (const auto& cr : by_count) {
         uint32_t rest = 0;
         for (uint32_t m_ : mask) rest += (m_ & ~(chosen | 1u << cr.second)) != 0;
-        if (used + cr.first * col_bytes > cap || used + (cr.first + rest) * col_bytes > avail) break;
-        used += cr.first * col_bytes;
+        if (used + cr.first * coset_bytes > cap || used + (cr.first + rest) * coset_bytes > avail) break;
+        used += cr.first * coset_bytes;
         chosen |= 1u << cr.second;
     }
     if (getenv("ZK_PROVER_TRACE")) {
         fprintf(stderr, "[zk prover] advice coset plan: free %.1f + pooled %.1f GiB, reserve %.1f GiB, budget %.1f GiB, cosets by columns served:", free_b / 1073741824.0, ctx->pool_bytes / 1073741824.0,
-                (cols_ahead * col_bytes) / 1073741824.0 + 16.0, budget / 1073741824.0);
+                reserve / 1073741824.0 + 16.0, budget / 1073741824.0);
         for (const auto& cr : by_count) fprintf(stderr, " r%u:%u", cr.second, cr.first);
         fprintf(stderr, " -> chosen 0x%x\n", chosen);
     }
@@ -1172,6 +1188,7 @@
     const bool shard_args;
     std::vector<uint32_t> act;
     bool late_cosets = false;
+    bool records = false;
     std::vector<std::vector<DevBuf>> lk_f;
     std::vector<DevBuf> lk_t, lk_m, lk_phi;
     std::vector<uint8_t> same_table;
@@ -1219,7 +1236,7 @@
     size_t key_slots = 0;
     PK_TRY(advice_coset_plan(ctx, pk, mask, &key_slots));
     if (pr->adv_coset.empty()) { pr->adv_coset.resize(R); for (auto& v : pr->adv_coset) v.resize(pk->A); }
-    const double col_bytes = (double)n * 32.0;
+    const double col_bytes = (double)n * (double)coset_row_bytes(f.records);
     const size_t free_b = device_free_bytes();
     double avail = (double)free_b + (double)ctx->pool_bytes - (4.0 * (2.0 * pk->L + pk->C) + (2.0 * pk->L + pk->C + pk->I + 8.0) + 2.0 * R + 32.0) * col_bytes - 24.0 * (double)(1ull << 30);
     if (pk->part_cache_state < 0 || (pk->part_cache_state == 1 && pk->part_cache_bytes == 0)) avail -= (double)key_slots * col_bytes;
@@ -1239,7 +1256,7 @@
         for (uint32_t c = 0; c < pk->A && ok; ++c) {
             if (!todo(cr.second, c)) continue;
             DevBuf& slot = pr->adv_coset[cr.second][c];
-            if (!slot.alloc(n * 32)) { ok = false; break; }
+            if (!slot.alloc(n * coset_row_bytes(f.records))) { ok = false; break; }
             csrc.push_back(pr->adv_coeff[c].p);
             cdst.push_back(slot.p);
         }
@@ -1249,7 +1266,7 @@
         }
         ctx->stream = ctx->stream_aux;
         f.late_cosets = true;
-        if (!csrc.empty()) PK_TRY(zk_coeff_to_coset_batch(ctx, csrc.data(), f.k, &g, cdst.data(), csrc.size()));
+        if (!csrc.empty()) PK_TRY(coeff_to_coset_batch_fmt(ctx, csrc.data(), f.k, g, cdst.data(), csrc.size(), f.records));
         ctx->stream = main_stream;
         used += csrc.size() * col_bytes;
         if (!ok) break;
@@ -1587,8 +1604,9 @@
     double budget = (env ? atof(env) : 96.0) * (double)(1ull << 30);
     budget = std::min(budget, (double)ctx->prop.totalGlobalMem / 3.0) - (double)ctx->coset_cache_bytes;
     const size_t free_b = device_free_bytes();
-    const double need = (double)key_slots * n * 32.0;
-    const double session = (double)refs.size() * n * 32.0 + (double)((size_t)n << q.E) * 32.0 * 2.0;
+    const double row = (double)coset_row_bytes(f.records);
+    const double need = (double)key_slots * n * row;
+    const double session = (double)refs.size() * n * row + (double)((size_t)n << q.E) * 32.0 * 2.0;
     pk->part_cache_state = (need <= budget && need + session <= (double)free_b + (double)ctx->pool_bytes) ? 1 : 0;
     if (pk->part_cache_state) pk->part_cache.resize(q.nparts);
 }
@@ -1632,6 +1650,7 @@
     std::vector<DevBuf>& bufs = cp.part_buf;
     const bool cache_on = cp.cache_on;
     const uint32_t k = f.k;
+    const size_t coset_bytes = n * coset_row_bytes(f.records);
     const Fr w_n = fr_root_of_unity(k);
     auto pre_coset = [&](uint32_t ref, uint32_t r) -> const void* {
         if ((ref >> 24) != CT_ADVICE || r >= pr->adv_coset.size()) return nullptr;
@@ -1651,7 +1670,7 @@
         for (uint32_t e : w.active) needed |= q.reads(e, refs[i]);
         if (!needed) continue;
         if (const void* pre = pre_coset(refs[i], r_)) { w.part_of[refs[i]] = pre; continue; }
-        if (!(cache_on && key_column(refs[i])) && !bufs[i].p) PK_ALLOC(ctx, bufs[i], n * 32);
+        if (!(cache_on && key_column(refs[i])) && !bufs[i].p) PK_ALLOC(ctx, bufs[i], coset_bytes);
         void* dst = bufs[i].p;
         DevBuf fresh;
         const bool cached = cache_on && key_column(refs[i]);
@@ -1659,22 +1678,22 @@
             auto it = pk->part_cache[r_].find(refs[i]);
             if (it != pk->part_cache[r_].end()) { w.part_of[refs[i]] = it->second.p; continue; }
             const char* env_fail = getenv("ZK_PK_COSET_CACHE_FAIL_AFTER");
-            const bool inject = env_fail && pk->part_cache_bytes / (n * 32) + fresh_slots.size() >= (size_t)atoll(env_fail);
-            bool got = pk->part_cache_state == 1 && !inject && fresh.alloc_unpooled(n * 32);
+            const bool inject = env_fail && pk->part_cache_bytes / coset_bytes + fresh_slots.size() >= (size_t)atoll(env_fail);
+            bool got = pk->part_cache_state == 1 && !inject && fresh.alloc_unpooled(coset_bytes);
             if (!got && pk->part_cache_state == 1) {
                 (void)hipGetLastError();
                 ctx->pool_trim();
-                got = !inject && fresh.alloc_unpooled(n * 32);
+                got = !inject && fresh.alloc_unpooled(coset_bytes);
                 if (!got) { (void)hipGetLastError(); pk->part_cache_state = 2; }
             }
             if (got) dst = fresh.p;
             else {
-                if (!bufs[i].p) PK_ALLOC(ctx, bufs[i], n * 32);
+                if (!bufs[i].p) PK_ALLOC(ctx, bufs[i], coset_bytes);
                 dst = bufs[i].p;
             }
         }
         w.part_of[refs[i]] = dst;
-        if (refs[i] == colref(CT_SPECIAL, SP_X)) PK_TRY(zk_fr_powers(ctx, &w_n, &w.g, dst, n));
+        if (refs[i] == colref(CT_SPECIAL, SP_X)) PK_TRY(fr_powers_fmt(ctx, w_n, w.g, dst, n, f.records));
         else {
             const Fr* cf = (refs[i] >> 24) == CT_SPLIT_R ? ((refs[i] & 0xFFFFFFu) < f.rem_coeff.size() ? f.rem_coeff[refs[i] & 0xFFFFFFu].fr() : nullptr)
                                                          : coeff_of(pk, refs[i], pr->adv_coeff, pr->inst_coeff, f.pz_coeff, f.m_coeff, f.phi_coeff);
@@ -1684,10 +1703,10 @@
         }
         if (cached && fresh.p) fresh_slots.emplace_back(refs[i], std::move(fresh));
     }
-    PK_TRY(zk_coeff_to_coset_batch(ctx, bat_src.data(), k, &w.g, bat_dst.data(), bat_src.size()));
+    PK_TRY(coeff_to_coset_batch_fmt(ctx, bat_src.data(), k, w.g, bat_dst.data(), bat_src.size(), f.records));
     for (auto& fs : fresh_slots) {
-        pk->part_cache_bytes += n * 32;
-        ctx->coset_cache_bytes += n * 32;
+        pk->part_cache_bytes += coset_bytes;
+        ctx->coset_cache_bytes += coset_bytes;
         pk->part_cache[r_][fs.first] = std::move(fs.second);
     }
     return ZK_OK;
@@ -1705,16 +1724,17 @@
     part.part = &w.part_of;
     Fr gn = w.g;
     for (uint32_t i = 0; i < k; ++i) gn = sqr(gn);
-    const Fr vinv = fr_inv_host(gn - Fr::one());
+    const Fr vinv = fr_inv_host(gn - Fr::one()), inv32 = fr_inv_host(fr_from_u64(32));
     for (uint32_t e : w.active) {
         ctx->prof_tag = "quotient_coset";
-        const int rc_q = run_program(ctx, part, q.cls(e).prog, hpart.p);
+        const int rc_q = run_program(ctx, part, q.cls(e).prog, hpart.p, f.records);
         ctx->prof_tag = nullptr;
         PK_TRY(rc_q);
         const F4 yp = host::fr_pow(f.lag.y, K - 1 - q.cls(e).last);
         Fr scale;
         memcpy((void*)&scale, yp.l, 32);
         scale = scale * vinv;
+        if (f.records) scale = scale * inv32;
         if (sharded) {
             PK_TRY(zk_fr_scale(ctx, hpart.p, &scale, n));
             DevBuf keep;
@@ -1767,12 +1787,27 @@
     return ZK_OK;
 }
 
+static int key_cache_format(Finish& f) {
+    zk_ctx* ctx = f.ctx; const zk_pk* pk = f.pk;
+    if (pk->part_cache_records == f.records) return ZK_OK;
+    if (pk->part_cache_bytes || !pk->part_cache.empty()) {
+        ZK_HIP(ctx, hipStreamSynchronize(ctx->stream));
+        pk->part_cache.clear();
+        ctx->coset_cache_bytes -= std::min(ctx->coset_cache_bytes, pk->part_cache_bytes);
+        pk->part_cache_bytes = 0;
+    }
+    pk->part_cache_state = -1;
+    pk->part_cache_records = f.records;
+    return ZK_OK;
+}
+
 static int stage_quotient(Finish& f) {
     zk_ctx* ctx = f.ctx;
     Quotient q;
     PK_TRY(quotient_prepare(f, q));
     {
         CosetPass cp;
+        PK_TRY(key_cache_format(f));
         if (f.pk->part_cache_state < 0) quotient_decide_key_cache(f, q);
         cp.cache_on = f.pk->part_cache_state >= 1;
         cp.part_buf.resize(q.plan->refs.size());
@@ -2064,6 +2099,18 @@
     return ZK_OK;
 }
 
+static int finish_coset_format(Finish& f) {
+    zk_proof* pr = f.pr;
+    f.records = quotient_records(f.k);
+    if (pr->coset_fmt >= 0 && (pr->coset_fmt == 1) != f.records) {
+        ZK_HIP(f.ctx, hipDeviceSynchronize());
+        pr->adv_coset.clear();
+        for (uint32_t& m_ : pr->pre_mask) m_ = 0;
+    }
+    pr->coset_fmt = f.records ? 1 : 0;
+    return ZK_OK;
+}
+
 int zk_proof_finish(zk_ctx* ctx, zk_proof* pr_raw, void* h_proof, size_t proof_cap, size_t* proof_len) {
     if (!ctx) return ZK_ERR_INVALID_ARG;
     PoolScope pool_scope(ctx);
@@ -2074,6 +2121,7 @@
     Finish f(ctx, pr.get());
     AuxJoin aux_join{ctx, &f.late_cosets};
     f.lag.theta = tr.squeeze();
+    PK_TRY(finish_coset_format(f));
     PK_TRY(stage_late_advice_cosets(f));
     PK_TRY(stage_lookup_multiplicities(f));
     f.lag.beta = tr.squeeze();
diff --git a/zkevm-circuits_amd/csrc/quotient.hip b/zkevm-circuits_amd/csrc/quotient.hip
--- a/zkevm-circuits_amd/csrc/quotient.hip
+++ b/zkevm-circuits_amd/csrc/quotient.hip
@@ -312,9 +312,16 @@
     C_UNPACK_T32 = 1u << 23,
     C_MAC2 = 1u << 24,
     C_MACS = 1u << 25,
+    C_ADDM = 1u << 26,
+    C_SUBM = 1u << 27,
 };
-static uint32_t q_class_mask(uint32_t w0) {
+static uint32_t q_class_mask(uint32_t w0, bool records = false) {
     uint32_t m = 0;
+    if (records && ((w0 & 0xffu) == K_ADD_COL || (w0 & 0xffu) == K_SUB_COL)) {
+        m = C_HASMEM | ((w0 & 0xffu) == K_ADD_COL ? C_ADDM : C_SUBM);
+        if (w0 & (K_SETTLE0 | K_SETTLE1 | K_NORM0 | K_NORM1 | K_SETTLE0_8 | K_SETTLE1_8)) m |= C_FLAGS;
+        return m;
+    }
     switch (w0 & 0xffu) {
         case Q_PUSH_COL: m = C_SPILL | C_UNPACK_T | C_HASMEM; break;
         case Q_PUSH_CONST: m = C_SPILL | C_RARE | C_PUSHC; break;
@@ -343,7 +350,7 @@
     return m;
 }
 
-template <bool FULL, bool ACC_MEM>
+template <bool FULL, bool ACC_MEM, bool REC>
 __global__ void __launch_bounds__(Q_THREADS) Q_OCC_ATTR
 k_quotient_eval2(const uint32_t* __restrict__ prog, uint32_t prog_len, const Fr* const* __restrict__ cols, const QC29* __restrict__ consts,
                  const QC29* __restrict__ consts_rp , const Fr* __restrict__ t_evals , uint32_t ext_k, uint32_t k,
@@ -375,6 +382,7 @@
         prog_len = slice_tab[2 * sl + 1];
         out += (size_t)sl << ext_k;
     }
+    prog_len = __builtin_amdgcn_readfirstlane(prog_len);
     const uint32_t i = blk * blockDim.x + threadIdx.x;
     const bool live = FULL || i < (uint32_t)ne;
     const uint32_t rot_scale = 1u << (ext_k - k), row_mask = (uint32_t)ne - 1u;
@@ -385,13 +393,34 @@
     typedef uint32_t U32x4 __attribute__((ext_vector_type(4)));
     using GU4 = const U32x4 __attribute__((address_space(1)));
     using GU1 = uint32_t __attribute__((address_space(1)));
-    struct Raw { U32x4 lo, hi; };
+    struct Raw { U32x4 lo, hi; uint32_t top; };
     auto load = [&](uint32_t a, uint32_t b, Raw& r) {
         const uint32_t row = (i + b * rot_scale) & row_mask;
         if (FULL || live) {
-            GU4* q = (GU4*)(uintptr_t)(cols[a] + row);
-            r.lo = q[0]; r.hi = q[1];
-        }
+            const Fr* col = cols[a];
+            if (REC && ZK_REC29_AOS) {
+                typedef U32x4 U32x4A __attribute__((aligned(4)));
+                using GU4A = const U32x4A __attribute__((address_space(1)));
+                const char* p = (const char*)col + (size_t)row * REC29_BYTES;
+                r.lo = *(GU4A*)(uintptr_t)p; r.hi = *(GU4A*)(uintptr_t)(p + 16);
+                r.top = *(const GU1*)(uintptr_t)(p + 32);
+            } else if (REC) {
+                using GC = const char __attribute__((address_space(1)));
+                GC* base = (GC*)(uintptr_t)col;
+                GC* p = base + (uint32_t)(row << 5);
+                r.lo = *(GU4*)p; r.hi = *(GU4*)(p + 16);
+                r.top = *(const GU1*)(base + (ne << 5) + (uint32_t)(row << 2));
+            } else {
+                GU4* q = (GU4*)(uintptr_t)(col + row);
+                r.lo = q[0]; r.hi = q[1];
+            }
+        }
+    };
+    auto raw_limbs = [](Q29& d, Raw& r) {
+        asm volatile("" : "+v"(r.lo), "+v"(r.hi), "+v"(r.top));
+        d.l[0] = r.lo.x; d.l[1] = r.lo.y; d.l[2] = r.lo.z; d.l[3] = r.lo.w;
+        d.l[4] = r.hi.x; d.l[5] = r.hi.y; d.l[6] = r.hi.z; d.l[7] = r.hi.w;
+        d.l[8] = r.top;
     };
     auto raw_fr = [](Raw& r) -> Fr {
         asm volatile("" : "+v"(r.lo), "+v"(r.hi));
@@ -432,25 +461,27 @@
     uint32_t w0 = prog[0], w1 = prog[1], w2 = prog[2], w3 = prog[3];
     uint32_t n0 = prog[4], n1 = prog[5], n2 = prog[6], n3 = prog[7];
     Raw m;
-    m.lo = U32x4{0, 0, 0, 0}; m.hi = U32x4{0, 0, 0, 0};
+    m.lo = U32x4{0, 0, 0, 0}; m.hi = U32x4{0, 0, 0, 0}; m.top = 0;
     if (w3 & C_HASMEM) load(w1, w2, m);
     for (uint32_t pc = 0; pc < prog_len; ++pc) {
         const uint32_t f0 = prog[4 * pc + 8], f1 = prog[4 * pc + 9], f2 = prog[4 * pc + 10], f3 = prog[4 * pc + 11];
-        if ((w0 & 0xffu) == Q_END) break;
         if (w3 & C_SPILL) { if (sp >= 1) st_put(sp - 1, t0); ++sp; }
-        if (w3 & C_UNPACK_T) q_unpack_to(t0, raw_fr(m));
+        if (w3 & C_UNPACK_T) { if (REC) raw_limbs(t0, m); else q_unpack_to(t0, raw_fr(m)); }
         if (w3 & C_UNPACK_T32) {
             if (w0 & K_SETTLE0) q_settle_ip(t0);
             if (w0 & K_NORM0) normalize29(t0);
             if (w0 & K_SETTLE0_8) q_settle8_ip(t0);
             st_put(sp - 1, t0);
             ++sp;
-            q_unpack_x32_to(t0, raw_fr(m));
-        }
-        if (w3 & C_UNPACK_B) q_unpack_to(B, raw_fr(m));
-        if (w3 & C_UNPACK_B32) q_unpack_x32_to(B, raw_fr(m));
+            if (REC) raw_limbs(t0, m); else q_unpack_x32_to(t0, raw_fr(m));
+        }
+        if (REC) { if (w3 & (C_UNPACK_B | C_UNPACK_B32)) raw_limbs(B, m); }
+        else {
+            if (w3 & C_UNPACK_B) q_unpack_to(B, raw_fr(m));
+            if (w3 & C_UNPACK_B32) q_unpack_x32_to(B, raw_fr(m));
+        }
         if (w3 & C_POP_B) { st_get(sp - 2, B); --sp; }
-        if (n3 & C_HASMEM) load(n1, n2, m);
+        if (!REC) { if (n3 & C_HASMEM) load(n1, n2, m); }
         if (w3 & C_FLAGS) {
             if (w0 & K_SETTLE0) q_settle_ip(t0);
             if (w0 & K_SETTLE1) q_settle_ip(B);
@@ -459,6 +490,21 @@
             if (w0 & K_SETTLE0_8) q_settle8_ip(t0);
             if (w0 & K_SETTLE1_8) q_settle8_ip(B);
         }
+        if (REC) {
+            if (w3 & C_ADDM) {
+                Q29 M;
+                raw_limbs(M, m);
+#pragma unroll
+                for (int q = 0; q < 9; ++q) t0.l[q] += M.l[q];
+            }
+            if (w3 & C_SUBM) {
+                Q29 M;
+                raw_limbs(M, m);
+#pragma unroll
+                for (int q = 0; q < 9; ++q) t0.l[q] = t0.l[q] + kp_balanced<Fr29P>(2, q) - M.l[q];
+            }
+            if (n3 & C_HASMEM) load(n1, n2, m);
+        }
         if (w3 & C_MULV) mul29_ipa(t0, B);
         if (w3 & C_MULC) mul29_ub_ipa(t0, cst(consts_rp, w1));
         if (w3 & C_MACC) {
@@ -486,12 +532,12 @@
         if (w3 & C_FOLDC) fold(w0, cst(consts_rp, w0 >> K_CONST_SHIFT), B);
         if (w3 & C_RARE) {
             if (w3 & C_PUSHC) {
-                const Q29 c = cst(consts, w1);
+                const Q29 c = cst(REC ? consts_rp : consts, w1);
 #pragma unroll
                 for (int q = 0; q < 9; ++q) t0.l[q] = c.l[q];
             }
             if (w3 & C_ADDC) {
-                const Q29 c = cst(consts, w1);
+                const Q29 c = cst(REC ? consts_rp : consts, w1);
 #pragma unroll
                 for (int q = 0; q < 9; ++q) t0.l[q] += c.l[q];
             }
@@ -500,12 +546,12 @@
                 for (int q = 0; q < 9; ++q) t0.l[q] = B.l[q] + kp_balanced<Fr29P>(2, q) - t0.l[q];
                 normalize29(t0);
             }
-            if (w3 & C_MULS) { q_shl5_ip(t0); mul29_ipb(t0, B); }
+            if (w3 & C_MULS) { if (!REC) q_shl5_ip(t0); mul29_ipb(t0, B); }
             if (w3 & C_MACS) {
                 Q29 S;
                 st_get(sp - 2, S);
                 --sp;
-                q_shl5_ip(t0);
+                if (!REC) q_shl5_ip(t0);
                 mul2add29_ub_ipb(t0, B, S, cst(consts_rp, w0 >> K_CONST_SHIFT));
             }
             if (w3 & C_NEG) {
@@ -513,12 +559,17 @@
                 for (int q = 0; q < 9; ++q) t0.l[q] = kp_balanced<Fr29P>(2, q) - t0.l[q];
                 normalize29(t0);
             }
-            if (w3 & C_SQ) { Q29 s2 = t0; q_shl5_ip(s2); mul29_ipa(t0, s2); }
+            if (w3 & C_SQ) { Q29 s2 = t0; if (!REC) q_shl5_ip(s2); mul29_ipa(t0, s2); }
             if (w3 & C_DBL) {
 #pragma unroll
                 for (int q = 0; q < 9; ++q) t0.l[q] <<= 1;
             }
-            if (w3 & C_TEE) { if (live) stg(tmp + (((uint64_t)w1 << ext_k) + i), pack29_lt2p(t0)); }
+            if (w3 & C_TEE) {
+                if (live) {
+                    if (REC) rec29_store<Fr29P>((Fr*)((char*)tmp + (((uint64_t)w1 << ext_k) * REC29_BYTES)), ne, i, canon29_lt2p(t0));
+                    else stg(tmp + (((uint64_t)w1 << ext_k) + i), pack29_lt2p(t0));
+                }
+            }
             if (w3 & C_FOLD) { fold(w0, cst(consts_rp, w1), t0); --sp; if (sp >= 1) st_get(sp - 1, t0); }
         }
         w0 = n0; w1 = n1; w2 = n2; w3 = n3;
@@ -969,7 +1020,7 @@
 }
 
 struct SlicePlan { std::vector<uint32_t> cut; };
-static bool plan_slices(const uint32_t* prog, uint32_t len, uint32_t ext_k, SlicePlan* out) {
+static bool plan_slices(const uint32_t* prog, uint32_t len, uint32_t ext_k, SlicePlan* out, size_t row_bytes = sizeof(Fr)) {
     const int knob = getenv("ZK_QUOTIENT_SLICES") ? atoi(getenv("ZK_QUOTIENT_SLICES")) : -1;
     if (knob == 0 || (knob < 0 && (len < 2048 || ext_k < 16)) || ext_k < 11) return false;
     std::vector<uint32_t> bpos;
@@ -1003,7 +1054,7 @@
     std::sort(colset.begin(), colset.end()); colset.erase(std::unique(colset.begin(), colset.end()), colset.end());
     if (knob < 0 && reads < 4 * ops.size()) return false;
     const uint64_t rows_in_flight = std::min<uint64_t>(1ull << ext_k, 327680);
-    const uint64_t ws = colset.size() * 32ull * rows_in_flight;
+    const uint64_t ws = colset.size() * (uint64_t)row_bytes * rows_in_flight;
     uint32_t want = knob > 0 ? (uint32_t)knob : (uint32_t)std::min<uint64_t>(64, (ws + (96ull << 20) - 1) / (96ull << 20));
     if (want < 2) return false;
     std::vector<char> ok(bpos.size(), 1);
@@ -1038,9 +1089,42 @@
     return ZK_OK;
 }
 
+__global__ void k_to_records(const Fr* __restrict__ src, Fr* __restrict__ dst, uint64_t n) {
+    const uint64_t i = (uint64_t)blockIdx.x * blockDim.x + threadIdx.x;
+    if (i >= n) return;
+    Fr x = ldg(src + i);
+    for (int j = 0; j < 5; ++j) x = dbl(x);
+    rec29_store<Fr29P>(dst, n, i, unpack29<Fr29P>(x));
+}
+
 extern "C" int zk_quotient_eval(zk_ctx* ctx, const uint32_t* h_program, uint32_t num_instr, const void* const* h_col_ptrs, uint32_t num_cols,
                                 const void* h_consts, uint32_t num_consts, uint32_t k, uint32_t ext_k, int divide_by_vanishing, void* d_out) {
     if (!ctx) return ZK_ERR_INVALID_ARG;
+    static const bool loop_records = getenv("ZK_QUOTIENT_LOOP_RECORDS") && atoi(getenv("ZK_QUOTIENT_LOOP_RECORDS")) == 1;
+    if (loop_records && h_program && d_out && (h_col_ptrs || !num_cols) && ext_k >= 2 && ext_k <= 28) {
+        const uint64_t ne = 1ull << ext_k;
+        std::vector<const void*> recs(num_cols);
+        for (uint32_t c = 0; c < num_cols; ++c) {
+            ZK_REQUIRE(ctx, h_col_ptrs[c], "null column pointer");
+            auto it = ctx->loop_records.find(h_col_ptrs[c]);
+            if (it == ctx->loop_records.end()) {
+                void* img = nullptr;
+                ZK_HIP(ctx, hipMalloc(&img, ne * REC29_BYTES));
+                it = ctx->loop_records.emplace(h_col_ptrs[c], img).first;
+                hipLaunchKernelGGL(k_to_records, dim3((unsigned)((ne + 255) / 256)), dim3(256), 0, ctx->stream, (const Fr*)h_col_ptrs[c], (Fr*)img, ne);
+                ZK_CHECK_LAUNCH(ctx);
+            }
+            recs[c] = it->second;
+        }
+        int rc = zk::quotient_eval_fmt(ctx, h_program, num_instr, recs.data(), num_cols, h_consts, num_consts, k, ext_k, divide_by_vanishing, d_out, true);
+        if (rc) return rc;
+        return fr_scale_run(ctx, (Fr*)d_out, fr_inv_host(fr_from_u64(32)), ne);
+    }
+    return zk::quotient_eval_fmt(ctx, h_program, num_instr, h_col_ptrs, num_cols, h_consts, num_consts, k, ext_k, divide_by_vanishing, d_out, false);
+}
+
+int zk::quotient_eval_fmt(zk_ctx* ctx, const uint32_t* h_program, uint32_t num_instr, const void* const* h_col_ptrs, uint32_t num_cols, const void* h_consts, uint32_t num_consts, uint32_t k,
+                          uint32_t ext_k, int divide_by_vanishing, void* d_out, bool records) {
     ZK_REQUIRE(ctx, h_program && d_out && (h_col_ptrs || !num_cols) && (h_consts || !num_consts), "null pointer");
     ZK_REQUIRE(ctx, k <= ext_k && ext_k <= 28, "need k <= ext_k <= 28");
     int depth = 0;
@@ -1049,11 +1133,13 @@
     if (rc) return rc;
     const int kernel_knob = getenv("ZK_QUOTIENT_KERNEL") ? atoi(getenv("ZK_QUOTIENT_KERNEL")) : 2;
     const bool v2 = kernel_knob != 1;
+    if (records && (!v2 || ext_k < 2 || ext_k > 26)) return ctx->fail(ZK_ERR_UNSUPPORTED, "quotient program: record operands need k_quotient_eval2 and 2^2 .. 2^26 rows");
+    const size_t tmp_row_bytes = records ? REC29_BYTES : sizeof(Fr);
     const int mac_level = getenv("ZK_QUOTIENT_MAC") ? atoi(getenv("ZK_QUOTIENT_MAC")) : 2;
     const bool mac = v2 && mac_level != 0, mac2 = mac && mac_level != 1;
     const uint64_t ne = 1ull << ext_k;
     SlicePlan plan;
-    const bool sliced = v2 && ((ne / Q_THREADS) & 7) == 0 && plan_slices(h_program, num_instr, ext_k, &plan);
+    const bool sliced = v2 && ((ne / Q_THREADS) & 7) == 0 && plan_slices(h_program, num_instr, ext_k, &plan, records ? REC29_BYTES : sizeof(Fr));
     const uint32_t S = sliced ? (uint32_t)plan.cut.size() - 1 : 1;
     std::vector<std::vector<LowInstr>> lows(S);
     std::vector<Fr> slice_k;
@@ -1103,7 +1189,7 @@
     if (depth < 1) depth = 1;
     Fr* d_tmp = nullptr;
     if (num_tmp) {
-        d_tmp = (Fr*)ctx->get_scratch(SC_QTMP, ((size_t)num_tmp << ext_k) * sizeof(Fr));
+        d_tmp = (Fr*)ctx->get_scratch(SC_QTMP, ((size_t)num_tmp << ext_k) * tmp_row_bytes);
         if (!d_tmp) return ZK_ERR_OOM;
     }
     uint32_t low_len = 0;
@@ -1148,7 +1234,7 @@
     for (Fr& c : consts_rp) c = times32(c);
     for (Fr& t : tev) t = times32(t);
     std::vector<const void*> col_tab(h_col_ptrs, h_col_ptrs + num_cols);
-    for (uint32_t t = 0; t < num_tmp; ++t) col_tab.push_back(d_tmp + ((size_t)t << ext_k));
+    for (uint32_t t = 0; t < num_tmp; ++t) col_tab.push_back((const char*)d_tmp + ((size_t)t << ext_k) * tmp_row_bytes);
     std::vector<LowInstr> comb;
     if (sliced) {
         if (nc_all >= (1u << (32 - K_CONST_SHIFT))) return ctx->fail(ZK_ERR_UNSUPPORTED, "quotient program: too many constants for a sliced launch");
@@ -1175,7 +1261,7 @@
         size_t w = 0;
         for (uint32_t sl = 0; sl < S; ++sl) {
             slice_tab[2 * sl] = (uint32_t)w; slice_tab[2 * sl + 1] = (uint32_t)lows[sl].size() + 1;
-            for (const LowInstr& in : lows[sl]) { hp[w++] = in.w0; hp[w++] = in.a; hp[w++] = in.b; if (v2) hp[w++] = q_class_mask(in.w0); }
+            for (const LowInstr& in : lows[sl]) { hp[w++] = in.w0; hp[w++] = in.a; hp[w++] = in.b; if (v2) hp[w++] = q_class_mask(in.w0, records); }
             for (int e = 0; e < 4; ++e) { hp[w++] = Q_END; hp[w++] = 0; hp[w++] = 0; if (v2) hp[w++] = 0; }
         }
         comb_at = w;
@@ -1207,10 +1293,14 @@
         ZK_HIP(ctx, hipFuncSetAttribute((const void*)k_quotient_eval<false, false>, hipFuncAttributeMaxDynamicSharedMemorySize, lds_max));
         ZK_HIP(ctx, hipFuncSetAttribute((const void*)k_quotient_eval<true, true>, hipFuncAttributeMaxDynamicSharedMemorySize, lds_max));
         ZK_HIP(ctx, hipFuncSetAttribute((const void*)k_quotient_eval<false, true>, hipFuncAttributeMaxDynamicSharedMemorySize, lds_max));
-        ZK_HIP(ctx, hipFuncSetAttribute((const void*)k_quotient_eval2<true, false>, hipFuncAttributeMaxDynamicSharedMemorySize, lds_max));
-        ZK_HIP(ctx, hipFuncSetAttribute((const void*)k_quotient_eval2<false, false>, hipFuncAttributeMaxDynamicSharedMemorySize, lds_max));
-        ZK_HIP(ctx, hipFuncSetAttribute((const void*)k_quotient_eval2<true, true>, hipFuncAttributeMaxDynamicSharedMemorySize, lds_max));
-        ZK_HIP(ctx, hipFuncSetAttribute((const void*)k_quotient_eval2<false, true>, hipFuncAttributeMaxDynamicSharedMemorySize, lds_max));
+        ZK_HIP(ctx, hipFuncSetAttribute((const void*)k_quotient_eval2<true, false, false>, hipFuncAttributeMaxDynamicSharedMemorySize, lds_max));
+        ZK_HIP(ctx, hipFuncSetAttribute((const void*)k_quotient_eval2<false, false, false>, hipFuncAttributeMaxDynamicSharedMemorySize, lds_max));
+        ZK_HIP(ctx, hipFuncSetAttribute((const void*)k_quotient_eval2<true, true, false>, hipFuncAttributeMaxDynamicSharedMemorySize, lds_max));
+        ZK_HIP(ctx, hipFuncSetAttribute((const void*)k_quotient_eval2<false, true, false>, hipFuncAttributeMaxDynamicSharedMemorySize, lds_max));
+        ZK_HIP(ctx, hipFuncSetAttribute((const void*)k_quotient_eval2<true, false, true>, hipFuncAttributeMaxDynamicSharedMemorySize, lds_max));
+        ZK_HIP(ctx, hipFuncSetAttribute((const void*)k_quotient_eval2<false, false, true>, hipFuncAttributeMaxDynamicSharedMemorySize, lds_max));
+        ZK_HIP(ctx, hipFuncSetAttribute((const void*)k_quotient_eval2<true, true, true>, hipFuncAttributeMaxDynamicSharedMemorySize, lds_max));
+        ZK_HIP(ctx, hipFuncSetAttribute((const void*)k_quotient_eval2<false, true, true>, hipFuncAttributeMaxDynamicSharedMemorySize, lds_max));
         ctx->quotient_attr_set = true;
     }
     ZkProfScope ps(ctx, ctx->prof_tag ? ctx->prof_tag : "quotient_eval");
@@ -1239,10 +1329,14 @@
                                tev.empty() || sliced ? (const Fr*)nullptr : (const Fr*)d_tev, ext_k, k, sliced ? d_part : (Fr*)d_out, d_tmp, d_acc, sliced ? 0u : tile_alias,
                                (const uint32_t*)d_prog + slice_tab_at, sliced ? S : 0u);
         };
-        if (v2 && full && acc_in_mem) launch2(k_quotient_eval2<true, true>);
-        else if (v2 && full) launch2(k_quotient_eval2<true, false>);
-        else if (v2 && acc_in_mem) launch2(k_quotient_eval2<false, true>);
-        else if (v2) launch2(k_quotient_eval2<false, false>);
+        if (records && full && acc_in_mem) launch2(k_quotient_eval2<true, true, true>);
+        else if (records && full) launch2(k_quotient_eval2<true, false, true>);
+        else if (records && acc_in_mem) launch2(k_quotient_eval2<false, true, true>);
+        else if (records) launch2(k_quotient_eval2<false, false, true>);
+        else if (v2 && full && acc_in_mem) launch2(k_quotient_eval2<true, true, false>);
+        else if (v2 && full) launch2(k_quotient_eval2<true, false, false>);
+        else if (v2 && acc_in_mem) launch2(k_quotient_eval2<false, true, false>);
+        else if (v2) launch2(k_quotient_eval2<false, false, false>);
         else if (full && acc_in_mem) launch(k_quotient_eval<true, true>);
         else if (full) launch(k_quotient_eval<true, false>);
         else if (acc_in_mem) launch(k_quotient_eval<false, true>);
@@ -1251,7 +1345,7 @@
     ZK_CHECK_LAUNCH(ctx);
     if (sliced) {
         const dim3 grid((unsigned)((ne + Q_THREADS - 1) / Q_THREADS)), block(Q_THREADS);
-        hipLaunchKernelGGL((k_quotient_eval2<true, false>), grid, block, (size_t)9 * Q_THREADS * 4, ctx->stream, (const uint32_t*)d_prog + comb_at, S + 1, (const Fr* const*)d_cols, (const QC29*)d_consts,
+        hipLaunchKernelGGL((k_quotient_eval2<true, false, false>), grid, block, (size_t)9 * Q_THREADS * 4, ctx->stream, (const uint32_t*)d_prog + comb_at, S + 1, (const Fr* const*)d_cols, (const QC29*)d_consts,
                            (const QC29*)(d_consts + nc_all), tev.empty() ? (const Fr*)nullptr : (const Fr*)d_tev, ext_k, k, (Fr*)d_out, d_tmp, (uint32_t*)nullptr, 0u, (const uint32_t*)nullptr, 0u);
         ZK_CHECK_LAUNCH(ctx);
     }
@@ -1263,9 +1357,13 @@
 extern "C" int zk_fr_powers(zk_ctx* ctx, const void* h_base, const void* h_mul, void* d_out, size_t n) {
     if (!ctx) return ZK_ERR_INVALID_ARG;
     ZK_REQUIRE(ctx, h_base && h_mul && d_out, "null pointer");
+    return zk::fr_powers_fmt(ctx, *(const Fr*)h_base, *(const Fr*)h_mul, d_out, n, false);
+}
+int zk::fr_powers_fmt(zk_ctx* ctx, const Fr& base, const Fr& mul, void* d_out, size_t n, bool records) {
     ZK_REQUIRE(ctx, n <= (1ull << 28), "too many powers");
+    ZK_REQUIRE(ctx, !records || (n & 3) == 0, "a record buffer has a multiple of four rows");
     if (!n) return ZK_OK;
-    hipLaunchKernelGGL(zk::k_powers, dim3((unsigned)((n + 255) / 256)), dim3(256), 0, ctx->stream, *(const Fr*)h_base, *(const Fr*)h_mul, (Fr*)d_out, (uint32_t)n, 0);
+    hipLaunchKernelGGL(zk::k_powers, dim3((unsigned)((n + 255) / 256)), dim3(256), 0, ctx->stream, base, mul, (Fr*)d_out, (uint32_t)n, records ? 2 : 0);
     ZK_CHECK_LAUNCH(ctx);
     return ZK_OK;
 }
```

New measurement: 1.776 (median of 6 runs). -3.3%, faster.
